# Kostis-S-Z/exploring_meta

Hardware: AMD Instinct MI355X
Metric: tasks/sec (higher is better)
Workload: dtype f32

## Files before the change

### exploring_meta_amd/_lib.py

```python

import ctypes as C
import os
import subprocess

_HERE = os.path.dirname(os.path.abspath(__file__))
CSRC = os.path.join(_HERE, 'csrc')
LIB_PATH = os.path.join(CSRC, 'libmi_maml.so')

_lib = None


class MiModelDesc(C.Structure):
    _fields_ = [('n_layers', C.c_int32), ('in_channels', C.c_int32), ('in_h', C.c_int32), ('in_w', C.c_int32),
                ('hidden', C.c_int32), ('max_pool', C.c_int32), ('ways', C.c_int32), ('head_mean_pool', C.c_int32)]


class MiPolicyDesc(C.Structure):
    _fields_ = [('state_size', C.c_int32), ('action_size', C.c_int32), ('hidden1', C.c_int32), ('hidden2', C.c_int32),
                ('activation', C.c_int32)]


class MiBnTangentArgs(C.Structure):
    _fields_ = [('z', C.c_void_p), ('zd', C.c_void_p), ('mu', C.c_void_p), ('rstd', C.c_void_p), ('m1', C.c_void_p),
                ('m2', C.c_void_p), ('gamma', C.c_void_p), ('beta', C.c_void_p), ('pstride', C.c_size_t),
                ('gammad', C.c_void_p), ('betad', C.c_void_p), ('vstride', C.c_size_t), ('dgamma', C.c_void_p),
                ('dbeta', C.c_void_p), ('gstride', C.c_size_t), ('dp', C.c_void_p), ('dpd', C.c_void_p),
                ('tasks', C.c_int32), ('n', C.c_int32), ('ho', C.c_int32), ('wo', C.c_int32), ('c', C.c_int32),
                ('pool', C.c_int32)]


class MiBlock1Args(C.Structure):
    _fields_ = [('x', C.c_void_p), ('w', C.c_void_p), ('wd', C.c_void_p), ('gamma', C.c_void_p), ('beta', C.c_void_p),
                ('pstride', C.c_size_t), ('gammad', C.c_void_p), ('betad', C.c_void_p), ('vstride', C.c_size_t),
                ('mu', C.c_void_p), ('rstd', C.c_void_p), ('m1', C.c_void_p), ('m2', C.c_void_p), ('dgamma', C.c_void_p),
                ('dbeta', C.c_void_p), ('gstride', C.c_size_t), ('rdgamma', C.c_void_p), ('rdbeta', C.c_void_p),
                ('hstride', C.c_size_t), ('dp', C.c_void_p), ('dpd', C.c_void_p), ('arg_in', C.c_void_p), ('zh_in', C.c_void_p),
                ('tasks', C.c_int32), ('n', C.c_int32), ('h', C.c_int32), ('w_', C.c_int32), ('ci', C.c_int32), ('co', C.c_int32)]


class MiTailArgs(C.Structure):
    _fields_ = [('z', C.c_void_p), ('zd', C.c_void_p), ('mu', C.c_void_p), ('rstd', C.c_void_p), ('m1', C.c_void_p), ('m2', C.c_void_p),
                ('gamma', C.c_void_p), ('beta', C.c_void_p), ('wl', C.c_void_p), ('bl', C.c_void_p), ('pstride', C.c_size_t),
                ('gammad', C.c_void_p), ('betad', C.c_void_p), ('wld', C.c_void_p), ('bld', C.c_void_p), ('vstride', C.c_size_t),
                ('y', C.c_void_p), ('f', C.c_void_p), ('dp', C.c_void_p), ('prob', C.c_void_p), ('dl', C.c_void_p),
                ('pooled', C.c_void_p), ('loss', C.c_void_p), ('acc', C.c_void_p), ('logits', C.c_void_p),
                ('dwl', C.c_void_p), ('dbl', C.c_void_p), ('sum0', C.c_void_p), ('sum1', C.c_void_p), ('gstride', C.c_size_t),
                ('df', C.c_void_p),
                ('tasks', C.c_int32), ('n', C.c_int32), ('ho', C.c_int32), ('wo', C.c_int32), ('c', C.c_int32), ('pool', C.c_int32),
                ('ways', C.c_int32), ('with_grad', C.c_int32), ('bwd_tasks', C.c_int32)]


class MiError(RuntimeError):
    pass


def build(verbose=False):
    r = subprocess.run(['make', '-C', CSRC, '-j4'], capture_output=True, text=True)
    if verbose or r.returncode != 0:
        print(r.stdout[-4000:], r.stderr[-4000:])
    if r.returncode != 0:
        raise MiError('building libmi_maml.so failed')
    return LIB_PATH


_SIGS = {
    'mi_engine_create': (C.c_int, [C.POINTER(MiModelDesc), C.c_int, C.POINTER(C.c_void_p)]),
    'mi_engine_destroy': (None, [C.c_void_p]),
    'mi_last_error': (C.c_char_p, [C.c_void_p]),
    'mi_version': (C.c_char_p, []),
    'mi_engine_set_fused_block1': (C.c_int, [C.c_void_p, C.c_int]),
    'mi_engine_set_overlap': (C.c_int, [C.c_void_p, C.c_int]),
    'mi_engine_set_graph': (C.c_int, [C.c_void_p, C.c_int]),
    'mi_engine_set_bn_export': (C.c_int, [C.c_void_p, C.c_void_p, C.c_size_t]),
    'mi_engine_set_fused_finalize': (C.c_int, [C.c_void_p, C.c_int]),
    'mi_engine_set_fused_block1_reduce': (C.c_int, [C.c_void_p, C.c_int]),
    'mi_debug_plan_offsets': (C.c_int, [C.c_void_p, C.c_int, C.c_int, C.c_int, C.c_int, C.c_int, C.POINTER(C.c_size_t)]),
    'mi_param_count': (C.c_int, [C.c_void_p, C.POINTER(C.c_size_t)]),
    'mi_workspace_bytes': (C.c_int, [C.c_void_p, C.c_int, C.c_int, C.c_int, C.c_int, C.c_int, C.POINTER(C.c_size_t)]),
    'mi_meta_batch_maml': (C.c_int, [C.c_void_p, C.c_void_p, C.c_void_p, C.c_void_p, C.c_void_p, C.c_int, C.c_int, C.c_int,
                                     C.c_int, C.c_float, C.c_int, C.c_int, C.c_void_p, C.c_void_p, C.c_void_p, C.c_void_p,
                                     C.c_void_p, C.c_size_t]),
    'mi_meta_batch_maml_tv': (C.c_int, [C.c_void_p, C.c_void_p, C.c_void_p, C.c_void_p, C.c_void_p, C.c_int, C.c_int, C.c_int, C.c_int,
                                        C.c_int, C.c_float, C.c_int, C.c_void_p, C.c_void_p, C.c_void_p, C.c_void_p, C.c_void_p, C.c_size_t]),
    'mi_workspace_bytes_lr': (C.c_int, [C.c_void_p, C.c_int, C.c_int, C.c_int, C.c_int, C.c_int, C.c_int, C.c_int, C.POINTER(C.c_size_t)]),
    'mi_meta_batch_maml_lr': (C.c_int, [C.c_void_p, C.c_void_p, C.c_void_p, C.c_void_p, C.c_void_p, C.c_int, C.c_int, C.c_int, C.c_int,
                                        C.c_int, C.c_void_p, C.c_int, C.c_int, C.c_void_p, C.c_void_p, C.c_void_p, C.c_void_p, C.c_void_p,
                                        C.c_void_p, C.c_size_t]),
    'mi_workspace_bytes_steps': (C.c_int, [C.c_void_p, C.c_int, C.c_int, C.c_int, C.c_int, C.c_int, C.c_int, C.c_int, C.c_int,
                                           C.POINTER(C.c_size_t)]),
    'mi_meta_batch_maml_steps': (C.c_int, [C.c_void_p, C.c_void_p, C.c_void_p, C.c_void_p, C.c_void_p, C.c_int, C.c_int, C.c_int, C.c_int,
                                           C.c_int, C.c_float, C.c_void_p, C.c_int, C.c_void_p, C.c_int, C.c_void_p, C.c_void_p, C.c_void_p,
                                           C.c_void_p, C.c_void_p, C.c_void_p, C.c_size_t]),
    'mi_engine_set_fused_tail': (C.c_int, [C.c_void_p, C.c_int]),
    'mi_engine_set_fused_last_block': (C.c_int, [C.c_void_p, C.c_int]),
    'mi_debug_tail_stamps': (C.c_int, [C.c_void_p, C.c_void_p]),
    'mi_anil_workspace_bytes': (C.c_int, [C.c_void_p, C.c_int, C.c_int, C.c_int, C.c_int, C.POINTER(C.c_size_t)]),
    'mi_meta_batch_anil': (C.c_int, [C.c_void_p, C.c_void_p, C.c_void_p, C.c_void_p, C.c_void_p, C.c_int, C.c_int, C.c_int,
                                     C.c_int, C.c_float, C.c_int, C.c_int, C.c_void_p, C.c_void_p, C.c_void_p, C.c_void_p,
                                     C.c_void_p, C.c_size_t]),
    'mi_anil_workspace_bytes_steps': (C.c_int, [C.c_void_p] + [C.c_int] * 9 + [C.POINTER(C.c_size_t)]),
    'mi_meta_batch_anil_lr': (C.c_int, [C.c_void_p, C.c_void_p, C.c_void_p, C.c_void_p, C.c_void_p, C.c_int, C.c_int, C.c_int, C.c_int,
                                        C.c_void_p, C.c_int, C.c_int, C.c_int, C.c_void_p, C.c_void_p, C.c_void_p, C.c_void_p, C.c_void_p,
                                        C.c_void_p, C.c_size_t]),
    'mi_meta_batch_anil_steps': (C.c_int, [C.c_void_p, C.c_void_p, C.c_void_p, C.c_void_p, C.c_void_p, C.c_int, C.c_int, C.c_int, C.c_int,
                                           C.c_float, C.c_void_p, C.c_int, C.c_void_p, C.c_int, C.c_int, C.c_void_p, C.c_void_p, C.c_void_p,
                                           C.c_void_p, C.c_void_p, C.c_void_p, C.c_size_t]),
    'mi_forward_workspace_bytes': (C.c_int, [C.c_void_p, C.c_int, C.c_int, C.POINTER(C.c_size_t)]),
    'mi_forward_logits': (C.c_int, [C.c_void_p, C.c_void_p, C.c_void_p, C.c_void_p, C.c_int, C.c_int, C.c_void_p, C.c_void_p,
                                    C.c_size_t]),
    'mi_learner_forward': (C.c_int, [C.c_void_p, C.c_void_p, C.c_void_p, C.c_int, C.c_void_p, C.c_int, C.c_int, C.c_void_p,
                                     C.c_int, C.c_void_p, C.c_void_p, C.c_size_t]),
    'mi_learner_backward': (C.c_int, [C.c_void_p, C.c_void_p, C.c_void_p, C.c_int, C.c_void_p, C.c_void_p, C.c_int, C.c_int,
                                      C.c_void_p, C.c_void_p, C.c_size_t]),
    'mi_learner_hvp_workspace_bytes': (C.c_int, [C.c_void_p, C.c_int, C.c_int, C.POINTER(C.c_size_t)]),
    'mi_learner_hvp': (C.c_int, [C.c_void_p, C.c_void_p, C.c_void_p, C.c_int, C.c_void_p, C.c_void_p, C.c_void_p, C.c_int, C.c_int,
                                 C.c_void_p, C.c_void_p, C.c_void_p, C.c_size_t]),
    'mi_cg_update': (C.c_int, [C.c_void_p, C.c_void_p, C.c_void_p, C.c_void_p, C.c_void_p, C.c_void_p, C.c_void_p, C.c_size_t, C.c_double]),
    'mi_cg_update_checked': (C.c_int, [C.c_void_p, C.c_void_p, C.c_void_p, C.c_void_p, C.c_void_p, C.c_void_p, C.c_void_p, C.c_size_t, C.c_double, C.c_double]),
    'mi_cg_init': (C.c_int, [C.c_void_p, C.c_void_p, C.c_void_p, C.c_void_p, C.c_void_p, C.c_void_p, C.c_void_p, C.c_size_t]),
    'mi_trpo_scale_step': (C.c_int, [C.c_void_p, C.c_void_p, C.c_void_p, C.c_size_t, C.c_float, C.c_void_p, C.c_void_p]),
    'mi_gae_max_rows': (C.c_int, [C.c_int]),
    'mi_upload_i32': (C.c_int, [C.c_void_p, C.c_void_p, C.c_void_p, C.c_int]),
    'mi_copy_segments': (C.c_int, [C.c_void_p, C.c_void_p, C.c_void_p, C.c_void_p, C.c_void_p, C.c_int]),
    'mi_gae_advantages': (C.c_int, [C.c_void_p, C.c_void_p, C.c_void_p, C.c_void_p, C.c_void_p, C.c_void_p, C.c_void_p, C.c_int, C.c_int,
                                    C.c_int, C.c_double, C.c_double, C.c_double, C.c_int, C.c_void_p, C.c_void_p]),
    'mi_adam_step': (C.c_int, [C.c_void_p, C.c_void_p, C.c_void_p, C.c_void_p, C.c_void_p, C.c_size_t, C.c_int, C.c_float,
                               C.c_float, C.c_float, C.c_float, C.c_float]),
    'mi_prepare_batch': (C.c_int, [C.c_void_p, C.c_void_p, C.c_void_p, C.c_int, C.c_int, C.c_int, C.c_int, C.c_int,
                                   C.c_void_p, C.c_void_p, C.c_void_p, C.c_void_p]),
    'mi_input_gram_scratch_bytes': (C.c_size_t, [C.c_int, C.c_int, C.c_int, C.c_int]),
    'mi_input_gram': (C.c_int, [C.c_void_p, C.c_void_p, C.c_int, C.c_int, C.c_int, C.c_int, C.c_int, C.c_void_p, C.c_size_t, C.c_void_p]),
    'mi_gram_bn_stats': (C.c_int, [C.c_void_p, C.c_void_p, C.c_int, C.c_int, C.c_int, C.c_void_p, C.c_size_t, C.c_void_p, C.c_size_t,
                                   C.c_int, C.c_void_p, C.c_void_p, C.c_void_p, C.c_void_p]),
    'mi_cka_scratch_bytes': (C.c_size_t, [C.c_int, C.c_int, C.c_int]),
    'mi_cka': (C.c_int, [C.c_void_p, C.c_void_p, C.c_void_p, C.c_int, C.c_int, C.c_int, C.c_double, C.c_void_p, C.c_size_t,
                         C.c_void_p]),
    'mi_cca_scratch_bytes': (C.c_size_t, [C.c_int, C.c_int, C.c_int]),
    'mi_cca': (C.c_int, [C.c_void_p, C.c_void_p, C.c_void_p, C.c_int, C.c_int, C.c_int, C.c_double, C.c_double, C.c_void_p,
                         C.c_size_t, C.c_void_p, C.c_void_p]),
    'mi_stream_copy': (C.c_int, [C.c_void_p, C.c_void_p, C.c_void_p, C.c_size_t]),
    'mi_sample_tasks': (C.c_int, [C.c_void_p, C.c_void_p, C.c_int, C.c_size_t, C.c_int, C.c_int, C.c_int, C.c_void_p, C.c_void_p,
                                  C.c_int, C.c_int, C.c_void_p]),
    'mi_draw_tasks': (C.c_int, [C.c_void_p, C.c_void_p, C.c_void_p, C.c_int, C.c_int, C.c_int, C.c_void_p, C.c_int, C.c_int, C.c_uint64,
                                C.c_uint64, C.c_uint64, C.c_int, C.c_void_p, C.c_void_p, C.c_void_p, C.c_void_p]),
    'mi_conv3x3_bn_stats': (C.c_int, [C.c_void_p, C.c_void_p, C.c_void_p, C.c_size_t, C.c_int, C.c_int, C.c_int, C.c_int,
                                      C.c_int, C.c_int, C.c_int, C.c_void_p, C.c_void_p, C.c_void_p, C.c_void_p, C.c_size_t]),
    'mi_bn_relu_pool': (C.c_int, [C.c_void_p, C.c_void_p, C.c_void_p, C.c_void_p, C.c_void_p, C.c_void_p, C.c_size_t,
                                  C.c_int, C.c_int, C.c_int, C.c_int, C.c_int, C.c_int, C.c_void_p]),
    'mi_bn_relu_pool_bwd': (C.c_int, [C.c_void_p, C.c_void_p, C.c_void_p, C.c_void_p, C.c_void_p, C.c_void_p, C.c_size_t,
                                      C.c_void_p, C.c_int, C.c_int, C.c_int, C.c_int, C.c_int, C.c_int, C.c_void_p,
                                      C.c_void_p, C.c_size_t, C.c_void_p, C.c_void_p, C.c_size_t]),
    'mi_conv3x3_bwd': (C.c_int, [C.c_void_p, C.c_void_p, C.c_void_p, C.c_void_p, C.c_size_t, C.c_int, C.c_int, C.c_int,
                                 C.c_int, C.c_int, C.c_int, C.c_int, C.c_void_p, C.c_void_p, C.c_size_t, C.c_void_p, C.c_size_t]),
    'mi_head_fwd_bwd': (C.c_int, [C.c_void_p, C.c_void_p, C.c_void_p, C.c_void_p, C.c_size_t, C.c_void_p, C.c_int, C.c_int,
                                  C.c_int, C.c_int, C.c_void_p, C.c_void_p, C.c_void_p, C.c_void_p, C.c_void_p, C.c_void_p,
                                  C.c_void_p, C.c_size_t, C.c_void_p]),
    'mi_kernel_scratch_bytes': (C.c_size_t, [C.c_int, C.c_int, C.c_int, C.c_int, C.c_int]),
    'mi_head_grads': (C.c_int, [C.c_void_p, C.c_void_p, C.c_void_p, C.c_size_t, C.c_void_p] + [C.c_int] * 4 +
                      [C.c_void_p, C.c_void_p, C.c_size_t, C.c_void_p]),
    'mi_head_tangent': (C.c_int, [C.c_void_p] * 5 + [C.c_size_t, C.c_void_p, C.c_void_p, C.c_size_t] + [C.c_void_p] * 4 + [C.c_int] * 5 +
                        [C.c_void_p, C.c_void_p, C.c_size_t, C.c_void_p]),
    'mi_spatial_mean': (C.c_int, [C.c_void_p, C.c_void_p, C.c_void_p, C.c_int, C.c_int, C.c_int]),
    'mi_spatial_mean_bwd': (C.c_int, [C.c_void_p, C.c_void_p, C.c_void_p, C.c_int, C.c_int, C.c_int]),
    'mi_tail_supported': (C.c_int, [C.c_int] * 7),
    'mi_tail_lds_bytes': (C.c_size_t, [C.c_int] * 4),
    'mi_tail_scratch_bytes': (C.c_size_t, [C.c_int] * 7),
    'mi_tail_run': (C.c_int, [C.c_void_p, C.POINTER(MiTailArgs), C.c_int, C.c_void_p, C.c_size_t]),
    'mi_conv3x3_tangent': (C.c_int, [C.c_void_p] * 5 + [C.c_size_t] + [C.c_void_p] * 3 + [C.c_int] * 7 + [C.c_void_p] * 4 + [C.c_size_t]),
    'mi_conv3x3_bwd2': (C.c_int, [C.c_void_p] * 7 + [C.c_size_t] + [C.c_int] * 7 + [C.c_void_p, C.c_void_p, C.c_size_t, C.c_void_p, C.c_size_t]),
    'mi_bn_tangent_fwd': (C.c_int, [C.c_void_p, C.POINTER(MiBnTangentArgs), C.c_void_p]),
    'mi_bn_tangent_bwd': (C.c_int, [C.c_void_p, C.POINTER(MiBnTangentArgs), C.c_void_p, C.c_void_p, C.c_size_t, C.c_void_p,
                                    C.c_void_p, C.c_size_t]),
    'mi_block1_scratch_bytes': (C.c_size_t, [C.c_int] * 6),
    'mi_block1_run': (C.c_int, [C.c_void_p, C.c_int, C.POINTER(MiBlock1Args), C.c_void_p, C.c_void_p, C.c_void_p, C.c_void_p,
                                C.c_void_p, C.c_size_t, C.c_void_p, C.c_size_t]),
    'mi_pooled_reduce': (C.c_int, [C.c_void_p] * 6 + [C.c_int] * 3 + [C.c_void_p, C.c_void_p, C.c_size_t, C.c_void_p, C.c_size_t]),
    'mi_block1_wgrad_gram': (C.c_int, [C.c_void_p, C.POINTER(MiBlock1Args), C.c_void_p, C.c_int, C.c_void_p, C.c_size_t,
                                       C.c_void_p, C.c_size_t]),
    'mi_debug_conv_tiles_per_wave': (C.c_int, [C.c_int] * 5),
    'mi_debug_wgrad_plan': (C.c_int, [C.c_int] * 8 + [C.POINTER(C.c_int)]),
    'mi_debug_conv_plan': (C.c_int, [C.c_int] * 10 + [C.POINTER(C.c_int)]),
    'mi_debug_set_trace': (C.c_int, [C.c_void_p, C.c_void_p, C.c_size_t]),
    'mi_policy_create': (C.c_int, [C.POINTER(MiPolicyDesc), C.c_int, C.POINTER(C.c_void_p)]),
    'mi_policy_destroy': (None, [C.c_void_p]),
    'mi_policy_last_error': (C.c_char_p, [C.c_void_p]),
    'mi_policy_param_count': (C.c_int, [C.c_void_p, C.POINTER(C.c_size_t)]),
    'mi_policy_forward': (C.c_int, [C.c_void_p, C.c_void_p, C.c_void_p, C.c_size_t, C.c_void_p, C.c_int, C.c_int, C.c_void_p,
                                    C.c_void_p, C.c_size_t]),
    'mi_particles_rollout_scratch_bytes': (C.c_size_t, [C.c_void_p, C.c_int, C.c_int, C.c_int]),
    'mi_particles_rollout': (C.c_int, [C.c_void_p, C.c_void_p, C.c_void_p, C.c_size_t, C.c_void_p, C.c_void_p, C.c_uint64, C.c_int, C.c_int,
                                       C.c_int] + [C.c_void_p] * 8 + [C.c_void_p, C.c_size_t]),
    'mi_policy_adapt': (C.c_int, [C.c_void_p, C.c_void_p, C.c_void_p, C.c_size_t, C.c_void_p, C.c_void_p, C.c_void_p,
                                  C.c_void_p, C.c_int, C.c_int, C.c_float, C.c_int, C.c_void_p, C.c_void_p, C.c_void_p, C.c_size_t]),
    'mi_policy_set_fused_fvp': (C.c_int, [C.c_int]),
    'mi_debug_policy_sweep_stamps': (C.c_int, [C.c_void_p]),
    'mi_policy_learner_workspace_bytes': (C.c_int, [C.c_void_p, C.c_int, C.c_int, C.POINTER(C.c_size_t)]),
    'mi_policy_vjp': (C.c_int, [C.c_void_p, C.c_void_p, C.c_void_p, C.c_size_t, C.c_void_p, C.c_void_p, C.c_void_p, C.c_int, C.c_int, C.c_int,
                                C.c_void_p, C.c_void_p, C.c_size_t]),
    'mi_policy_hvp': (C.c_int, [C.c_void_p, C.c_void_p, C.c_void_p, C.c_size_t, C.c_void_p, C.c_void_p, C.c_void_p, C.c_void_p, C.c_int, C.c_int,
                                C.c_int, C.c_void_p, C.c_void_p, C.c_void_p, C.c_size_t]),
    'mi_policy_set_fused_learner': (C.c_int, [C.c_int]),
    'mi_policy_learner_fused_supported': (C.c_int, [C.c_void_p]),
    'mi_debug_conv_stamps': (C.c_int, [C.c_void_p]),
    'mi_conv_set_split_bf16': (C.c_int, [C.c_int]),
    'mi_conv_get_split_bf16': (C.c_int, [C.POINTER(C.c_uint)]),
    'mi_conv_set_b16': (C.c_int, [C.c_int]),
    'mi_block1_set_split_bf16': (C.c_int, [C.c_int]),
    'mi_sparse_wgrad_set_split_bf16': (C.c_int, [C.c_int]),
    'mi_policy_meta_workspace_bytes': (C.c_int, [C.c_void_p, C.c_int, C.c_int, C.c_int, C.c_int, C.c_int, C.POINTER(C.c_size_t)]),
    'mi_policy_meta_batch': (C.c_int, [C.c_void_p, C.c_void_p, C.c_void_p, C.c_int, C.c_void_p, C.c_void_p, C.c_int] + [C.c_void_p] * 8 +
                             [C.c_int, C.c_int, C.c_int, C.c_float, C.c_float, C.c_int, C.c_int, C.c_int, C.c_void_p, C.c_void_p,
                              C.c_void_p, C.c_void_p, C.c_size_t]),
    'mi_policy_meta_batch_dones': (C.c_int, [C.c_void_p, C.c_void_p, C.c_void_p, C.c_int, C.c_void_p, C.c_void_p, C.c_int] + [C.c_void_p] * 10 +
                                   [C.c_int, C.c_int, C.c_int, C.c_float, C.c_float, C.c_int, C.c_int, C.c_int, C.c_void_p, C.c_void_p,
                                    C.c_void_p, C.c_void_p, C.c_size_t]),
    'mi_policy_update_workspace_bytes': (C.c_int, [C.c_void_p, C.c_int, C.c_int, C.POINTER(C.c_size_t)]),
    'mi_policy_update': (C.c_int, [C.c_void_p, C.c_void_p, C.c_void_p, C.c_size_t] + [C.c_void_p] * 5 +
                         [C.c_int, C.c_int, C.c_int, C.c_int, C.c_float, C.c_float, C.c_int, C.c_void_p, C.c_void_p, C.c_void_p, C.c_size_t]),
    'mi_policy_meta_lr_workspace_bytes': (C.c_int, [C.c_void_p, C.c_int, C.c_int, C.c_int, C.c_int, C.c_int, C.c_int, C.c_int,
                                                    C.POINTER(C.c_size_t)]),
    'mi_policy_meta_batch_lr': (C.c_int, [C.c_void_p, C.c_void_p, C.c_void_p, C.c_int, C.c_void_p, C.c_void_p, C.c_void_p, C.c_int] +
                                [C.c_void_p] * 10 + [C.c_int, C.c_int, C.c_int, C.c_float, C.c_void_p, C.c_int, C.c_int, C.c_int, C.c_int] +
                                [C.c_void_p] * 5 + [C.c_size_t]),
    'mi_policy_update_lr': (C.c_int, [C.c_void_p, C.c_void_p, C.c_void_p, C.c_size_t] + [C.c_void_p] * 5 +
                            [C.c_int, C.c_int, C.c_int, C.c_int, C.c_float, C.c_void_p, C.c_int, C.c_void_p, C.c_void_p, C.c_void_p, C.c_size_t]),
    'mi_trpo_steps_workspace_bytes': (C.c_int, [C.c_void_p, C.c_int, C.c_int, C.c_int, C.POINTER(C.c_size_t)]),
    'mi_trpo_surrogate_steps': (C.c_int, [C.c_void_p, C.c_void_p, C.c_void_p, C.c_int] + [C.c_void_p] * 10 +
                                [C.c_int, C.c_int, C.c_float, C.c_void_p, C.c_void_p, C.c_void_p, C.c_void_p, C.c_size_t]),
    'mi_trpo_fvp_steps': (C.c_int, [C.c_void_p, C.c_void_p, C.c_int] + [C.c_void_p] * 5 +
                          [C.c_int, C.c_int, C.c_float, C.c_float, C.c_void_p, C.c_void_p, C.c_void_p, C.c_size_t]),
    'mi_trpo_general_steps_workspace_bytes': (C.c_int, [C.c_void_p, C.c_int, C.c_int, C.c_int, C.POINTER(C.c_size_t)]),
    'mi_trpo_kl_prepare_steps': (C.c_int, [C.c_void_p, C.c_void_p, C.c_int] + [C.c_void_p] * 7 +
                                 [C.c_int, C.c_int, C.c_float, C.c_void_p, C.c_void_p, C.c_size_t]),
    'mi_trpo_fvp_general_steps': (C.c_int, [C.c_void_p, C.c_void_p, C.c_int] + [C.c_void_p] * 6 +
                                  [C.c_int, C.c_int, C.c_float, C.c_float, C.c_void_p, C.c_void_p, C.c_void_p, C.c_size_t]),
    'mi_policy_adapt_lr': (C.c_int, [C.c_void_p, C.c_void_p, C.c_void_p, C.c_size_t, C.c_void_p, C.c_void_p, C.c_void_p,
                                     C.c_void_p, C.c_int, C.c_int, C.c_void_p, C.c_int, C.c_void_p, C.c_void_p, C.c_void_p, C.c_size_t]),
    'mi_trpo_steps_lr_workspace_bytes': (C.c_int, [C.c_void_p, C.c_int, C.c_int, C.c_int, C.c_int, C.POINTER(C.c_size_t)]),
    'mi_trpo_surrogate_steps_lr': (C.c_int, [C.c_void_p, C.c_void_p, C.c_void_p, C.c_int] + [C.c_void_p] * 10 +
                                   [C.c_int, C.c_int, C.c_void_p, C.c_int, C.c_void_p, C.c_void_p, C.c_void_p, C.c_void_p, C.c_void_p,
                                    C.c_size_t]),
    'mi_trpo_fvp_steps_lr': (C.c_int, [C.c_void_p, C.c_void_p, C.c_int] + [C.c_void_p] * 5 +
                             [C.c_int, C.c_int, C.c_void_p, C.c_int, C.c_void_p, C.c_float, C.c_void_p, C.c_void_p, C.c_void_p, C.c_size_t]),
    'mi_trpo_general_steps_lr_workspace_bytes': (C.c_int, [C.c_void_p, C.c_int, C.c_int, C.c_int, C.c_int, C.POINTER(C.c_size_t)]),
    'mi_trpo_kl_prepare_steps_lr': (C.c_int, [C.c_void_p, C.c_void_p, C.c_int] + [C.c_void_p] * 7 +
                                    [C.c_int, C.c_int, C.c_void_p, C.c_int, C.c_void_p, C.c_void_p, C.c_void_p, C.c_size_t]),
    'mi_trpo_fvp_general_steps_lr': (C.c_int, [C.c_void_p, C.c_void_p, C.c_int] + [C.c_void_p] * 6 +
                                     [C.c_int, C.c_int, C.c_void_p, C.c_int, C.c_void_p, C.c_float, C.c_void_p, C.c_void_p, C.c_void_p,
                                      C.c_size_t]),
    'mi_profile_enable': (C.c_int, [C.c_void_p, C.c_int, C.c_int]),
    'mi_profile_kinds': (C.c_int, []),
    'mi_profile_op_name': (C.c_char_p, [C.c_int]),
    'mi_profile_collect': (C.c_int, [C.c_void_p, C.POINTER(C.c_double), C.POINTER(C.c_int64), C.c_int]),
}

EXPORTS = tuple(_SIGS)


def load():
    global _lib
    if _lib is not None:
        return _lib
    path = os.environ.get('MI_MAML_LIB', LIB_PATH)
    if not os.path.exists(path):
        raise MiError(f'{path} is missing: run `python -c "import __graft_entry__ as g; g.build()"` '
                      '(hipcc --offload-arch=gfx950). There is no CPU fallback for the MAML hot path.')
    import torch
    lib = C.CDLL(path)
    for name, (res, args) in _SIGS.items():
        fn = getattr(lib, name)
        fn.restype = res
        fn.argtypes = args
    _lib = lib
    return lib


def check(rc, handle=None):
    if rc != 0:
        msg = load().mi_last_error(handle)
        raise MiError(f'libmi_maml error {rc}: {msg.decode() if msg else "?"}')
```

### exploring_meta_amd/csrc/bn_pool.hip

```cpp
#include "mi_common.h"
#include "kernels.h"

#include "bn_window.h"

#define BN_THREAD_SETUP(POOL)                                                                   \
  const int quads = a.c >> 2;                                                                   \
  const int quad = threadIdx.x % quads, wl = threadIdx.x / quads, wpb = 256 / quads;            \
  const int task = blockIdx.y, c0 = quad * 4;                                                   \
  const WinIter<POOL> it(a);                                                                    \
  const size_t z_task = (size_t)a.n * a.ho * a.wo * a.c;                                        \
  const size_t p_task = (size_t)a.n * it.hp * it.wp * a.c;                                      \
  const ChanConst k = load_consts(a, task, c0);                                                 \
  const float* z_t = a.z + (size_t)task * z_task;                                               \
  (void)p_task; (void)z_t;

__device__ __forceinline__ void block_reduce_write(const double* acc0, const double* acc1, const BnArgs& a, int quads,
                                                   int task) {
  __shared__ double red[256 * 8];
#pragma unroll
  for (int c = 0; c < 4; ++c) {
    red[threadIdx.x * 8 + c] = acc0[c];
    red[threadIdx.x * 8 + 4 + c] = acc1[c];
  }
  __syncthreads();
  if ((int)threadIdx.x < a.c) {
    const int q = threadIdx.x >> 2, comp = threadIdx.x & 3, wpb = 256 / quads;
    double s0 = 0.0, s1 = 0.0;
    for (int w = 0; w < wpb; ++w) {
      s0 += red[(w * quads + q) * 8 + comp];
      s1 += red[(w * quads + q) * 8 + 4 + comp];
    }
    double* pb = a.partial + ((size_t)task * gridDim.x + blockIdx.x) * 2 * a.c;
    mi_partial_store(pb + threadIdx.x, s0, a.fin);
    mi_partial_store(pb + a.c + threadIdx.x, s1, a.fin);
  }
  mi_finalize_last(a.fin, a.partial + (size_t)task * gridDim.x * 2 * a.c, gridDim.x, a.c, task, gridDim.x, red);
}

template <int POOL>
__global__ __launch_bounds__(256) void bn_fwd_kernel(BnArgs a) {
  BN_THREAD_SETUP(POOL)
  float* out_t = a.out + (size_t)task * p_task;
  float* zh_t = a.zh_out ? a.zh_out + (size_t)task * p_task : nullptr;
  unsigned am = 0u;
  Window<POOL> w;
  for (int win = blockIdx.x * wpb + wl; win < it.nwin; win += gridDim.x * wpb) {
    w.locate(a, it, win, c0);
    if (!w.pooled) continue;
    floatx4 umax, zh_at, zd_at;
    scan_window<POOL, false>(w, z_t, nullptr, k, umax, zh_at, zd_at);
    floatx4 o;
#pragma unroll
    for (int c = 0; c < 4; ++c) { o[c] = fmaxf(umax[c], 0.f); mi_amax_acc(am, o[c]); }
    *reinterpret_cast<floatx4*>(out_t + w.poff) = o;
    if (zh_t) *reinterpret_cast<floatx4*>(zh_t + w.poff) = zh_at;
  }
  if (a.amax_out) mi_amax_commit(am, a.amax_out, task);
}

template <int POOL>
__global__ __launch_bounds__(256) void bn_bwd_reduce_kernel(BnArgs a) {
  BN_THREAD_SETUP(POOL)
  const float* dp_t = a.dp + (size_t)task * p_task;
  double dg[4] = {0, 0, 0, 0}, db[4] = {0, 0, 0, 0};
  Window<POOL> w;
  for (int win = blockIdx.x * wpb + wl; win < it.nwin; win += gridDim.x * wpb) {
    w.locate(a, it, win, c0);
    if (!w.pooled) continue;
    floatx4 umax, zh_at, zd_at;
    scan_window<POOL, false>(w, z_t, nullptr, k, umax, zh_at, zd_at);
    const floatx4 d = *reinterpret_cast<const floatx4*>(dp_t + w.poff);
#pragma unroll
    for (int c = 0; c < 4; ++c) {
      const float du = umax[c] > 0.f ? d[c] : 0.f;
      db[c] += (double)du;
      dg[c] += (double)du * (double)zh_at[c];
    }
  }
  block_reduce_write(dg, db, a, quads, task);
}

template <int POOL>
__global__ __launch_bounds__(256) void bn_bwd_apply_kernel(BnArgs a) {
  BN_THREAD_SETUP(POOL)
  const float* dp_t = a.dp + (size_t)task * p_task;
  float* out_t = a.out + (size_t)task * z_task;
  float dgm[4], dbm[4], gr[4];
  load4(a.dgamma + (size_t)task * a.gstride + c0, dgm);
  load4(a.dbeta + (size_t)task * a.gstride + c0, dbm);
#pragma unroll
  for (int c = 0; c < 4; ++c) { dgm[c] *= a.inv_m; dbm[c] *= a.inv_m; gr[c] = k.g[c] * k.r[c]; }
  unsigned am = 0u;
  Window<POOL> w;
  for (int win = blockIdx.x * wpb + wl; win < it.nwin; win += gridDim.x * wpb) {
    w.locate(a, it, win, c0);
    w.analyse(z_t, k);
    float d[4] = {0.f, 0.f, 0.f, 0.f};
    if (w.pooled) load4(dp_t + w.poff, d);
#pragma unroll
    for (int p = 0; p < Window<POOL>::NP; ++p) {
      if (!w.exists[p]) continue;
      float o[4];
#pragma unroll
      for (int c = 0; c < 4; ++c) {
        const float du = (w.pooled && w.arg[c] == p && w.umax[c] > 0.f) ? d[c] : 0.f;
        o[c] = gr[c] * (du - dbm[c] - w.zh[p][c] * dgm[c]);
        mi_amax_acc(am, o[c]);
      }
      store4(out_t + w.off[p], o);
    }
  }
  if (a.amax_out) mi_amax_commit(am, a.amax_out, task);
}

template <int POOL>
__global__ __launch_bounds__(256) void bn_tan_fwd_kernel(BnArgs a) {
  BN_THREAD_SETUP(POOL)
  const float* zd_t = a.zd + (size_t)task * z_task;
  float* out_t = a.out + (size_t)task * p_task;
  float m1[4], m2[4], gd[4], bd[4];
  load4(a.m1 + (size_t)task * a.c + c0, m1);
  load4(a.m2 + (size_t)task * a.c + c0, m2);
  load4(a.gammad + (size_t)task * a.vstride + c0, gd);
  load4(a.betad + (size_t)task * a.vstride + c0, bd);
  unsigned am = 0u;
  Window<POOL> w;
  for (int win = blockIdx.x * wpb + wl; win < it.nwin; win += gridDim.x * wpb) {
    w.locate(a, it, win, c0);
    if (!w.pooled) continue;
    floatx4 umax, zh_at, zd_at;
    scan_window<POOL, true>(w, z_t, zd_t, k, umax, zh_at, zd_at);
    floatx4 o, zo;
#pragma unroll
    for (int c = 0; c < 4; ++c) {
      const float zhd = k.r[c] * (zd_at[c] - m1[c] - zh_at[c] * m2[c]);
      const float ud = gd[c] * zh_at[c] + k.g[c] * zhd + bd[c];
      o[c] = (umax[c] > 0.f) ? ud : 0.f;
      zo[c] = zhd;
      mi_amax_acc(am, o[c]);
    }
    *reinterpret_cast<floatx4*>(out_t + w.poff) = o;
    if (a.zh_out) *reinterpret_cast<floatx4*>(a.zh_out + (size_t)task * p_task + w.poff) = zo;
  }
  if (a.amax_out) mi_amax_commit(am, a.amax_out, task);
}

template <int POOL>
__global__ __launch_bounds__(256) void bn_tan_bwd_reduce_kernel(BnArgs a) {
  BN_THREAD_SETUP(POOL)
  const float* zd_t = a.zd + (size_t)task * z_task;
  const float* dp_t = a.dp + (size_t)task * p_task;
  const float* dpd_t = a.dpd + (size_t)task * p_task;
  float m1[4], m2[4];
  load4(a.m1 + (size_t)task * a.c + c0, m1);
  load4(a.m2 + (size_t)task * a.c + c0, m2);
  double rg[4] = {0, 0, 0, 0}, rb[4] = {0, 0, 0, 0};
  Window<POOL> w;
  for (int win = blockIdx.x * wpb + wl; win < it.nwin; win += gridDim.x * wpb) {
    w.locate(a, it, win, c0);
    if (!w.pooled) continue;
    floatx4 umax, zh_at, zd_at;
    scan_window<POOL, true>(w, z_t, zd_t, k, umax, zh_at, zd_at);
    const floatx4 d = *reinterpret_cast<const floatx4*>(dp_t + w.poff);
    const floatx4 dd = *reinterpret_cast<const floatx4*>(dpd_t + w.poff);
#pragma unroll
    for (int c = 0; c < 4; ++c) {
      const bool on = umax[c] > 0.f;
      const float du = on ? d[c] : 0.f, dud = on ? dd[c] : 0.f;
      const float zhd = k.r[c] * (zd_at[c] - m1[c] - zh_at[c] * m2[c]);
      rb[c] += (double)dud;
      rg[c] += (double)dud * (double)zh_at[c] + (double)du * (double)zhd;
    }
  }
  block_reduce_write(rg, rb, a, quads, task);
}

template <int POOL>
__global__ __launch_bounds__(256) void bn_tan_bwd_apply_kernel(BnArgs a) {
  BN_THREAD_SETUP(POOL)
  const float* zd_t = a.zd + (size_t)task * z_task;
  const float* dp_t = a.dp + (size_t)task * p_task;
  const float* dpd_t = a.dpd + (size_t)task * p_task;
  float* out_t = a.out + (size_t)task * z_task;
  float m1[4], m2[4], gd[4], dgm[4], dbm[4], rgm[4], rbm[4], c1[4], gr[4];
  load4(a.m1 + (size_t)task * a.c + c0, m1);
  load4(a.m2 + (size_t)task * a.c + c0, m2);
  load4(a.gammad + (size_t)task * a.vstride + c0, gd);
  load4(a.dgamma + (size_t)task * a.gstride + c0, dgm);
  load4(a.dbeta + (size_t)task * a.gstride + c0, dbm);
  load4(a.rdgamma + (size_t)task * a.hstride + c0, rgm);
  load4(a.rdbeta + (size_t)task * a.hstride + c0, rbm);
#pragma unroll
  for (int c = 0; c < 4; ++c) {
    dgm[c] *= a.inv_m; dbm[c] *= a.inv_m; rgm[c] *= a.inv_m; rbm[c] *= a.inv_m;
    const float rd = -k.r[c] * k.r[c] * m2[c];
    c1[c] = gd[c] * k.r[c] + k.g[c] * rd;
    gr[c] = k.g[c] * k.r[c];
  }
  unsigned am = 0u;
  Window<POOL> w;
  for (int win = blockIdx.x * wpb + wl; win < it.nwin; win += gridDim.x * wpb) {
    w.locate(a, it, win, c0);
    w.analyse(z_t, k);
    float d[4] = {0.f, 0.f, 0.f, 0.f}, dd[4] = {0.f, 0.f, 0.f, 0.f};
    if (w.pooled) { load4(dp_t + w.poff, d); load4(dpd_t + w.poff, dd); }
#pragma unroll
    for (int p = 0; p < Window<POOL>::NP; ++p) {
      if (!w.exists[p]) continue;
      float zdv[4], o[4];
      load4(zd_t + w.off[p], zdv);
#pragma unroll
      for (int c = 0; c < 4; ++c) {
        const bool sel = w.pooled && w.arg[c] == p && w.umax[c] > 0.f;
        const float du = sel ? d[c] : 0.f, dud = sel ? dd[c] : 0.f;
        const float zh = w.zh[p][c];
        const float zhd = k.r[c] * (zdv[c] - m1[c] - zh * m2[c]);
        const float e = du - dbm[c] - zh * dgm[c];
        o[c] = c1[c] * e + gr[c] * (dud - rbm[c] - zhd * dgm[c] - zh * rgm[c]);
        mi_amax_acc(am, o[c]);
      }
      store4(out_t + w.off[p], o);
    }
  }
  if (a.amax_out) mi_amax_commit(am, a.amax_out, task);
}

__global__ __launch_bounds__(256) void bn_finalize_kernel(const double* __restrict__ partial, int nblk, int c, FinArgs f) {
  __shared__ double red[2 * 256];
  mi_fold_partials<false>(partial + (size_t)blockIdx.x * nblk * 2 * c, nblk, c, f, blockIdx.x, red);
}

template <bool TAN>
__global__ __launch_bounds__(256) void pooled_reduce_kernel(PoolRedArgs a) {
  __shared__ double red[256 * 8];
  const int task = blockIdx.y, quads = a.c >> 2, wpb = 256 / quads;
  const int q = threadIdx.x % quads, rl = threadIdx.x / quads;
  const size_t base = (size_t)task * a.rows * a.c + 4 * q;
  double s0[4] = {0, 0, 0, 0}, s1[4] = {0, 0, 0, 0};
  if (rl < wpb)
    for (int row = blockIdx.x * wpb + rl; row < a.rows; row += gridDim.x * wpb) {
      const size_t off = base + (size_t)row * a.c;
      float p[4], d[4], zh[4], dd[4], zhd[4];
      load4(a.p + off, p); load4(a.dp + off, d); load4(a.zh + off, zh);
      if (TAN) { load4(a.dpd + off, dd); load4(a.zhd + off, zhd); }
#pragma unroll
      for (int c = 0; c < 4; ++c) {
        const bool on = p[c] > 0.f;
        const float dv = on ? d[c] : 0.f;
        if (!TAN) {
          s0[c] += (double)dv * (double)zh[c];
          s1[c] += (double)dv;
        } else {
          const float ddv = on ? dd[c] : 0.f;
          s0[c] += (double)ddv * (double)zh[c] + (double)dv * (double)zhd[c];
          s1[c] += (double)ddv;
        }
      }
    }
#pragma unroll
  for (int c = 0; c < 4; ++c) {
    red[threadIdx.x * 8 + c] = s0[c];
    red[threadIdx.x * 8 + 4 + c] = s1[c];
  }
  __syncthreads();
  if ((int)threadIdx.x < a.c) {
    const int qq = threadIdx.x >> 2, comp = threadIdx.x & 3;
    double t0 = 0.0, t1 = 0.0;
    for (int w = 0; w < wpb; ++w) {
      t0 += red[(w * quads + qq) * 8 + comp];
      t1 += red[(w * quads + qq) * 8 + 4 + comp];
    }
    double* pb = a.partial + ((size_t)task * gridDim.x + blockIdx.x) * 2 * a.c;
    mi_partial_store(pb + threadIdx.x, t0, a.fin);
    mi_partial_store(pb + a.c + threadIdx.x, t1, a.fin);
  }
  mi_finalize_last(a.fin, a.partial + (size_t)task * gridDim.x * 2 * a.c, gridDim.x, a.c, task, gridDim.x, red);
}

int pooled_reduce_blocks(int rows, int c, int tasks) {
  const int wpb = 256 / (c / 4);
  int blocks = ceil_div(rows, wpb);
  const int cap = ceil_div(2048, tasks);
  if (blocks > cap) blocks = cap;
  return blocks < 1 ? 1 : blocks;
}
hipError_t launch_pooled_reduce(hipStream_t st, const PoolRedArgs& a, int tasks, int tangent, int* nblk) {
  if (a.c % 4 || a.c > 256 || 256 % (a.c / 4)) return hipErrorInvalidValue;
  const int blocks = pooled_reduce_blocks(a.rows, a.c, tasks);
  if (tangent) hipLaunchKernelGGL(pooled_reduce_kernel<true>, dim3(blocks, tasks), dim3(256), 0, st, a);
  else hipLaunchKernelGGL(pooled_reduce_kernel<false>, dim3(blocks, tasks), dim3(256), 0, st, a);
  *nblk = blocks;
  return hipGetLastError();
}

int bn_blocks_per_task(int n, int ho, int wo, int c, int pool, int tasks) {
  const int nwin = pool ? n * ((ho + 1) / 2) * ((wo + 1) / 2) : n * ho * wo;
  const int wpb = 256 / (c / 4);
  int blocks = ceil_div(nwin, wpb);
  const int cap = ceil_div(2048, tasks);
  if (blocks > cap) blocks = cap;
  if (blocks < 1) blocks = 1;
  return blocks;
}

hipError_t launch_bn_finalize(hipStream_t st, const double* partial, int nblk, int tasks, int c, double inv_m, int mode,
                              float* out0, size_t stride0, float* out1, size_t stride1) {
  if (c > 256 || 256 % c != 0) return hipErrorInvalidValue;
  const FinArgs f{nullptr, out0, out1, stride0, stride1, inv_m, mode};
  hipLaunchKernelGGL(bn_finalize_kernel, dim3(tasks), dim3(256), 0, st, partial, nblk, c, f);
  return hipGetLastError();
}

#define BN_LAUNCH(KERNEL)                                                                          \
  const int blocks = bn_blocks_per_task(a.n, a.ho, a.wo, a.c, pool, tasks);                        \
  dim3 grid(blocks, tasks);                                                                        \
  if (pool) hipLaunchKernelGGL(KERNEL<1>, grid, dim3(256), 0, st, a);                              \
  else hipLaunchKernelGGL(KERNEL<0>, grid, dim3(256), 0, st, a);

hipError_t launch_bn_fwd(hipStream_t st, const BnArgs& a, int tasks, int pool) {
  BN_LAUNCH(bn_fwd_kernel)
  return hipGetLastError();
}
hipError_t launch_bn_bwd_reduce(hipStream_t st, const BnArgs& a, int tasks, int pool, int* nblk) {
  BN_LAUNCH(bn_bwd_reduce_kernel)
  *nblk = blocks;
  return hipGetLastError();
}
hipError_t launch_bn_bwd_apply(hipStream_t st, const BnArgs& a, int tasks, int pool) {
  BN_LAUNCH(bn_bwd_apply_kernel)
  return hipGetLastError();
}
hipError_t launch_bn_tan_fwd(hipStream_t st, const BnArgs& a, int tasks, int pool) {
  BN_LAUNCH(bn_tan_fwd_kernel)
  return hipGetLastError();
}
hipError_t launch_bn_tan_bwd_reduce(hipStream_t st, const BnArgs& a, int tasks, int pool, int* nblk) {
  BN_LAUNCH(bn_tan_bwd_reduce_kernel)
  *nblk = blocks;
  return hipGetLastError();
}
hipError_t launch_bn_tan_bwd_apply(hipStream_t st, const BnArgs& a, int tasks, int pool) {
  BN_LAUNCH(bn_tan_bwd_apply_kernel)
  return hipGetLastError();
}
```

### exploring_meta_amd/csrc/bn_window.h

```cpp
#pragma once
#include "mi_common.h"
#include "kernels.h"

struct ChanConst {
  float mu[4], r[4], g[4], b[4];
};

__device__ __forceinline__ void load4(const float* p, float* o) {
  const float4 v = *reinterpret_cast<const float4*>(p);
  o[0] = v.x; o[1] = v.y; o[2] = v.z; o[3] = v.w;
}
__device__ __forceinline__ void store4(float* p, const float* o) {
  *reinterpret_cast<float4*>(p) = make_float4(o[0], o[1], o[2], o[3]);
}

__device__ __forceinline__ ChanConst load_consts(const BnArgs& a, int task, int c0) {
  ChanConst k;
  load4(a.mu + (size_t)task * a.c + c0, k.mu);
  load4(a.rstd + (size_t)task * a.c + c0, k.r);
  load4(a.gamma + (size_t)task * a.pstride + c0, k.g);
  load4(a.beta + (size_t)task * a.pstride + c0, k.b);
  return k;
}

template <int POOL>
struct WinIter {
  int hw2, ww2, nwin, hp, wp;
  __device__ WinIter(const BnArgs& a) {
    if (POOL) {
      hw2 = (a.ho + 1) >> 1; ww2 = (a.wo + 1) >> 1; hp = a.ho >> 1; wp = a.wo >> 1;
    } else {
      hw2 = a.ho; ww2 = a.wo; hp = a.ho; wp = a.wo;
    }
    nwin = a.n * hw2 * ww2;
  }
};

template <int POOL>
struct Window {
  static constexpr int NP = POOL ? 4 : 1;
  size_t off[NP];
  bool exists[NP];
  bool pooled;
  size_t poff;
  float zh[NP][4], u[NP][4];
  int arg[4];
  float umax[4];
  bool better[NP][4];

  __device__ __forceinline__ void locate(const BnArgs& a, const WinIter<POOL>& it, int win, int c0) {
    const int n = win / (it.hw2 * it.ww2);
    const int rem = win - n * it.hw2 * it.ww2;
    const int wy = rem / it.ww2, wx = rem - wy * it.ww2;
    if (POOL) {
#pragma unroll
      for (int k = 0; k < NP; ++k) {
        const int y = 2 * wy + (k >> 1), x = 2 * wx + (k & 1);
        exists[k] = (y < a.ho) && (x < a.wo);
        off[k] = ((size_t)(n * a.ho + y) * a.wo + x) * a.c + c0;
      }
      pooled = (wy < it.hp) && (wx < it.wp);
      poff = ((size_t)(n * it.hp + wy) * it.wp + wx) * a.c + c0;
    } else {
      exists[0] = true;
      off[0] = ((size_t)(n * a.ho + wy) * a.wo + wx) * a.c + c0;
      pooled = true;
      poff = off[0];
    }
  }
  __device__ __forceinline__ void analyse(const float* __restrict__ z_t, const ChanConst& k) {
#pragma unroll
    for (int p = 0; p < NP; ++p) {
      float zv[4] = {0.f, 0.f, 0.f, 0.f};
      if (exists[p]) load4(z_t + off[p], zv);
#pragma unroll
      for (int c = 0; c < 4; ++c) {
        zh[p][c] = bn_zh(zv[c], k.mu[c], k.r[c]);
        u[p][c] = bn_u(zh[p][c], k.g[c], k.b[c]);
      }
    }
#pragma unroll
    for (int c = 0; c < 4; ++c) {
      int best = 0;
      float bu = u[0][c];
#pragma unroll
      for (int p = 1; p < NP; ++p) {
        better[p][c] = u[p][c] > bu;
        if (better[p][c]) { bu = u[p][c]; best = p; }
      }
      arg[c] = best;
      umax[c] = bu;
    }
  }
  __device__ __forceinline__ float at_arg(const float (&v)[NP][4], int c) const {
    float r = v[0][c];
#pragma unroll
    for (int p = 1; p < NP; ++p) r = better[p][c] ? v[p][c] : r;
    return r;
  }
};

template <int POOL, bool WITH_ZD>
__device__ __forceinline__ void scan_values(const floatx4* zv, const floatx4* zdv, const ChanConst& k, floatx4& umax, floatx4& zh_at,
                                            floatx4& zd_at) {
#pragma unroll
  for (int p = 0; p < Window<POOL>::NP; ++p) {
    const floatx4 z = zv[p];
    floatx4 zd = {0.f, 0.f, 0.f, 0.f};
    if (WITH_ZD) zd = zdv[p];
#pragma unroll
    for (int c = 0; c < 4; ++c) {
      const float zh = bn_zh(z[c], k.mu[c], k.r[c]);
      const float u = bn_u(zh, k.g[c], k.b[c]);
      if (p == 0) {
        umax[c] = u; zh_at[c] = zh; zd_at[c] = zd[c];
      } else {
        const bool gt = u > umax[c];
        umax[c] = gt ? u : umax[c];
        zh_at[c] = gt ? zh : zh_at[c];
        zd_at[c] = gt ? zd[c] : zd_at[c];
      }
    }
  }
}
template <int POOL, bool WITH_ZD>
__device__ __forceinline__ void scan_window(const Window<POOL>& w, const float* __restrict__ z_t, const float* __restrict__ zd_t,
                                            const ChanConst& k, floatx4& umax, floatx4& zh_at, floatx4& zd_at) {
  floatx4 zv[Window<POOL>::NP], zdv[Window<POOL>::NP];
#pragma unroll
  for (int p = 0; p < Window<POOL>::NP; ++p) {
    zv[p] = *reinterpret_cast<const floatx4*>(z_t + w.off[p]);
    if (WITH_ZD) zdv[p] = *reinterpret_cast<const floatx4*>(zd_t + w.off[p]);
  }
  scan_values<POOL, WITH_ZD>(zv, zdv, k, umax, zh_at, zd_at);
}
```

### exploring_meta_amd/csrc/engine.hip

```cpp
#include <array>
#include <string>
#include <vector>
#include <cstdio>
#include <cmath>
#include <cstring>
#include "mi_common.h"
#include "kernels.h"
#include "../../include/mi_maml.h"

#define EPI_NONE 0
#define EPI_STATS 1
#define EPI_TSTATS 2
#define EPI_BRED 3

static thread_local std::string g_err;

struct Layer {
  int ci, co, h, w, ho, wo, stride, pool, hp, wp;
  size_t off_gamma, off_beta, off_w, off_b;
};

typedef std::array<unsigned long long, 31> GraphKey;
struct mi_engine {
  mi_model_desc d;
  int device;
  std::vector<Layer> L;
  int head_c, head_hw, feat;
  size_t off_wl, off_bl, P;
  size_t PS;
  int32_t* perm_dev;
  bool fuse1 = false;
  bool gram1 = true;
  bool gramq = true;
  bool overlap = true;
  bool fuse_fin = true;
  bool fuse_b1red = true;
  bool fuse_tail = true;
  bool fuse_last = !(getenv("MI_FUSE_LAST") && atoi(getenv("MI_FUSE_LAST")) == 0);
  unsigned long long* tail_stamps = nullptr;
  unsigned zoff[10] = {}, zlen[10] = {};
  int nzero = 0;
  unsigned* counters = nullptr;
  static constexpr int kMaxCounterTasks = 65536;
  struct SideCtx { hipStream_t side = nullptr; hipEvent_t fork = nullptr, join = nullptr; } sc[1];
  std::string err;
  bool graph_on = false;
  struct GraphEntry { GraphKey key; hipGraphExec_t exec = nullptr; hipGraph_t graph = nullptr; int seen = 0; };
  std::vector<GraphEntry> graphs;
  float* bn_export = nullptr;
  size_t bn_export_floats = 0;
  int export_pass = 0;
  float* trace = nullptr;
  size_t trace_floats = 0;
  int prof_on = 0, prof_filter = -1;
  std::vector<hipEvent_t> ev0, ev1;
  std::vector<int> ev_kind;
  size_t ev_used = 0;
};

enum ProfOp { OP_CONV_FWD = 0, OP_BN_FINALIZE, OP_BN_FWD, OP_HEAD, OP_BN_BWD_REDUCE, OP_BN_BWD_APPLY, OP_WGRAD, OP_WGRAD_REDUCE,
              OP_DGRAD, OP_TAN_CONV, OP_BN_TAN_FWD, OP_HEAD_TAN, OP_BN_TAN_BWD_REDUCE, OP_BN_TAN_BWD_APPLY, OP_TAN_WGRAD,
              OP_TAN_DGRAD, OP_MISC, OP_GRAM, OP_GRAM_STATS, OP_COUNT };
static const char* kOpNames[OP_COUNT] = {"conv_fwd_stats", "bn_finalize", "bn_relu_pool_fwd", "head_fwd_bwd", "bn_bwd_reduce",
                                         "bn_bwd_apply", "wgrad", "wgrad_reduce", "dgrad", "tangent_conv_fwd", "bn_tangent_fwd",
                                         "head_tangent", "bn_tangent_bwd_reduce", "bn_tangent_bwd_apply", "tangent_wgrad",
                                         "tangent_dgrad", "misc", "input_gram", "gram_stats"};

static bool prof_begin(mi_engine* e, hipStream_t st, int kind) {
  if (!e || !e->prof_on || (e->prof_filter >= 0 && e->prof_filter != kind)) return false;
  if (e->ev_used == e->ev0.size()) {
    hipEvent_t a, b;
    if (hipEventCreate(&a) != hipSuccess || hipEventCreate(&b) != hipSuccess) return false;
    e->ev0.push_back(a); e->ev1.push_back(b); e->ev_kind.push_back(0);
  }
  e->ev_kind[e->ev_used] = kind;
  (void)hipEventRecord(e->ev0[e->ev_used], st);
  return true;
}
static void prof_end(mi_engine* e, hipStream_t st, bool active) {
  if (!active) return;
  (void)hipEventRecord(e->ev1[e->ev_used], st);
  e->ev_used++;
}

static int fail(mi_engine* e, int code, const std::string& msg) {
  if (e) e->err = msg;
  g_err = msg;
  return code;
}
#define LAUNCH(e, st, op, layer, call)                                                             \
  do {                                                                                             \
    const bool _pa = prof_begin(e, st, (op) * 8 + (layer));                                        \
    hipError_t _s = (call);                                                                        \
    prof_end(e, st, _pa);                                                                          \
    if (_s != hipSuccess)                                                                          \
      return fail(e, MI_ERR_HIP, std::string(#call) + ": " + hipGetErrorString(_s) + " @" + std::to_string(__LINE__)); \
  } while (0)
#define HIPCHK(e, call)                                                                            \
  do {                                                                                             \
    hipError_t _s = (call);                                                                        \
    if (_s != hipSuccess)                                                                          \
      return fail(e, MI_ERR_HIP, std::string(#call) + ": " + hipGetErrorString(_s) + " @" + std::to_string(__LINE__)); \
  } while (0)

static int head_lds_check(mi_engine* e, const char* who, int n, int ways, int tangent) {
  if (head_lds_fits(n, ways, tangent)) return MI_OK;
  return fail(e, MI_ERR_ARG, std::string(who) + ": the classifier head's " + (tangent ? "tangent" : "gradient") + " launch with n = " + std::to_string(n) +
                                 " rows per task and ways = " + std::to_string(ways) + " needs " + std::to_string(head_grads_lds_bytes(n, ways, tangent)) +
                                 " bytes of LDS, the device has " + std::to_string(head_lds_limit_bytes()) + " (n * ways <= " + (tangent ? "19712" : "39424") + ")");
}
#define HEAD_LDS(e, who, n, ways, tangent)                                         \
  do {                                                                             \
    const int _hrc = head_lds_check(e, who, n, ways, tangent);                     \
    if (_hrc) return _hrc;                                                         \
  } while (0)

static FinArgs fin_of(const mi_engine* e, int T, double inv_m, int mode, float* o0, size_t s0, float* o1, size_t s1) {
  const bool on = e->fuse_fin && e->counters && T <= mi_engine::kMaxCounterTasks;
  return FinArgs{on ? e->counters : nullptr, o0, o1, s0, s1, inv_m, mode};
}

static ConvGeom geom(const Layer& l, int n) { return ConvGeom{n, l.h, l.w, l.ho, l.wo, l.ci, l.co, l.stride}; }
static ConvGeom geom_dgrad(const Layer& l, int n) {
  return ConvGeom{n, l.ho, l.wo, l.h, l.w, l.co, l.ci, l.stride};
}

static bool dgrad_carries_reduce(const mi_engine* e, int l) {
  if (!e->fuse_b1red || l < 1 || l >= (int)e->L.size()) return false;
  const Layer& L = e->L[l];
  return L.stride == 1 && L.ci == L.co && L.co == e->L[l - 1].co && L.h == L.ho && L.w == L.wo && (L.ci == 32 || L.ci == 64);
}

extern "C" const char* mi_version(void) { return "mi_maml 0.1 (gfx950)"; }
extern "C" const char* mi_last_error(const mi_engine* e) { return e ? e->err.c_str() : g_err.c_str(); }

extern "C" int mi_engine_create(const mi_model_desc* d, int device, mi_engine** out) {
  if (!d || !out) return fail(nullptr, MI_ERR_ARG, "null argument");
  if (d->n_layers < 1 || d->n_layers > 8) return fail(nullptr, MI_ERR_ARG, "n_layers must be 1..8");
  if (d->hidden != 32 && d->hidden != 64) return fail(nullptr, MI_ERR_ARG, "hidden must be 32 or 64");
  if (d->in_channels != 1 && d->in_channels != 3 && d->in_channels != 32 && d->in_channels != 64)
    return fail(nullptr, MI_ERR_ARG, "in_channels must be 1, 3, 32 or 64");
  if (d->ways < 1 || d->ways > 64) return fail(nullptr, MI_ERR_ARG, "ways must be 1..64");
  mi_engine* e = new mi_engine();
  e->d = *d;
  e->device = device;
  e->perm_dev = nullptr;
  int ci = d->in_channels, h = d->in_h, w = d->in_w;
  size_t off = 0;
  std::vector<int32_t> perm;
  for (int i = 0; i < d->n_layers; ++i) {
    Layer l;
    l.ci = ci; l.co = d->hidden; l.h = h; l.w = w;
    l.stride = d->max_pool ? 1 : 2;
    l.pool = d->max_pool ? 1 : 0;
    l.ho = (h + 2 - 3) / l.stride + 1;
    l.wo = (w + 2 - 3) / l.stride + 1;
    l.hp = l.pool ? l.ho / 2 : l.ho;
    l.wp = l.pool ? l.wo / 2 : l.wo;
    if (l.hp < 1 || l.wp < 1) { delete e; return fail(nullptr, MI_ERR_ARG, "input too small for this many blocks"); }
    l.off_gamma = off; off += l.co;
    l.off_beta = off; off += l.co;
    l.off_w = off; off += (size_t)9 * l.ci * l.co;
    l.off_b = off; off += l.co;
    for (size_t k = perm.size(); k < l.off_w; ++k) perm.push_back((int32_t)k);
    for (int tap = 0; tap < 9; ++tap)
      for (int c1 = 0; c1 < l.ci; ++c1)
        for (int c2 = 0; c2 < l.co; ++c2) perm.push_back((int32_t)(l.off_w + ((size_t)c2 * l.ci + c1) * 9 + tap));
    for (size_t k = perm.size(); k < off; ++k) perm.push_back((int32_t)k);
    e->L.push_back(l);
    ci = l.co; h = l.hp; w = l.wp;
  }
  e->fuse1 = block1_supported(e->L[0].ci, e->L[0].stride, e->L[0].pool, e->L[0].ho, e->L[0].wo, e->L[0].co);
  e->head_c = ci;
  e->head_hw = h * w;
  e->feat = d->head_mean_pool ? ci : ci * h * w;
  e->off_wl = off; off += (size_t)d->ways * e->feat;
  e->off_bl = off; off += d->ways;
  e->P = off;
  e->PS = align_up(off, 64);
  for (const Layer& l : e->L) { e->zoff[e->nzero] = (unsigned)l.off_b; e->zlen[e->nzero] = (unsigned)l.co; e->nzero++; }
  if (e->PS > e->P) { e->zoff[e->nzero] = (unsigned)e->P; e->zlen[e->nzero] = (unsigned)(e->PS - e->P); e->nzero++; }
  for (int wy = 0; wy < d->ways; ++wy)
    for (int i = 0; i < e->feat; ++i) {
      size_t ref;
      if (d->head_mean_pool) ref = (size_t)wy * e->feat + i;
      else { const int s = i / e->head_c, c = i % e->head_c; ref = (size_t)wy * e->feat + (size_t)c * e->head_hw + s; }
      perm.push_back((int32_t)(e->off_wl + ref));
    }
  for (size_t k = perm.size(); k < off; ++k) perm.push_back((int32_t)k);
  int prev = -1;
  (void)hipGetDevice(&prev);
  if (hipSetDevice(device) != hipSuccess) { delete e; return fail(nullptr, MI_ERR_HIP, "hipSetDevice failed"); }
  const bool ok = hipMalloc(&e->perm_dev, perm.size() * sizeof(int32_t)) == hipSuccess &&
                  hipMemcpy(e->perm_dev, perm.data(), perm.size() * sizeof(int32_t), hipMemcpyHostToDevice) == hipSuccess &&
                  hipMalloc(&e->counters, mi_engine::kMaxCounterTasks * sizeof(unsigned)) == hipSuccess &&
                  hipMemset(e->counters, 0, mi_engine::kMaxCounterTasks * sizeof(unsigned)) == hipSuccess;
  if (prev >= 0 && prev != device) (void)hipSetDevice(prev);
  if (!ok) {
    if (e->perm_dev) (void)hipFree(e->perm_dev);
    if (e->counters) (void)hipFree(e->counters);
    delete e;
    return fail(nullptr, MI_ERR_HIP, "allocating the parameter permutation table / arrival counters failed");
  }
  *out = e;
  return MI_OK;
}

extern "C" void mi_engine_destroy(mi_engine* e) {
  if (!e) return;
  if (e->perm_dev) (void)hipFree(e->perm_dev);
  if (e->counters) (void)hipFree(e->counters);
  for (auto& g : e->graphs) {
    if (g.exec) (void)hipGraphExecDestroy(g.exec);
    if (g.graph) (void)hipGraphDestroy(g.graph);
  }
  for (auto& c : e->sc) {
    if (c.fork) (void)hipEventDestroy(c.fork);
    if (c.join) (void)hipEventDestroy(c.join);
  }
  for (auto ev : e->ev0) (void)hipEventDestroy(ev);
  for (auto ev : e->ev1) (void)hipEventDestroy(ev);
  delete e;
}

extern "C" int mi_engine_set_fused_block1(mi_engine* e, int on) {
  if (!e) return MI_ERR_ARG;
  e->fuse1 = on && block1_supported(e->L[0].ci, e->L[0].stride, e->L[0].pool, e->L[0].ho, e->L[0].wo, e->L[0].co);
  e->gram1 = on != 2;
  e->gramq = on != 3;
  return MI_OK;
}

extern "C" int mi_engine_set_fused_finalize(mi_engine* e, int on) {
  if (!e) return MI_ERR_ARG;
  e->fuse_fin = on != 0;
  return MI_OK;
}
extern "C" int mi_engine_set_fused_block1_reduce(mi_engine* e, int on) {
  if (!e) return MI_ERR_ARG;
  e->fuse_b1red = on != 0;
  return MI_OK;
}

extern "C" int mi_engine_set_graph(mi_engine* e, int on) {
  if (!e) return MI_ERR_ARG;
  e->graph_on = on != 0;
  return MI_OK;
}

extern "C" int mi_engine_set_fused_tail(mi_engine* e, int on) {
  if (!e) return MI_ERR_ARG;
  e->fuse_tail = on != 0;
  return MI_OK;
}

extern "C" int mi_engine_set_fused_last_block(mi_engine* e, int on) {
  if (!e) return MI_ERR_ARG;
  e->fuse_last = on != 0;
  return MI_OK;
}

extern "C" int mi_engine_set_overlap(mi_engine* e, int on) {
  if (!e) return MI_ERR_ARG;
  e->overlap = on != 0;
  return MI_OK;
}

static hipStream_t pool_stream(const mi_engine* e, int which) {
  static hipStream_t g_pool[64][1] = {};
  const int d = (e->device >= 0 && e->device < 64) ? e->device : 0;
  if (!g_pool[d][which]) {
    int prev = -1;
    (void)hipGetDevice(&prev);
    if (prev != e->device) (void)hipSetDevice(e->device);
    if (hipStreamCreateWithFlags(&g_pool[d][which], hipStreamNonBlocking) != hipSuccess) g_pool[d][which] = nullptr;
    if (prev >= 0 && prev != e->device) (void)hipSetDevice(prev);
  }
  return g_pool[d][which];
}
static bool make_event(hipEvent_t* ev) { return *ev || hipEventCreateWithFlags(ev, hipEventDisableTiming) == hipSuccess; }

static hipStream_t side_fork(mi_engine* e, hipStream_t st, int half) {
  if (!e->overlap) return st;
  mi_engine::SideCtx& c = e->sc[half];
  if (!c.side) {
    c.side = pool_stream(e, 0);
    if (!c.side || !make_event(&c.fork) || !make_event(&c.join)) { e->overlap = false; return st; }
  }
  if (hipEventRecord(c.fork, st) != hipSuccess || hipStreamWaitEvent(c.side, c.fork, 0) != hipSuccess) return st;
  return c.side;
}
static int side_join(mi_engine* e, hipStream_t st, int half, bool used) {
  if (!used) return MI_OK;
  mi_engine::SideCtx& c = e->sc[half];
  if (hipEventRecord(c.join, c.side) != hipSuccess || hipStreamWaitEvent(st, c.join, 0) != hipSuccess)
    return fail(e, MI_ERR_HIP, "side-stream join failed");
  return MI_OK;
}

extern "C" int mi_engine_set_bn_export(mi_engine* e, float* buf, size_t floats) {
  if (!e) return MI_ERR_ARG;
  e->bn_export = buf;
  e->bn_export_floats = buf ? floats : 0;
  return MI_OK;
}

extern "C" int mi_debug_set_trace(mi_engine* e, float* buf, size_t floats) {
  if (!e) return MI_ERR_ARG;
  e->trace = buf;
  e->trace_floats = buf ? floats : 0;
  return MI_OK;
}

int mi_internal_fail(int code, const char* msg) { return fail(nullptr, code, msg); }

extern "C" int mi_param_count(const mi_engine* e, size_t* n) {
  if (!e || !n) return MI_ERR_ARG;
  *n = e->P;
  return MI_OK;
}

struct Bump {
  char* base;
  size_t off;
  template <class T> T* take(size_t count) {
    off = align_up(off, 256);
    T* p = base ? reinterpret_cast<T*>(base + off) : nullptr;
    off += count * sizeof(T);
    return p;
  }
};

struct ActSet {
  float *z[8], *p[8], *dz[8], *dp[8], *mu[8], *rstd[8];
  float* zhl[8];
  float* zhm;
  uint8_t* arg0;
  float *f, *df, *prob, *dl;
};
struct TanSet {
  float *zd[8], *pd[8], *m1[8], *m2[8];
  float* zhdl[8];
  float* zhdm;
  float* rdz[8];
  float *dpd[2], *fd, *rdf;
};
struct Plan {
  float *theta, *g, *lam, *hv;
  float* lam2;
  float *lrv = nullptr, *dir = nullptr, *dir2 = nullptr, *prod = nullptr;
  float* qg = nullptr;
  float *xs, *xq;
  int32_t *ys, *yq;
  std::vector<ActSet> sup;
  ActSet qry;
  TanSet tan;
  double* bnpart;
  float* wgpart;
  float* wgpart_side;
  float* wgpart_l[8];
  double *gram_part, *gram_s;
  double *gram_q, *gram_part_q;
  int half = 0;
  float *tmp_loss, *tmp_acc;
  float* hscr;
  float* tail_wpart = nullptr; double* tail_bpart = nullptr; float* tail_scr = nullptr;
  unsigned* cells;
  int cell_cap, cell_used = 0, cell_T = 0;
  bool f16 = false;
  std::vector<std::pair<const void*, unsigned*>> cellmap;
  size_t bytes;
};

static void plan_actset(const mi_engine* e, Bump& b, ActSet& A, int T, int n, bool with_bwd) {
  const int nl = (int)e->L.size();
  A.zhm = nullptr;
  A.arg0 = nullptr;
  for (int l = 0; l < 8; ++l) A.zhl[l] = nullptr;
  for (int l = 0; l < nl; ++l) {
    const Layer& L = e->L[l];
    const size_t zs = (size_t)T * n * L.ho * L.wo * L.co, ps = (size_t)T * n * L.hp * L.wp * L.co;
    const bool fused = (l == 0 && e->fuse1);
    A.z[l] = fused ? nullptr : b.take<float>(zs);
    A.p[l] = b.take<float>(ps);
    A.dz[l] = (with_bwd && !fused) ? b.take<float>(zs) : nullptr;
    A.dp[l] = with_bwd ? b.take<float>(ps) : nullptr;
    if (fused && with_bwd && e->gram1) { A.zhm = b.take<float>(ps); A.arg0 = b.take<uint8_t>(ps); }
    A.zhl[l] = (!fused && with_bwd && l >= 1 && L.pool && dgrad_carries_reduce(e, l + 1)) ? b.take<float>(ps) : nullptr;
    A.mu[l] = b.take<float>((size_t)T * L.co);
    A.rstd[l] = b.take<float>((size_t)T * L.co);
  }
  if (e->d.head_mean_pool) {
    A.f = b.take<float>((size_t)T * n * e->feat);
    A.df = with_bwd ? b.take<float>((size_t)T * n * e->feat) : nullptr;
  } else {
    A.f = A.p[nl - 1];
    A.df = A.dp[nl - 1];
  }
  A.prob = b.take<float>((size_t)T * n * e->d.ways);
  A.dl = b.take<float>((size_t)T * n * e->d.ways);
}

static unsigned long long kernel_selection_key() {
  unsigned mask = 0;
  const unsigned form = (unsigned)mi_conv_get_split_bf16(&mask);
  return (unsigned long long)form + 4ull * (unsigned)conv_b16() + 16ull * (unsigned)block1_split_form() + 64ull * (unsigned)sparse_wgrad_split_form() + 128ull * (unsigned long long)mask;
}

struct PlanShape { int T, ns, nq, K, second_order, lr_steps, want_lr_grad, steps; };
static PlanShape maml_shape(int tasks, int ways, int shots, int K, int second_order, int lr_steps, int want_lr_grad, int steps = 0) {
  return PlanShape{tasks, ways * shots, ways * shots, K, second_order, lr_steps, want_lr_grad, steps};
}
static PlanShape forward_shape(int tasks, int n) { return PlanShape{tasks, n, n, 0, 0, 0, 0, 0}; }
static PlanShape hvp_shape(int tasks, int n) { return PlanShape{tasks, n, n, 1, 1, 0, 0, 0}; }

template <class Between>
static void plan_partials(const mi_engine* e, Bump& b, Plan& pl, int T, int n, bool per_block, bool gram, int ng, bool gram_q, bool cells_first,
                          Between between) {
  const int nl = (int)e->L.size();
  size_t bnp = 0, wgp = 0, pmax = 0;
  for (int l = 0; l < nl; ++l) {
    const Layer& L = e->L[l];
    const ConvGeom gg = geom(L, n);
    int blk = conv_max_blocks_per_task(gg);
    const int bb = bn_blocks_per_task(n, L.ho, L.wo, L.co, L.pool, 1);
    if (bb > blk) blk = bb;
    const size_t need = (size_t)T * blk * 2 * L.co;
    if (need > bnp) bnp = need;
    size_t w = wgrad_partial_floats(gg, T);
    if (l == 0 && e->fuse1) {
      int bpt = block1_blocks_per_task(n, L.ho, L.wo, L.co, T);
      const int sb = sparse_wgrad_blocks_per_task(n, L.ho, L.wo, L.co, T);
      if (sb > bpt) bpt = sb;
      w = (size_t)T * bpt * 9 * L.ci * L.co;
    }
    if (w > wgp) wgp = w;
    const size_t ps = (size_t)T * n * L.hp * L.wp * L.co;
    if (ps > pmax) pmax = ps;
  }
  pl.bnpart = b.take<double>(bnp);
  pl.wgpart = b.take<float>(wgp);
  pl.wgpart_side = b.take<float>(wgp);
  for (int l = 0; l < 8; ++l) pl.wgpart_l[l] = nullptr;
  for (int l = 0; per_block && l < nl; ++l) {
    if (l == 0 && e->fuse1) { pl.wgpart_l[0] = pl.wgpart; continue; }
    pl.wgpart_l[l] = b.take<float>(wgrad_partial_floats(geom(e->L[l], n), T));
  }
  auto cells = [&] {
    pl.cells = conv_operand_form() == 2 ? b.take<unsigned>((size_t)pl.cell_cap * T * MI_CELL_WORDS) : nullptr;
    pl.cell_T = T;
  };
  if (cells_first) cells();
  pl.gram_part = pl.gram_s = pl.gram_q = pl.gram_part_q = nullptr;
  if (gram && e->fuse1 && e->gram1 && gram_supported(e->L[0].w, e->L[0].ci)) {
    pl.gram_part = b.take<double>(gram_partial_doubles(T, ng, e->L[0].h, e->L[0].ci));
    pl.gram_s = b.take<double>(gram_doubles(T, e->L[0].ci));
    if (gram_q) {
      pl.gram_q = b.take<double>(gram_doubles(T, e->L[0].ci));
      pl.gram_part_q = b.take<double>(gram_partial_doubles(T, ng, e->L[0].h, e->L[0].ci));
    }
  }
  if (!cells_first) { between(pmax); cells(); }
}

static void make_plan(const mi_engine* e, void* ws, const PlanShape& s, Plan& pl) {
  const int T = s.T, ns = s.ns, nq = s.nq, K = s.K, second_order = s.second_order;
  Bump b{reinterpret_cast<char*>(ws), 0};
  const int nl = (int)e->L.size();
  const size_t TP = (size_t)T * e->PS;
  pl.theta = b.take<float>(TP * (K + 1));
  pl.g = b.take<float>(TP * (K > 0 ? K : 1));
  pl.lam = b.take<float>(TP);
  pl.hv = b.take<float>(TP);
  pl.lam2 = (second_order && K > 0) ? b.take<float>(TP) : nullptr;
  const size_t img = (size_t)e->d.in_h * e->d.in_w * e->d.in_channels;
  pl.xs = b.take<float>((size_t)T * ns * img);
  pl.xq = b.take<float>((size_t)T * nq * img);
  pl.ys = b.take<int32_t>((size_t)T * ns);
  pl.yq = b.take<int32_t>((size_t)T * nq);
  pl.tmp_loss = b.take<float>(T);
  pl.tmp_acc = b.take<float>(T);
  const int nmax = ns > nq ? ns : nq;
  pl.hscr = b.take<float>((size_t)T * nmax * (e->d.ways + 2));
  pl.tail_wpart = b.take<float>(tail_wpart_floats(T, e->feat, e->d.ways));
  pl.tail_bpart = b.take<double>(tail_bpart_doubles(T, e->L.back().co));
  pl.tail_scr = b.take<float>(tail_scr_floats(T, nmax, e->d.ways));
  const int nsets = (second_order && K > 0) ? K : 1;
  pl.sup.resize(nsets);
  for (int k = 0; k < nsets; ++k) plan_actset(e, b, pl.sup[k], T, ns, true);
  plan_actset(e, b, pl.qry, T, nq, true);
  pl.cell_cap = 8 + (K + 1) * 2 * nl + K * 4 * nl + 4 * nl;
  if (s.steps) pl.cell_cap += K * 2 * nl;
  const bool swept_twice = K >= 2 || (K >= 1 && second_order);
  plan_partials(e, b, pl, T, nmax, true, swept_twice, ns, e->gramq && nq == ns, false, [&](size_t pmax) {
    if (!(second_order && K > 0)) return;
    TanSet& X = pl.tan;
    for (int l = 0; l < nl; ++l) {
      const Layer& L = e->L[l];
      X.zd[l] = (l == 0 && e->fuse1) ? nullptr : b.take<float>((size_t)T * ns * L.ho * L.wo * L.co);
      X.pd[l] = b.take<float>((size_t)T * ns * L.hp * L.wp * L.co);
      if (l == 0) X.zhdm = e->fuse1 ? b.take<float>((size_t)T * ns * L.hp * L.wp * L.co) : nullptr;
      X.zhdl[l] = (!(l == 0 && e->fuse1) && l >= 1 && L.pool && dgrad_carries_reduce(e, l + 1)) ? b.take<float>((size_t)T * ns * L.hp * L.wp * L.co) : nullptr;
      X.m1[l] = b.take<float>((size_t)T * L.co);
      X.m2[l] = b.take<float>((size_t)T * L.co);
    }
    for (int l = 0; l < nl; ++l) {
      const Layer& L = e->L[l];
      X.rdz[l] = (l == 0 && e->fuse1) ? nullptr : b.take<float>((size_t)T * ns * L.ho * L.wo * L.co);
    }
    X.dpd[0] = b.take<float>(pmax);
    X.dpd[1] = b.take<float>(pmax);
    if (e->d.head_mean_pool) {
      X.fd = b.take<float>((size_t)T * ns * e->feat);
      X.rdf = b.take<float>((size_t)T * ns * e->feat);
    } else {
      X.fd = nullptr;
      X.rdf = nullptr;
    }
  });
  if (s.lr_steps > 0) {
    pl.lrv = b.take<float>((size_t)s.lr_steps * e->PS);
    if (second_order && K > 0) {
      pl.dir = b.take<float>(TP);
      pl.dir2 = b.take<float>(TP);
      if (s.want_lr_grad) pl.prod = b.take<float>(TP * K);
    } else if (s.steps == 2 && s.want_lr_grad) {
      pl.prod = b.take<float>(TP * K);
    }
  }
  if (s.steps == 2) pl.qg = b.take<float>(TP * K);
  pl.bytes = align_up(b.off, 256);
}

static int plan_in(mi_engine* e, void* workspace, size_t workspace_bytes, const PlanShape& s, Plan& pl) {
  make_plan(e, workspace, s, pl);
  if (pl.bytes > workspace_bytes)
    return fail(e, MI_ERR_WORKSPACE, "workspace too small: need " + std::to_string(pl.bytes) + " bytes");
  return MI_OK;
}

static int plan_bytes(const mi_engine* e, const PlanShape& s, size_t* bytes) {
  Plan pl;
  make_plan(e, nullptr, s, pl);
  *bytes = pl.bytes;
  return MI_OK;
}

static int plan_begin(mi_engine* e, hipStream_t st, Plan& pl) {
  pl.f16 = conv_operand_form() == 2;
  pl.cell_used = 0;
  pl.cellmap.clear();
  if (pl.f16) HIPCHK(e, hipMemsetAsync(pl.cells, 0, (size_t)pl.cell_cap * pl.cell_T * MI_CELL_WORDS * sizeof(unsigned), st));
  return MI_OK;
}
static unsigned* cell_bind(mi_engine* e, Plan& pl, const void* tensor) {
  static const bool no_hooks = getenv("MI_F16_NO_PRODUCER_AMAX") && atoi(getenv("MI_F16_NO_PRODUCER_AMAX")) != 0;
  if (!pl.f16 || !tensor) return nullptr;
  for (auto it = pl.cellmap.begin(); it != pl.cellmap.end(); ++it)
    if (it->first == tensor) { pl.cellmap.erase(it); break; }
  if (no_hooks || pl.cell_used >= pl.cell_cap) return nullptr;
  unsigned* c = pl.cells + (size_t)(pl.cell_used++) * pl.cell_T * MI_CELL_WORDS;
  pl.cellmap.emplace_back(tensor, c);
  return c;
}
static int cell_of(mi_engine* e, hipStream_t st, Plan& pl, const float* tensor, size_t per_task, int T, const unsigned** out) {
  *out = nullptr;
  if (!pl.f16 || !tensor) return MI_OK;
  for (const auto& kv : pl.cellmap)
    if (kv.first == tensor) { *out = kv.second; return MI_OK; }
  if (pl.cell_used >= pl.cell_cap) return fail(e, MI_ERR_WORKSPACE, "fp16 operand form: no largest-magnitude cell left for this call");
  unsigned* c = pl.cells + (size_t)(pl.cell_used++) * pl.cell_T * MI_CELL_WORDS;
  pl.cellmap.emplace_back(tensor, c);
  LAUNCH(e, st, OP_MISC, 5, launch_amax(st, tensor, per_task, T, c));
  *out = c;
  return MI_OK;
}

extern "C" int mi_debug_plan_offsets(const mi_engine* e, int tasks, int ways, int shots, int adapt_steps, int second_order,
                                     size_t* out) {
  if (!e || !out) return MI_ERR_ARG;
  Plan pl;
  char* base = reinterpret_cast<char*>(4096);
  make_plan(e, base, maml_shape(tasks, ways, shots, adapt_steps, second_order, 0, 0), pl);
  auto off = [&](const void* p) { return (size_t)(reinterpret_cast<const char*>(p) - base); };
  out[0] = off(pl.theta); out[1] = off(pl.g); out[2] = off(pl.xs); out[3] = off(pl.sup[0].p[0]); out[4] = off(pl.sup[0].dp[0]);
  out[5] = off(pl.sup[0].mu[0]); out[6] = off(pl.sup[0].rstd[0]); out[7] = off(pl.sup[0].p[1]); out[8] = off(pl.qry.p[0]);
  out[9] = pl.bytes;
  return MI_OK;
}

static bool lr_steps_ok(int lr_steps, int adapt_steps) { return lr_steps == 1 || (adapt_steps > 0 && lr_steps == adapt_steps); }

extern "C" int mi_workspace_bytes(const mi_engine* e, int tasks, int ways, int shots, int adapt_steps, int second_order,
                                  size_t* bytes) {
  if (!e || !bytes || tasks < 1 || ways < 1 || shots < 1 || adapt_steps < 0) return MI_ERR_ARG;
  return plan_bytes(e, maml_shape(tasks, ways, shots, adapt_steps, second_order, 0, 0), bytes);
}

extern "C" int mi_workspace_bytes_lr(const mi_engine* e, int tasks, int ways, int shots, int adapt_steps, int second_order, int lr_steps,
                                     int want_lr_grad, size_t* bytes) {
  if (!e || !bytes || tasks < 1 || ways < 1 || shots < 1 || adapt_steps < 0) return MI_ERR_ARG;
  if (!lr_steps_ok(lr_steps, adapt_steps)) return MI_ERR_ARG;
  return plan_bytes(e, maml_shape(tasks, ways, shots, adapt_steps, second_order, lr_steps, want_lr_grad), bytes);
}

static PlanShape steps_shape(int tasks, int grad_tasks, int ways, int shots, int K, int second_order, int lr_steps, int want_lr_grad) {
  return maml_shape(tasks, ways, shots, K, (second_order && grad_tasks > 0) ? 1 : 0, lr_steps, want_lr_grad, grad_tasks > 0 ? 2 : 1);
}
extern "C" int mi_workspace_bytes_steps(const mi_engine* e, int tasks, int grad_tasks, int ways, int shots, int adapt_steps, int second_order,
                                        int lr_steps, int want_lr_grad, size_t* bytes) {
  if (!e || !bytes || tasks < 1 || grad_tasks < 0 || grad_tasks > tasks || ways < 1 || shots < 1 || adapt_steps < 1) return MI_ERR_ARG;
  if (lr_steps != 0 && !lr_steps_ok(lr_steps, adapt_steps)) return MI_ERR_ARG;
  return plan_bytes(e, steps_shape(tasks, grad_tasks, ways, shots, adapt_steps, second_order, lr_steps, want_lr_grad), bytes);
}

struct Tangent {
  const float* v;
  const float* g;
  float* hv;
  TanSet& X;
  int cur = 0;
};

#define CELL(ptr, per_task, out)                                                   \
  do {                                                                             \
    const int _crc = cell_of(e, st, pl, ptr, per_task, T, &(out));                 \
    if (_crc) return _crc;                                                         \
  } while (0)

static B1Args b1_args(const mi_engine* e, Plan& pl, const ActSet& A, const Tangent* tan, const float* x0, int n, const float* theta) {
  const Layer& L = e->L[0];
  const size_t P = e->PS;
  B1Args a{};
  a.x = x0;
  a.w = theta + L.off_w; a.wstride = P;
  a.mu = A.mu[0]; a.rstd = A.rstd[0];
  a.gamma = theta + L.off_gamma; a.beta = theta + L.off_beta; a.pstride = P;
  a.partial = pl.bnpart; a.wpartial = pl.wgpart;
  a.n = n; a.hh = L.ho; a.ww = L.wo; a.co = L.co;
  a.inv_m = 1.f / (float)(n * L.ho * L.wo);
  if (tan) {
    a.wd = tan->v + L.off_w; a.vstride = P;
    a.m1 = tan->X.m1[0]; a.m2 = tan->X.m2[0];
    a.gammad = tan->v + L.off_gamma; a.betad = tan->v + L.off_beta;
    a.dgamma = tan->g + L.off_gamma; a.dbeta = tan->g + L.off_beta; a.gstride = P;
  }
  return a;
}

static BnArgs bn_args(const mi_engine* e, const ActSet& A, const Tangent* tan, int l, int n, const float* theta) {
  const Layer& L = e->L[l];
  const size_t P = e->PS;
  BnArgs ba{};
  ba.z = A.z[l]; ba.mu = A.mu[l]; ba.rstd = A.rstd[l];
  ba.gamma = theta + L.off_gamma; ba.beta = theta + L.off_beta; ba.pstride = P;
  ba.dp = A.dp[l];
  ba.n = n; ba.ho = L.ho; ba.wo = L.wo; ba.c = L.co;
  ba.inv_m = 1.f / (float)(n * L.ho * L.wo);
  if (tan) {
    ba.zd = tan->X.zd[l]; ba.m1 = tan->X.m1[l]; ba.m2 = tan->X.m2[l];
    ba.gammad = tan->v + L.off_gamma; ba.betad = tan->v + L.off_beta; ba.vstride = P;
    ba.dgamma = tan->g + L.off_gamma; ba.dbeta = tan->g + L.off_beta; ba.gstride = P;
    ba.dpd = tan->X.dpd[tan->cur];
  }
  return ba;
}

static HeadArgs head_args(const mi_engine* e, float* hscr, const float* f, const float* theta, const float* v, float* g, float* df, int n, int T) {
  HeadArgs ha{};
  ha.f = f;
  ha.wl = theta + e->off_wl; ha.bl = theta + e->off_bl; ha.pstride = e->PS;
  if (v) { ha.wld = v + e->off_wl; ha.bld = v + e->off_bl; ha.vstride = e->PS; }
  ha.dwl = g ? g + e->off_wl : nullptr; ha.dbl = g ? g + e->off_bl : nullptr; ha.gstride = e->PS;
  ha.df = df;
  ha.n = n; ha.feat = e->feat; ha.ways = e->d.ways;
  if (hscr) {
    ha.rdl = hscr;
    ha.rowloss = hscr + (size_t)T * n * e->d.ways;
    ha.rowhit = ha.rowloss + (size_t)T * n;
  }
  return ha;
}
static HeadArgs head_args_primal(const mi_engine* e, float* hscr, const float* f, const int32_t* y, int n, int T, const float* theta, float* g,
                                 float* loss, float* acc, float* logits, float* prob, float* dl, float* df, bool with_grad) {
  HeadArgs ha = head_args(e, hscr, f, theta, nullptr, with_grad ? g : nullptr, with_grad ? df : nullptr, n, T);
  ha.y = y; ha.loss = loss; ha.acc = acc; ha.logits = logits; ha.prob = prob; ha.dl = dl;
  return ha;
}

static bool fused_last_ok(const mi_engine* e, const Plan& pl, int n, int T) {
  const int nl = (int)e->L.size();
  if (!e->fuse_last || e->d.head_mean_pool || pl.f16 || (nl == 1 && e->fuse1) || !e->counters || T > mi_engine::kMaxCounterTasks || T > 65535 ||
      !pl.tail_wpart)
    return false;
  const Layer& L = e->L[nl - 1];
  return tail_supported(n, L.ho, L.wo, L.co, L.pool, e->feat, e->d.ways);
}
static TailArgs tail_args(const mi_engine* e, const Plan& pl, const ActSet& A, const Tangent* tan, const HeadArgs& ha, int n, const float* theta,
                          float* g, bool with_grad, int Tb) {
  const int l = (int)e->L.size() - 1;
  const Layer& L = e->L[l];
  TailArgs ta{};
  ta.bn = bn_args(e, A, tan, l, n, theta);
  ta.bn.out = tan ? tan->X.rdz[l] : A.dz[l];
  ta.hd = ha;
  ta.pooled = tan ? tan->X.pd[l] : A.p[l];
  ta.sum0 = with_grad ? g + L.off_gamma : nullptr; ta.sum1 = with_grad ? g + L.off_beta : nullptr; ta.sum_stride = e->PS;
  ta.with_grad = with_grad ? 1 : 0; ta.bwd_tasks = Tb;
  ta.wpart = pl.tail_wpart; ta.bpart = pl.tail_bpart; ta.scr = pl.tail_scr; ta.counter = e->counters; ta.stamps = e->tail_stamps;
  return ta;
}
extern "C" int mi_debug_tail_stamps(mi_engine* e, unsigned long long* buf) {
  if (!e) return MI_ERR_ARG;
  e->tail_stamps = buf;
  return MI_OK;
}

static bool block1_reads_stored_argmax(const mi_engine* e, const ActSet& A, const double* gram) {
  const Layer& L = e->L[0];
  return gram && A.arg0 && sparse_wgrad_supported(L.wo, L.ci, L.co);
}

static int trunk_forward(mi_engine* e, hipStream_t st, Plan& pl, ActSet& A, const float* x0, int n, int T, const float* theta,
                         const double* gram = nullptr, bool stats_ready = false, bool skip_last_bn = false, const Tangent* tan = nullptr) {
  const int nl = (int)e->L.size();
  const size_t P = e->PS;
  const int fin_mode = tan ? FIN_TSTATS : FIN_STATS, op_conv = tan ? OP_TAN_CONV : OP_CONV_FWD, op_bn = tan ? OP_BN_TAN_FWD : OP_BN_FWD;
  for (int l = 0; l < nl; ++l) {
    const Layer& L = e->L[l];
    const int mpix = n * L.ho * L.wo;
    const double inv_m = 1.0 / ((double)n * L.ho * L.wo);
    float* s0 = tan ? tan->X.m1[l] : A.mu[l];
    float* s1 = tan ? tan->X.m2[l] : A.rstd[l];
    if (l == 0 && e->fuse1) {
      B1Args ba = b1_args(e, pl, A, tan, x0, n, theta);
      int blk = 0;
      if (gram && stats_ready) {
      } else if (gram) {
        LAUNCH(e, st, OP_GRAM_STATS, 0, launch_gram_stats(st, gram, T, L.ci, L.co, theta + L.off_w, P, ba.wd, ba.vstride, inv_m, tan ? 1 : 0, s0, s1,
                                                          tan ? A.mu[0] : nullptr, tan ? A.rstd[0] : nullptr));
      } else {
        ba.fin = fin_of(e, T, inv_m, fin_mode, s0, L.co, s1, L.co);
        LAUNCH(e, st, op_conv, 0, launch_block1(st, ba, T, L.ci, tan ? B1_TSTATS : B1_STATS, &blk));
        if (!ba.fin.counter)
          LAUNCH(e, st, OP_BN_FINALIZE, 0, launch_bn_finalize(st, pl.bnpart, blk, T, L.co, inv_m, fin_mode, s0, L.co, s1, L.co));
        ba.fin = FinArgs{};
      }
      int mode = B1_FWD;
      if (tan) {
        ba.out = tan->X.pd[0];
        ba.zh_out = A.zhm ? tan->X.zhdm : nullptr;
        mode = B1_TFWD;
        if (A.zhm && A.arg0) {
          ba.arg_in = A.arg0; ba.zh_in = A.zhm;
          mode = B1_TFWD_ARG;
        }
      } else {
        ba.out = A.p[0];
        ba.zh_out = A.zhm;
        ba.arg_out = A.arg0;
        ba.fwd_fp32 = (gram && A.arg0) ? 0 : 1;
      }
      ba.amax_out = cell_bind(e, pl, ba.out);
      LAUNCH(e, st, op_bn, 0, launch_block1(st, ba, T, L.ci, mode, nullptr));
      continue;
    }
    ConvArgs ca{};
    int nterms = 1;
    ca.in[0] = l == 0 ? x0 : A.p[l - 1];
    ca.wt[0] = (tan ? tan->v : theta) + L.off_w;
    if (tan) {
      if (l > 0) { ca.in[1] = tan->X.pd[l - 1]; ca.wt[1] = theta + L.off_w; nterms = 2; }
      ca.z = A.z[l]; ca.mu = A.mu[l]; ca.rstd = A.rstd[l];
    }
    ca.wstride = P;
    ca.out = tan ? tan->X.zd[l] : A.z[l];
    ca.partial = pl.bnpart;
    ca.g = geom(L, n);
    ca.mpix = mpix;
    int blk = 0;
    ca.fin = fin_of(e, T, 1.0 / (double)mpix, fin_mode, s0, L.co, s1, L.co);
    if (l >= 1) {
      CELL(ca.in[0], (size_t)n * L.h * L.w * L.ci, ca.amax[0]);
      if (tan) CELL(ca.in[1], (size_t)n * L.h * L.w * L.ci, ca.amax[1]);
    }
    LAUNCH(e, st, op_conv, l, launch_conv3x3(st, ca, T, nterms, tan ? EPI_TSTATS : EPI_STATS, 0, &blk));
    if (!ca.fin.counter)
      LAUNCH(e, st, OP_BN_FINALIZE, l, launch_bn_finalize(st, pl.bnpart, blk, T, L.co, 1.0 / (double)mpix, fin_mode, s0, L.co, s1, L.co));
    if (skip_last_bn && l == nl - 1) break;
    BnArgs ba = bn_args(e, A, tan, l, n, theta);
    ba.out = tan ? tan->X.pd[l] : A.p[l];
    ba.zh_out = tan ? (A.zhl[l] ? tan->X.zhdl[l] : nullptr) : A.zhl[l];
    ba.amax_out = cell_bind(e, pl, ba.out);
    LAUNCH(e, st, op_bn, l, tan ? launch_bn_tan_fwd(st, ba, T, L.pool) : launch_bn_fwd(st, ba, T, L.pool));
  }
  return MI_OK;
}

static const float* zh_at_argmax(const mi_engine* e, const ActSet& A, int lower) {
  return (lower == 0 && e->fuse1) ? A.zhm : A.zhl[lower];
}

static void adv_add_seg(AdvanceArgs* adv, size_t off, int nelem, const float* partial, int nchunks) {
  AdvanceSeg& sg = adv->seg[adv->nseg++];
  sg.off = (unsigned)off; sg.nelem = (unsigned)nelem; sg.partial = partial; sg.nchunks = nchunks;
}
static int trunk_backward(mi_engine* e, hipStream_t st, Plan& pl, ActSet& A, const float* x0, int n, int T, const float* theta,
                          float* g, const double* gram = nullptr, AdvanceArgs* adv = nullptr, bool last_bn_done = false, Tangent* tan = nullptr) {
  const int nl = (int)e->L.size();
  const size_t P = e->PS;
  const int op_red = tan ? OP_BN_TAN_BWD_REDUCE : OP_BN_BWD_REDUCE, op_apply = tan ? OP_BN_TAN_BWD_APPLY : OP_BN_BWD_APPLY,
            op_wgrad = tan ? OP_TAN_WGRAD : OP_WGRAD, op_dgrad = tan ? OP_TAN_DGRAD : OP_DGRAD;
  bool forked = false, red_done[9] = {false, false, false, false, false, false, false, false, false};
  auto issue_wgrad = [&](hipStream_t ws, WgradArgs& w, int wl) -> int {
    const Layer& Lw = e->L[wl];
    w.partial = adv ? pl.wgpart_l[wl] : (ws != st ? pl.wgpart_side : pl.wgpart);
    int nch = 0;
    LAUNCH(e, ws, op_wgrad, wl, launch_wgrad3x3(ws, w, T, (tan && wl > 0) ? 2 : 1, &nch));
    if (adv) adv_add_seg(adv, Lw.off_w, 9 * Lw.ci * Lw.co, w.partial, nch);
    else LAUNCH(e, ws, OP_WGRAD_REDUCE, wl, launch_wgrad_reduce(ws, w.partial, nch, 9 * Lw.ci * Lw.co, T, g + Lw.off_w, P));
    return MI_OK;
  };
  for (int l = nl - 1; l >= 0; --l) {
    const Layer& L = e->L[l];
    const int mpix = n * L.ho * L.wo;
    const float* dpd = tan ? tan->X.dpd[tan->cur] : nullptr;
    if (l == 0 && e->fuse1) {
      B1Args b1 = b1_args(e, pl, A, tan, x0, n, theta);
      b1.dp = A.dp[0]; b1.dpd = dpd;
      int blk = 0;
      const FinArgs fin = fin_of(e, T, 1.0, FIN_SUMS, g + L.off_gamma, P, g + L.off_beta, P);
      if (red_done[0]) {
      } else if (A.zhm) {
        PoolRedArgs pr{A.p[0], A.zhm, tan ? tan->X.zhdm : nullptr, A.dp[0], dpd, pl.bnpart, n * L.hp * L.wp, L.co, fin};
        LAUNCH(e, st, op_red, 0, launch_pooled_reduce(st, pr, T, tan ? 1 : 0, &blk));
      } else {
        b1.fin = fin;
        LAUNCH(e, st, op_red, 0, launch_block1(st, b1, T, L.ci, tan ? B1_TBWD_REDUCE : B1_BWD_REDUCE, &blk));
        b1.fin = FinArgs{};
      }
      if (!fin.counter && !red_done[0])
        LAUNCH(e, st, OP_BN_FINALIZE, 0, launch_bn_finalize(st, pl.bnpart, blk, T, L.co, 1.0, FIN_SUMS, g + L.off_gamma, P, g + L.off_beta, P));
      if (tan) { b1.rdgamma = g + L.off_gamma; b1.rdbeta = g + L.off_beta; b1.hstride = P; }
      else { b1.dgamma = g + L.off_gamma; b1.dbeta = g + L.off_beta; b1.gstride = P; }
      if (block1_reads_stored_argmax(e, A, gram)) {
        SparseWgArgs sw{};
        sw.x = x0; sw.arg = A.arg0; sw.dp = A.dp[0]; sw.wpartial = pl.wgpart; sw.n = n; sw.hh = L.ho; sw.ww = L.wo; sw.co = L.co;
        if (tan) {
          sw.dpd = dpd; sw.rstd = A.rstd[0]; sw.m2 = b1.m2;
          sw.gamma = b1.gamma; sw.pstride = P; sw.gammad = b1.gammad; sw.vstride = P;
        }
        LAUNCH(e, st, op_wgrad, 0, launch_sparse_wgrad(st, sw, T, L.ci, tan ? 1 : 0, &blk));
        GramWgArgs gw{};
        gw.g = gram; gw.spartial = pl.wgpart; gw.nblk = blk; gw.w = b1.w; gw.wstride = P; gw.wd = b1.wd; gw.vstride = b1.vstride;
        gw.mu = A.mu[0]; gw.rstd = A.rstd[0]; gw.m1 = b1.m1; gw.m2 = b1.m2;
        gw.gamma = b1.gamma; gw.pstride = P; gw.gammad = b1.gammad;
        gw.dgamma = b1.dgamma; gw.dbeta = b1.dbeta; gw.gstride = P;
        gw.rdgamma = b1.rdgamma; gw.rdbeta = b1.rdbeta; gw.hstride = b1.hstride;
        gw.out = g + L.off_w; gw.ostride = P; gw.ci = L.ci; gw.co = L.co; gw.inv_m = 1.0 / (double)mpix;
        if (adv) { adv->b1_wgrad = 1; adv->gw_tangent = tan ? 1 : 0; adv->gw = gw; }
        else LAUNCH(e, st, OP_WGRAD_REDUCE, 0, launch_gram_wgrad(st, gw, T, tan ? 1 : 0));
        continue;
      }
      LAUNCH(e, st, op_wgrad, 0, launch_block1(st, b1, T, L.ci, tan ? B1_TBWD_WGRAD : B1_BWD_WGRAD, &blk));
      if (adv) adv_add_seg(adv, L.off_w, 9 * L.ci * L.co, pl.wgpart, blk);
      else LAUNCH(e, st, OP_WGRAD_REDUCE, 0, launch_wgrad_reduce(st, pl.wgpart, blk, 9 * L.ci * L.co, T, g + L.off_w, P));
      continue;
    }
    BnArgs ba = bn_args(e, A, tan, l, n, theta);
    ba.partial = pl.bnpart;
    int blk = 0;
    const bool bn_done = last_bn_done && l == nl - 1;
    if (!red_done[l] && !bn_done) {
      ba.fin = fin_of(e, T, 1.0, FIN_SUMS, g + L.off_gamma, P, g + L.off_beta, P);
      LAUNCH(e, st, op_red, l, tan ? launch_bn_tan_bwd_reduce(st, ba, T, L.pool, &blk) : launch_bn_bwd_reduce(st, ba, T, L.pool, &blk));
      if (!ba.fin.counter)
        LAUNCH(e, st, OP_BN_FINALIZE, l, launch_bn_finalize(st, pl.bnpart, blk, T, L.co, 1.0, FIN_SUMS, g + L.off_gamma, P, g + L.off_beta, P));
    }
    if (tan) { ba.rdgamma = g + L.off_gamma; ba.rdbeta = g + L.off_beta; ba.hstride = P; }
    else { ba.dgamma = g + L.off_gamma; ba.dbeta = g + L.off_beta; ba.gstride = P; }
    float* dz = tan ? tan->X.rdz[l] : A.dz[l];
    ba.out = dz;
    ba.amax_out = cell_bind(e, pl, ba.out);
    LAUNCH(e, st, op_apply, l, tan ? launch_bn_tan_bwd_apply(st, ba, T, L.pool) : launch_bn_bwd_apply(st, ba, T, L.pool));
    WgradArgs wa{};
    wa.x[0] = l == 0 ? x0 : A.p[l - 1];
    wa.dz[0] = dz;
    if (tan && l > 0) { wa.x[1] = tan->X.pd[l - 1]; wa.dz[1] = A.dz[l]; }
    if (l >= 1) {
      CELL(wa.x[0], (size_t)n * L.h * L.w * L.ci, wa.amax_x[0]);
      CELL(wa.dz[0], (size_t)n * L.ho * L.wo * L.co, wa.amax_dz[0]);
      if (tan) {
        CELL(wa.x[1], (size_t)n * L.h * L.w * L.ci, wa.amax_x[1]);
        CELL(wa.dz[1], (size_t)n * L.ho * L.wo * L.co, wa.amax_dz[1]);
      }
    }
    wa.g = geom(L, n);
    wa.mpix = mpix;
    hipStream_t ws = l > 0 ? side_fork(e, st, pl.half) : st;
    if (ws != st) forked = true;
    const int rc = issue_wgrad(ws, wa, l);
    if (rc) return rc;
    if (l > 0) {
      ConvArgs ca{};
      ca.in[0] = dz; ca.wt[0] = theta + L.off_w; ca.amax[0] = wa.amax_dz[0];
      if (tan) { ca.in[1] = A.dz[l]; ca.wt[1] = tan->v + L.off_w; ca.amax[1] = wa.amax_dz[1]; }
      ca.wstride = P;
      ca.out = tan ? tan->X.dpd[tan->cur ^ 1] : A.dp[l - 1];
      ca.g = geom_dgrad(L, n);
      ca.mpix = n * L.h * L.w;
      const int nterms = tan ? 2 : 1;
      const float* zh_lo = dgrad_carries_reduce(e, l) ? zh_at_argmax(e, A, l - 1) : nullptr;
      const float* zhd_lo = !tan ? nullptr : (l - 1 == 0 && e->fuse1) ? tan->X.zhdm : tan->X.zhdl[l - 1];
      if (zh_lo && (!tan || zhd_lo)) {
        const Layer& L0 = e->L[l - 1];
        ca.bp = A.p[l - 1]; ca.bzh = zh_lo; ca.partial = pl.bnpart;
        if (tan) { ca.bzhd = zhd_lo; ca.bdp = A.dp[l - 1]; }
        ca.barg = (l - 1 == 0 && e->fuse1) ? A.arg0 : nullptr;
        ca.fin = fin_of(e, T, 1.0, FIN_SUMS, g + L0.off_gamma, P, g + L0.off_beta, P);
        int blk0 = 0;
        LAUNCH(e, st, op_dgrad, l, launch_conv3x3(st, ca, T, nterms, EPI_BRED, 1, &blk0));
        if (!ca.fin.counter)
          LAUNCH(e, st, OP_BN_FINALIZE, l - 1, launch_bn_finalize(st, pl.bnpart, blk0, T, L0.co, 1.0, FIN_SUMS, g + L0.off_gamma, P, g + L0.off_beta, P));
        red_done[l - 1] = true;
      } else {
        LAUNCH(e, st, op_dgrad, l, launch_conv3x3(st, ca, T, nterms, EPI_NONE, 1, nullptr));
      }
      if (tan) tan->cur ^= 1;
    }
  }
  return side_join(e, st, pl.half, forked);
}

static int head_pass(mi_engine* e, hipStream_t st, float* hscr, const float* f, const int32_t* y, int n, int T, const float* theta,
                     float* g, float* loss, float* acc, float* logits, float* prob, float* dl, float* df, bool with_grad) {
  const HeadArgs ha = head_args_primal(e, hscr, f, y, n, T, theta, g, loss, acc, logits, prob, dl, df, with_grad);
  if (with_grad) HEAD_LDS(e, "head", n, ha.ways, 0);
  LAUNCH(e, st, OP_HEAD, 0, launch_head_fwd_bwd(st, ha, T, with_grad ? 1 : 0));
  return MI_OK;
}

static int export_bn_stats(mi_engine* e, hipStream_t st, const ActSet& A, int T) {
  if (!e->bn_export) return MI_OK;
  const int nl = (int)e->L.size();
  int ctot = 0;
  for (const Layer& L : e->L) ctot += L.co;
  const size_t need = (size_t)(e->export_pass + 1) * T * 2 * ctot;
  if (need > e->bn_export_floats) return fail(e, MI_ERR_WORKSPACE, "BatchNorm export buffer too small: need " + std::to_string(need) + " floats");
  BnExportArgs ea{};
  ea.nl = nl; ea.ctot = ctot;
  int off = 0;
  for (int l = 0; l < nl; ++l) { ea.mu[l] = A.mu[l]; ea.rstd[l] = A.rstd[l]; ea.c[l] = e->L[l].co; ea.off[l] = off; off += e->L[l].co; }
  ea.out = e->bn_export + (size_t)e->export_pass * T * 2 * ctot;
  HIPCHK(e, launch_bn_export(st, ea, T));
  e->export_pass += 1;
  return MI_OK;
}

struct ExportPause {
  mi_engine* e; float* buf;
  explicit ExportPause(mi_engine* e_) : e(e_), buf(e_ ? e_->bn_export : nullptr) { if (e) e->bn_export = nullptr; }
  ~ExportPause() { if (e) e->bn_export = buf; }
};

static int pass_fwd_bwd(mi_engine* e, hipStream_t st, Plan& pl, ActSet& A, const float* x0, const int32_t* y, int n, int T,
                        const float* theta, float* g, float* loss, float* acc, float* logits, bool with_grad,
                        const double* gram = nullptr, AdvanceArgs* adv = nullptr, bool stats_ready = false, int Tb = -1) {
  const int nl = (int)e->L.size();
  if (Tb < 0) Tb = T;
  const bool fused_last = fused_last_ok(e, pl, n, T);
  int rc = trunk_forward(e, st, pl, A, x0, n, T, theta, gram, stats_ready, fused_last);
  if (rc) return rc;
  rc = export_bn_stats(e, st, A, T);
  if (rc) return rc;
  if (e->d.head_mean_pool) HIPCHK(e, launch_spatial_mean(st, A.p[nl - 1], A.f, T * n, e->head_hw, e->head_c));
  if (with_grad && !adv) HIPCHK(e, hipMemsetAsync(g, 0, (size_t)T * e->PS * sizeof(float), st));
  if (fused_last) {
    const HeadArgs ha = head_args_primal(e, pl.hscr, A.f, y, n, T, theta, g, loss, acc, logits, A.prob, A.dl, A.df, with_grad);
    const TailArgs ta = tail_args(e, pl, A, nullptr, ha, n, theta, g, with_grad, Tb);
    LAUNCH(e, st, OP_HEAD, 0, launch_tail(st, ta, T, e->L[nl - 1].pool, 0));
    if (!with_grad || Tb == 0) return MI_OK;
    return trunk_backward(e, st, pl, A, x0, n, Tb, theta, g, gram, adv, true);
  }
  rc = head_pass(e, st, pl.hscr, A.f, y, n, T, theta, g, loss, acc, logits, A.prob, A.dl, A.df, with_grad);
  if (rc || !with_grad || Tb == 0) return rc;
  if (e->d.head_mean_pool) HIPCHK(e, launch_spatial_mean_bwd(st, A.df, A.dp[nl - 1], Tb * n, e->head_hw, e->head_c));
  return trunk_backward(e, st, pl, A, x0, n, Tb, theta, g, gram, adv);
}

static int pass_hvp(mi_engine* e, hipStream_t st, Plan& pl, ActSet& A, const float* x0, int n, int T, const float* theta,
                    const float* g, const float* v, float* hv, const double* gram = nullptr, const float* dl_fixed = nullptr,
                    float* ld_out = nullptr, AdvanceArgs* adv = nullptr, bool stats_ready = false) {
  const int nl = (int)e->L.size();
  TanSet& X = pl.tan;
  Tangent tan{v, g, hv, X};
  const bool fused_last = !dl_fixed && !ld_out && fused_last_ok(e, pl, n, T);
  if (!adv) HIPCHK(e, hipMemsetAsync(hv, 0, (size_t)T * e->PS * sizeof(float), st));
  const int rc = trunk_forward(e, st, pl, A, x0, n, T, theta, gram, stats_ready, fused_last, &tan);
  if (rc) return rc;
  const float* fd = X.pd[nl - 1];
  if (e->d.head_mean_pool) {
    HIPCHK(e, launch_spatial_mean(st, X.pd[nl - 1], X.fd, T * n, e->head_hw, e->head_c));
    fd = X.fd;
  }
  HeadArgs ha = head_args(e, pl.hscr, A.f, theta, v, hv, e->d.head_mean_pool ? X.rdf : X.dpd[tan.cur], n, T);
  ha.fd = fd;
  ha.prob = A.prob; ha.dl = A.dl;
  if (dl_fixed) { ha.dl = const_cast<float*>(dl_fixed); ha.fixed_dl = 1; ha.ld_out = ld_out; }
  if (fused_last) {
    const TailArgs ta = tail_args(e, pl, A, &tan, ha, n, theta, hv, true, T);
    LAUNCH(e, st, OP_HEAD_TAN, 0, launch_tail(st, ta, T, e->L[nl - 1].pool, 1));
  } else {
    HEAD_LDS(e, "head tangent", n, ha.ways, 1);
    LAUNCH(e, st, OP_HEAD_TAN, 0, launch_head_tangent(st, ha, T));
  }
  if (e->d.head_mean_pool) HIPCHK(e, launch_spatial_mean_bwd(st, X.rdf, X.dpd[tan.cur], T * n, e->head_hw, e->head_c));
  return trunk_backward(e, st, pl, A, x0, n, T, theta, hv, gram, adv, fused_last, &tan);
}

static AdvanceArgs advance_base(const mi_engine* e, float* g) {
  AdvanceArgs a{};
  a.g = g; a.gstride = e->PS; a.ostride = e->PS; a.n = (unsigned)e->PS;
  a.nzero = e->nzero;
  for (int z = 0; z < e->nzero; ++z) { a.zoff[z] = e->zoff[z]; a.zlen[z] = e->zlen[z]; }
  a.off_w1 = (unsigned)e->L[0].off_w;
  a.ci = (e->L[0].ci == 1 || e->L[0].ci == 3) ? e->L[0].ci : 0;
  a.co = e->L[0].co;
  a.counter = e->counters;
  return a;
}

enum MetaAlgo { ALGO_MAML = 0, ALGO_ANIL = 1, ALGO_MAML_LR = 2, ALGO_MAML_STEPS = 3, ALGO_ANIL_LR = 4, ALGO_ANIL_STEPS = 5 };
static bool is_anil(MetaAlgo a) { return a == ALGO_ANIL || a == ALGO_ANIL_LR || a == ALGO_ANIL_STEPS; }
struct MetaCall {
  MetaAlgo algo;
  const float* theta; const float* data; const int64_t* labels;
  int tasks, grad_tasks, ways, shots, adapt_steps, second_order;
  float inner_lr;
  const float* lr_vec; int lr_steps; float* lr_grad_out;
  float *loss_out, *acc_out, *meta_grad_out, *logits_out;
  void* workspace; size_t workspace_bytes;
  const float* step_w = nullptr;
};

static int check_call(mi_engine* e, const MetaCall& c) {
  if (!e) return fail(nullptr, MI_ERR_ARG, "null engine");
  if (c.grad_tasks < 0 || c.grad_tasks > c.tasks) return fail(e, MI_ERR_ARG, "grad_tasks must be in 0..tasks");
  if (c.algo == ALGO_MAML_STEPS) {
    if (c.adapt_steps < 1) return fail(e, MI_ERR_ARG, "mi_meta_batch_maml_steps needs adapt_steps >= 1: its weights are those of theta_1 .. theta_K");
    if (!c.step_w) return fail(e, MI_ERR_ARG, "step_w is NULL: mi_meta_batch_maml_steps takes adapt_steps weights on the device");
    if (e->trace) return fail(e, MI_ERR_ARG, "the debug trace does not cover mi_meta_batch_maml_steps");
    if (!c.lr_vec && c.lr_grad_out) return fail(e, MI_ERR_ARG, "lr_grad_out given without lr_vec");
  }
  if (c.algo == ALGO_MAML_LR || (c.algo == ALGO_MAML_STEPS && c.lr_vec)) {
    if (!lr_steps_ok(c.lr_steps, c.adapt_steps))
      return fail(e, MI_ERR_ARG, "lr_steps = " + std::to_string(c.lr_steps) + " must be 1 or adapt_steps = " + std::to_string(c.adapt_steps) +
                                     (c.adapt_steps == 0 ? " (without inner steps: 1)" : ""));
    if (!c.lr_vec) return fail(e, MI_ERR_ARG, "lr_vec is NULL: mi_meta_batch_maml_lr takes lr_steps * P step sizes on the device");
    if (c.lr_grad_out && c.grad_tasks == 0)
      return fail(e, MI_ERR_ARG, "lr_grad_out given but grad_tasks = 0: the step-size gradient is summed over the train tasks");
  }
  if (c.algo == ALGO_ANIL_STEPS) {
    if (c.adapt_steps < 1)
      return fail(e, MI_ERR_ARG, "mi_meta_batch_anil_steps needs adapt_steps >= 1, got " + std::to_string(c.adapt_steps) + ": its weights are those of theta_1 .. theta_K");
    if (!c.step_w) return fail(e, MI_ERR_ARG, "step_w is NULL: mi_meta_batch_anil_steps takes adapt_steps weights on the device");
    if (!c.lr_vec && c.lr_grad_out) return fail(e, MI_ERR_ARG, "mi_meta_batch_anil_steps: lr_grad_out given without lr_vec");
  }
  if (c.algo == ALGO_ANIL_LR || c.algo == ALGO_ANIL_STEPS) {
    const char* who = c.algo == ALGO_ANIL_LR ? "mi_meta_batch_anil_lr" : "mi_meta_batch_anil_steps";
    if (e->trace) return fail(e, MI_ERR_ARG, std::string("the debug trace does not cover ") + who);
    if (c.algo == ALGO_ANIL_LR && !c.lr_vec)
// ... 232 lines not shown
static size_t anil_head_stride(const mi_engine* e) { return align_up(e->P - e->off_wl, 64); }
static void make_anil_ext(const mi_engine* e, void* ws, size_t plain_bytes, int T, int n, int K, bool with_grad, bool so, int lr_steps,
                          bool want_lr_grad, bool steps, AnilExt& ax) {
  Bump b{reinterpret_cast<char*>(ws), plain_bytes};
  ax = AnilExt{};
  ax.hs = anil_head_stride(e);
  const size_t th = (size_t)T * ax.hs;
  if (lr_steps > 0) ax.lrh = b.take<float>((size_t)lr_steps * ax.hs);
  if (lr_steps > 0 && with_grad && so && K > 0) ax.dir = b.take<float>(th);
  if (steps && with_grad) {
    if (K > 1) ax.qg = b.take<float>(th * (K - 1));
    ax.dqt = b.take<float>((size_t)T * n * e->feat);
  }
  if (lr_steps > 0 && with_grad && want_lr_grad && K > 0 && (so || steps)) ax.prod = b.take<float>(th * K);
  ax.bytes = align_up(b.off, 256);
}

extern "C" int mi_anil_workspace_bytes_steps(const mi_engine* e, int tasks, int ways, int shots, int adapt_steps, int with_grad, int second_order,
                                             int lr_steps, int want_lr_grad, int step_outputs, size_t* bytes) {
  if (!e || !bytes || tasks < 1 || ways < 1 || shots < 1 || adapt_steps < 0 || lr_steps < 0) return MI_ERR_ARG;
  if (lr_steps != 0 && !lr_steps_ok(lr_steps, adapt_steps)) return MI_ERR_ARG;
  if (lr_steps == 0 && !step_outputs) return MI_ERR_ARG;
  AnilPlan ap;
  make_anil_plan(e, nullptr, tasks, ways * shots, adapt_steps, ap);
  AnilExt ax;
  make_anil_ext(e, nullptr, ap.bytes, tasks, ways * shots, adapt_steps, with_grad != 0, with_grad && second_order, lr_steps, want_lr_grad != 0,
                step_outputs != 0, ax);
  *bytes = ax.bytes;
  return MI_OK;
}

static int meta_batch_anil_impl(mi_engine* e, void* stream, const MetaCall& c) {
  hipStream_t st = reinterpret_cast<hipStream_t>(stream);
  const int T = c.tasks, K = c.adapt_steps, n = c.ways * c.shots, nl = (int)e->L.size(), with_grad = c.grad_tasks > 0;
  const float inner_lr = c.inner_lr;
  const bool ext = c.lr_vec || c.step_w, msl = c.step_w != nullptr, so = c.second_order && with_grad;
  AnilPlan ap;
  make_anil_plan(e, c.workspace, T, n, K, ap);
  AnilExt ax{};
  if (ext) make_anil_ext(e, c.workspace, ap.bytes, T, n, K, with_grad != 0, so, c.lr_vec ? c.lr_steps : 0, c.lr_grad_out != nullptr, msl, ax);
  if ((ext ? ax.bytes : ap.bytes) > c.workspace_bytes)
    return fail(e, MI_ERR_WORKSPACE, "workspace too small: need " + std::to_string(ext ? ax.bytes : ap.bytes) + " bytes");
  const size_t TP = (size_t)T * e->PS, fsz = (size_t)T * n * e->feat, pw = (size_t)T * n * e->d.ways;
  const int Ph = (int)(e->P - e->off_wl), hbase = (int)e->off_wl;
  const size_t hb = (size_t)e->d.ways * e->feat;
  const int32_t* hperm = e->perm_dev + e->off_wl;
  auto lr_of = [&](int k) { return ax.lrh + (c.lr_steps == 1 ? 0 : (size_t)k * ax.hs); };
  LAUNCH(e, st, OP_MISC, 0, launch_nchw_to_nhwc(st, c.data, (size_t)T * 2 * n, e->d.in_channels, e->d.in_h, e->d.in_w, ap.x));
  LAUNCH(e, st, OP_MISC, 0, launch_split_labels(st, c.labels, T, 2 * n, ap.ys, ap.yq));
  LAUNCH(e, st, OP_MISC, 1, launch_gather_params(st, c.theta, 0, e->perm_dev, (int)e->P, (int)e->PS, T, ap.theta));
  const double* gram = with_grad ? ap.scratch.gram_s : nullptr;
  if (gram)
    LAUNCH(e, st, OP_GRAM, 0, launch_input_gram(st, ap.x, T, 2 * n, e->L[0].h, e->L[0].w, e->L[0].ci, ap.scratch.gram_part, ap.scratch.gram_s));
  int rc = plan_begin(e, st, ap.scratch);
  if (rc) return rc;
  rc = trunk_forward(e, st, ap.scratch, ap.act, ap.x, 2 * n, T, ap.theta, gram);
  if (rc) return rc;
  e->export_pass = 0;
  rc = export_bn_stats(e, st, ap.act, T);
  if (rc) return rc;
  LAUNCH(e, st, OP_MISC, 4, launch_split_rows(st, ap.act.p[nl - 1], T, 2 * n, e->feat, ap.fs, ap.fq));
  if (c.lr_vec) LAUNCH(e, st, OP_MISC, 1, launch_anil_gather_lr(st, c.lr_vec, hperm, hbase, Ph, (int)ax.hs, c.lr_steps, ax.lrh));
  if (msl && with_grad) HIPCHK(e, hipMemsetAsync(ap.dfq, 0, fsz * sizeof(float), st));
  auto query_at = [&](int j) -> int {
    const bool bwd = with_grad && j >= 1;
    HeadArgs ha = head_args_primal(e, ap.hscr, ap.fq, ap.yq, n, T, ap.theta + (size_t)j * TP, ap.lam, c.loss_out + (size_t)j * T,
                                   c.acc_out + (size_t)j * T, c.logits_out ? c.logits_out + (size_t)j * pw : nullptr, ap.prob + K * pw,
                                   ap.dl + K * pw, ax.dqt, bwd);
    if (bwd && j < K) { ha.dwl = ax.qg + (size_t)(j - 1) * T * ax.hs; ha.dbl = ha.dwl + hb; ha.gstride = ax.hs; }
    if (bwd) HEAD_LDS(e, "head", n, ha.ways, 0);
    LAUNCH(e, st, OP_HEAD, 0, launch_head_fwd_bwd(st, ha, T, bwd ? 1 : 0));
    if (bwd) LAUNCH(e, st, OP_MISC, 2, launch_fma_dev(st, ap.dfq, ax.dqt, c.step_w + (j - 1), fsz));
    return MI_OK;
  };
  for (int k = 0; k < K; ++k) {
    if (msl) { rc = query_at(k); if (rc) return rc; }
    float* th = ap.theta + (size_t)k * TP;
    float* gk = ap.g + (size_t)k * TP;
    if (!ext) HIPCHK(e, hipMemsetAsync(gk, 0, TP * sizeof(float), st));
    rc = head_pass(e, st, ap.hscr, ap.fs, ap.ys, n, T, th, gk, ap.tmp_loss, ap.tmp_acc, nullptr, ap.prob + k * pw, ap.dl + k * pw,
                   nullptr, true);
    if (rc) return rc;
    if (ext)
      LAUNCH(e, st, OP_MISC, 2, launch_anil_advance(st, th + hbase, gk + hbase, e->PS, c.lr_vec ? lr_of(k) : nullptr, inner_lr, Ph, T, th + TP + hbase));
    else
      LAUNCH(e, st, OP_MISC, 2, launch_axpy(st, th, gk, inner_lr, TP, th + TP));
  }
  float* thK = ap.theta + (size_t)K * TP;
  if (with_grad) HIPCHK(e, hipMemsetAsync(ap.lam, 0, TP * sizeof(float), st));
  if (msl) rc = query_at(K);
  else rc = head_pass(e, st, ap.hscr, ap.fq, ap.yq, n, T, thK, ap.lam, c.loss_out, c.acc_out, c.logits_out, ap.prob + K * pw, ap.dl + K * pw, ap.dfq,
                      with_grad != 0);
  if (rc || !with_grad) return rc;
  HIPCHK(e, hipMemsetAsync(ap.dfs, 0, fsz * sizeof(float), st));
  if (ext) {
    auto adjoint = [&](int k, bool hessian) -> int {
      AnilAdjArgs a{};
      a.lam = ap.lam + hbase; a.lstride = e->PS; a.cstride = ax.hs; a.ph = Ph; a.tasks = T;
      a.alpha = c.lr_vec ? 1.f : inner_lr;
      if (hessian) { a.hv = ap.hv + hbase; a.dfs = ap.dfs; a.rdf = ap.rdf; a.fcount = fsz; }
      if (msl && k == K) a.w = c.step_w + (K - 1);
      else if (msl && k >= 1) { a.w = c.step_w + (k - 1); a.inj = ax.qg + (size_t)(k - 1) * T * ax.hs; }
      if (k >= 1 && ax.dir) { a.lr = lr_of(k - 1); a.dir = ax.dir; }
      if (k >= 1 && ax.prod) { a.g = ap.g + (size_t)(k - 1) * TP + hbase; a.prod = ax.prod + (size_t)(k - 1) * T * ax.hs; }
      if (!a.hv && !a.w && !a.lr && !a.prod) return MI_OK;
      LAUNCH(e, st, OP_MISC, 2, launch_anil_adjoint(st, a));
      return MI_OK;
    };
    rc = adjoint(K, false);
    if (rc) return rc;
    for (int k = K - 1; k >= 0; --k) {
      if (so) {
        HeadArgs ha = head_args(e, ap.hscr, ap.fs, ap.theta + (size_t)k * TP, c.lr_vec ? nullptr : ap.lam, ap.hv, ap.rdf, n, T);
        if (c.lr_vec) { ha.wld = ax.dir; ha.bld = ax.dir + hb; ha.vstride = ax.hs; }
        ha.prob = ap.prob + k * pw; ha.dl = ap.dl + k * pw;
        HEAD_LDS(e, "head tangent", n, ha.ways, 1);
        LAUNCH(e, st, OP_HEAD_TAN, 0, launch_head_tangent(st, ha, T));
        rc = adjoint(k, true);
      } else if (msl && k >= 1) {
        rc = adjoint(k, false);
      }
      if (rc) return rc;
    }
  } else if (c.second_order) {
    for (int k = K - 1; k >= 0; --k) {
      HIPCHK(e, hipMemsetAsync(ap.hv, 0, TP * sizeof(float), st));
      HeadArgs ha = head_args(e, ap.hscr, ap.fs, ap.theta + (size_t)k * TP, ap.lam, ap.hv, ap.rdf, n, T);
      ha.prob = ap.prob + k * pw; ha.dl = ap.dl + k * pw;
      HEAD_LDS(e, "head tangent", n, ha.ways, 1);
      LAUNCH(e, st, OP_HEAD_TAN, 0, launch_head_tangent(st, ha, T));
      LAUNCH(e, st, OP_MISC, 2, launch_axpy(st, ap.dfs, ap.rdf, inner_lr, fsz, ap.dfs));
      LAUNCH(e, st, OP_MISC, 2, launch_axpy(st, ap.lam, ap.hv, inner_lr, TP, ap.lam));
    }
  }
  LAUNCH(e, st, OP_MISC, 4, launch_interleave_rows(st, ap.dfs, ap.dfq, T, n, e->feat, ap.act.dp[nl - 1]));
  rc = trunk_backward(e, st, ap.scratch, ap.act, ap.x, 2 * n, T, ap.theta, ap.lam, gram);
  if (rc) return rc;
  LAUNCH(e, st, OP_MISC, 3, launch_scatter_sum(st, ap.lam, e->perm_dev, (int)e->P, (int)e->PS, T, c.meta_grad_out));
  if (c.lr_vec && c.lr_grad_out)
    LAUNCH(e, st, OP_MISC, 3, launch_anil_lr_fold(st, ax.prod, ax.hs, ap.g + hbase, ap.lam + hbase, e->PS, hperm, hbase, Ph, T, K, c.lr_steps,
                                                  c.lr_grad_out));
  return MI_OK;
}

static GraphKey graph_key(const mi_engine* e, void* stream, const MetaCall& c) {
  typedef unsigned long long u;
  unsigned lr_bits;
  memcpy(&lr_bits, &c.inner_lr, sizeof lr_bits);
  return GraphKey{(u)c.algo, (u)(uintptr_t)stream, (u)(uintptr_t)c.theta, (u)(uintptr_t)c.data, (u)(uintptr_t)c.labels, (u)c.tasks,
                  (u)c.grad_tasks, (u)c.ways, (u)c.shots, (u)c.adapt_steps, (u)c.second_order, (u)lr_bits, (u)(uintptr_t)c.lr_vec,
                  (u)c.lr_steps, (u)(uintptr_t)c.lr_grad_out, (u)(uintptr_t)c.loss_out, (u)(uintptr_t)c.acc_out,
                  (u)(uintptr_t)c.meta_grad_out, (u)(uintptr_t)c.logits_out, (u)(uintptr_t)c.workspace, (u)c.workspace_bytes,
                  (u)e->fuse1, (u)e->gram1, (u)e->gramq, (u)e->overlap, (u)e->fuse_fin, (u)e->fuse_b1red, (u)e->fuse_tail, (u)e->fuse_last,
                  kernel_selection_key(), (u)(uintptr_t)c.step_w};
}

static int meta_batch_entry(mi_engine* e, void* stream, const MetaCall& c) {
  const int crc = check_call(e, c);
  if (crc) return crc;
  const auto fn = is_anil(c.algo) ? meta_batch_anil_impl : meta_batch_maml_impl;
  if (!e->graph_on || e->prof_on || e->trace || e->bn_export || !stream)
    return fn(e, stream, c);
  const GraphKey key = graph_key(e, stream, c);
  mi_engine::GraphEntry* ent = nullptr;
  for (auto& g : e->graphs)
    if (g.key == key) { ent = &g; break; }
  hipStream_t st = reinterpret_cast<hipStream_t>(stream);
  if (ent && ent->exec) {
    HIPCHK(e, hipGraphLaunch(ent->exec, st));
    return MI_OK;
  }
  if (!ent) {
    if (e->graphs.size() >= 8) {
      if (e->graphs.front().exec) (void)hipGraphExecDestroy(e->graphs.front().exec);
      if (e->graphs.front().graph) (void)hipGraphDestroy(e->graphs.front().graph);
      e->graphs.erase(e->graphs.begin());
    }
    e->graphs.push_back(mi_engine::GraphEntry{});
    e->graphs.back().key = key;
    e->graphs.back().seen = 1;
    return fn(e, stream, c);
  }
  HIPCHK(e, hipStreamBeginCapture(st, hipStreamCaptureModeThreadLocal));
  const int rc = fn(e, stream, c);
  hipGraph_t graph = nullptr;
  const hipError_t ce = hipStreamEndCapture(st, &graph);
  if (rc != MI_OK || ce != hipSuccess || !graph) {
    if (graph) (void)hipGraphDestroy(graph);
    e->graph_on = false;
    return rc != MI_OK ? rc : fail(e, MI_ERR_HIP, std::string("graph capture failed: ") + hipGetErrorString(ce));
  }
  hipGraphExec_t exec = nullptr;
  if (hipGraphInstantiate(&exec, graph, nullptr, nullptr, 0) != hipSuccess) {
    (void)hipGraphDestroy(graph);
    e->graph_on = false;
    return fail(e, MI_ERR_HIP, "hipGraphInstantiate failed");
  }
  ent->graph = graph;
  ent->exec = exec;
  HIPCHK(e, hipGraphLaunch(exec, st));
  return MI_OK;
}

extern "C" int mi_meta_batch_maml(mi_engine* e, void* stream, const float* theta, const float* data, const int64_t* labels,
                                  int tasks, int ways, int shots, int adapt_steps, float inner_lr, int second_order,
                                  int with_grad, float* loss_out, float* acc_out, float* meta_grad_out, float* logits_out,
                                  void* workspace, size_t workspace_bytes) {
  return meta_batch_entry(e, stream, MetaCall{ALGO_MAML, theta, data, labels, tasks, with_grad ? tasks : 0, ways, shots, adapt_steps,
                                              second_order, inner_lr, nullptr, 0, nullptr, loss_out, acc_out, meta_grad_out, logits_out,
                                              workspace, workspace_bytes});
}
extern "C" int mi_meta_batch_maml_tv(mi_engine* e, void* stream, const float* theta, const float* data, const int64_t* labels,
                                     int tasks, int grad_tasks, int ways, int shots, int adapt_steps, float inner_lr, int second_order,
                                     float* loss_out, float* acc_out, float* meta_grad_out, float* logits_out,
                                     void* workspace, size_t workspace_bytes) {
  return meta_batch_entry(e, stream, MetaCall{ALGO_MAML, theta, data, labels, tasks, grad_tasks, ways, shots, adapt_steps, second_order,
                                              inner_lr, nullptr, 0, nullptr, loss_out, acc_out, meta_grad_out, logits_out, workspace,
                                              workspace_bytes});
}
extern "C" int mi_meta_batch_maml_lr(mi_engine* e, void* stream, const float* theta, const float* data, const int64_t* labels, int tasks,
                                     int grad_tasks, int ways, int shots, int adapt_steps, const float* lr_vec, int lr_steps,
                                     int second_order, float* loss_out, float* acc_out, float* meta_grad_out, float* lr_grad_out,
                                     float* logits_out, void* workspace, size_t workspace_bytes) {
  return meta_batch_entry(e, stream, MetaCall{ALGO_MAML_LR, theta, data, labels, tasks, grad_tasks, ways, shots, adapt_steps, second_order,
                                              0.f, lr_vec, lr_steps, lr_grad_out, loss_out, acc_out, meta_grad_out, logits_out, workspace,
                                              workspace_bytes});
}
extern "C" int mi_meta_batch_maml_steps(mi_engine* e, void* stream, const float* theta, const float* data, const int64_t* labels, int tasks,
                                        int grad_tasks, int ways, int shots, int adapt_steps, float inner_lr, const float* lr_vec, int lr_steps,
                                        const float* step_w, int second_order, float* loss_steps_out, float* acc_steps_out, float* meta_grad_out,
                                        float* lr_grad_out, float* logits_steps_out, void* workspace, size_t workspace_bytes) {
  MetaCall c{ALGO_MAML_STEPS, theta, data, labels, tasks, grad_tasks, ways, shots, adapt_steps, second_order, lr_vec ? 0.f : inner_lr, lr_vec,
             lr_vec ? lr_steps : 0, lr_grad_out, loss_steps_out, acc_steps_out, meta_grad_out, logits_steps_out, workspace, workspace_bytes};
  c.step_w = step_w;
  return meta_batch_entry(e, stream, c);
}
extern "C" int mi_meta_batch_anil(mi_engine* e, void* stream, const float* theta, const float* data, const int64_t* labels,
                                  int tasks, int ways, int shots, int adapt_steps, float inner_lr, int second_order,
                                  int with_grad, float* loss_out, float* acc_out, float* meta_grad_out, float* logits_out,
                                  void* workspace, size_t workspace_bytes) {
  return meta_batch_entry(e, stream, MetaCall{ALGO_ANIL, theta, data, labels, tasks, with_grad ? tasks : 0, ways, shots, adapt_steps,
                                              second_order, inner_lr, nullptr, 0, nullptr, loss_out, acc_out, meta_grad_out, logits_out,
                                              workspace, workspace_bytes});
}

extern "C" int mi_meta_batch_anil_lr(mi_engine* e, void* stream, const float* theta, const float* data, const int64_t* labels, int tasks,
                                     int ways, int shots, int adapt_steps, const float* lr_vec, int lr_steps, int second_order, int with_grad,
                                     float* loss_out, float* acc_out, float* meta_grad_out, float* lr_grad_out, float* logits_out,
                                     void* workspace, size_t workspace_bytes) {
  return meta_batch_entry(e, stream, MetaCall{ALGO_ANIL_LR, theta, data, labels, tasks, with_grad ? tasks : 0, ways, shots, adapt_steps,
                                              second_order, 0.f, lr_vec, lr_steps, lr_grad_out, loss_out, acc_out, meta_grad_out, logits_out,
                                              workspace, workspace_bytes});
}
extern "C" int mi_meta_batch_anil_steps(mi_engine* e, void* stream, const float* theta, const float* data, const int64_t* labels, int tasks,
                                        int ways, int shots, int adapt_steps, float inner_lr, const float* lr_vec, int lr_steps,
                                        const float* step_w, int second_order, int with_grad, float* loss_steps_out, float* acc_steps_out,
                                        float* meta_grad_out, float* lr_grad_out, float* logits_steps_out, void* workspace,
                                        size_t workspace_bytes) {
  MetaCall c{ALGO_ANIL_STEPS, theta, data, labels, tasks, with_grad ? tasks : 0, ways, shots, adapt_steps, second_order, lr_vec ? 0.f : inner_lr,
             lr_vec, lr_vec ? lr_steps : 0, lr_grad_out, loss_steps_out, acc_steps_out, meta_grad_out, logits_steps_out, workspace,
             workspace_bytes};
  c.step_w = step_w;
  return meta_batch_entry(e, stream, c);
}

extern "C" int mi_forward_logits(mi_engine* e, void* stream, const float* theta, const float* x, int tasks, int n,
                                 float* logits_out, void* workspace, size_t workspace_bytes) {
  return mi_learner_forward(e, stream, theta, 1, x, tasks, n, logits_out, 0, nullptr, workspace, workspace_bytes);
}

extern "C" int mi_forward_workspace_bytes(const mi_engine* e, int tasks, int n, size_t* bytes) {
  if (!e || !bytes || tasks < 1 || n < 1) return MI_ERR_ARG;
  return plan_bytes(e, forward_shape(tasks, n), bytes);
}

static int learner_begin(mi_engine* e, hipStream_t st, const float* theta, int theta_tasks, const float* x, int tasks, int n, const char* bad,
                         void* workspace, size_t workspace_bytes, const PlanShape& s, Plan& pl, float* Plan::*ximg) {
  if (!e) return fail(nullptr, MI_ERR_ARG, "null engine");
  if (!theta || !x || !workspace || tasks < 1 || n < 1) return fail(e, MI_ERR_ARG, "bad learner arguments");
  if (theta_tasks != 1 && theta_tasks != tasks) return fail(e, MI_ERR_ARG, "theta_tasks must be 1 (shared) or == tasks");
  if (bad) return fail(e, MI_ERR_ARG, bad);
  int rc = plan_in(e, workspace, workspace_bytes, s, pl);
  if (rc) return rc;
  rc = plan_begin(e, st, pl);
  if (rc) return rc;
  LAUNCH(e, st, OP_MISC, 0, launch_nchw_to_nhwc(st, x, (size_t)tasks * n, e->d.in_channels, e->d.in_h, e->d.in_w, pl.*ximg));
  LAUNCH(e, st, OP_MISC, 1, launch_gather_params(st, theta, theta_tasks == 1 ? 0 : e->P, e->perm_dev, (int)e->P, (int)e->PS, tasks, pl.theta));
  return MI_OK;
}
static int learner_scatter(mi_engine* e, hipStream_t st, const float* g, int theta_tasks, int tasks, float* out) {
  if (theta_tasks == 1) {
    LAUNCH(e, st, OP_MISC, 3, launch_scatter_sum(st, g, e->perm_dev, (int)e->P, (int)e->PS, tasks, out));
  } else {
    LAUNCH(e, st, OP_MISC, 3, launch_scatter_tasks(st, g, e->perm_dev, (int)e->P, (int)e->PS, tasks, out));
  }
  return MI_OK;
}

static int learner_fwd_bwd(mi_engine* e, hipStream_t st, Plan& pl, ActSet& A, const float* x, const float* dlogits, int n, int tasks, float* g) {
  const int nl = (int)e->L.size();
  int rc = trunk_forward(e, st, pl, A, x, n, tasks, pl.theta);
  if (rc) return rc;
  if (e->d.head_mean_pool) HIPCHK(e, launch_spatial_mean(st, A.p[nl - 1], A.f, tasks * n, e->head_hw, e->head_c));
  HIPCHK(e, hipMemsetAsync(g, 0, (size_t)tasks * e->PS * sizeof(float), st));
  HeadArgs ha = head_args(e, nullptr, A.f, pl.theta, nullptr, g, A.df, n, tasks);
  ha.dl = const_cast<float*>(dlogits);
  HEAD_LDS(e, "head backward", n, ha.ways, 0);
// ... 412 lines not shown
```

### exploring_meta_amd/csrc/kernels.h

```cpp
#pragma once
#include "mi_common.h"
#include "finalize.h"

struct ConvArgs {
  const float* in[2];
  const float* wt[2];
  size_t wstride;
  float* out;
  const float* z;
  const float* mu;
  const float* rstd;
  double* partial;
  FinArgs fin;
  const float *bp, *bzh, *bzhd, *bdp;
  const uint8_t* barg;
  ConvGeom g;
  int mpix;
  int ntiles, tiles_per_wave;
  int split_bf16;
  int stagger;
  const unsigned* amax[2];
};

struct WgradArgs {
  const float* x[2];
  const float* dz[2];
  float* partial;
  ConvGeom g;
  int mpix, chunk_pix, nchunks, nterms;
  const unsigned* amax_x[2]; const unsigned* amax_dz[2];
  int form;
};

struct BnArgs {
  const float* z;
  const float* zd;
  const float* mu;
  const float* rstd;
  const float* m1;
  const float* m2;
  const float* gamma; const float* beta; size_t pstride;
  const float* gammad; const float* betad; size_t vstride;
  const float* dgamma; const float* dbeta; size_t gstride;
  const float* rdgamma; const float* rdbeta; size_t hstride;
  const float* dp;
  const float* dpd;
  float* out;
  unsigned* amax_out;
  float* zh_out;
  double* partial;
  FinArgs fin;
  int n, ho, wo, c;
  float inv_m;
};


struct PoolRedArgs {
  const float* p;
  const float* zh;
  const float* zhd;
  const float* dp;
  const float* dpd;
  double* partial;
  int rows, c;
  FinArgs fin;
};
int pooled_reduce_blocks(int rows, int c, int tasks);
hipError_t launch_pooled_reduce(hipStream_t st, const PoolRedArgs& a, int tasks, int tangent, int* nblk);

int conv_operand_form();
int conv_b16();
int block1_split_form();
int sparse_wgrad_split_form();
hipError_t launch_conv3x3(hipStream_t st, ConvArgs a, int tasks, int nterms, int epi, int mode, int* blocks_per_task);
hipError_t launch_wgrad3x3(hipStream_t st, WgradArgs a, int tasks, int nterms, int* nchunks_out);
hipError_t launch_wgrad_reduce(hipStream_t st, const float* partial, int nchunks, int nelem, int tasks, float* out, size_t ostride);
size_t wgrad_partial_floats(const ConvGeom& g, int tasks);
int conv_max_blocks_per_task(const ConvGeom& g);
int conv_tiles_per_wave(int mpix, int tasks, int cot);
enum { WG_FAM_FIRST = 0, WG_FAM_CHUNKED = 1, WG_FAM_ROWS_F32 = 2, WG_FAM_ROWS_BF16 = 3, WG_FAM_STRIPS_BF16 = 4 };
struct WgradPlan {
  int family;
  int size;
  int exact;
  int per_block;
  int blocks;
  int per_term;
  int form;
  int nchunks;
  int strip_cand;
};
WgradPlan wgrad_plan(const ConvGeom& g, int tasks, int nterms, bool have_scales);
enum { CONV_K_FIRST = 0, CONV_K_GENERIC = 1, CONV_K_S1_F32 = 2, CONV_K_S1_BF16_32X32 = 3, CONV_K_S1_BF16_16X16 = 4, CONV_K_S1_F16 = 5 };
struct ConvPlan { int kernel, tiles_per_wave, ntiles, blocks, tile_pix, waves, form, stats64; };
ConvPlan conv_plan(const ConvGeom& g, int tasks, int nterms, int epi, int mode, bool have_scales);

int bn_blocks_per_task(int n, int ho, int wo, int c, int pool, int tasks);
hipError_t launch_bn_finalize(hipStream_t st, const double* partial, int nblk, int tasks, int c, double inv_m, int mode,
                              float* out0, size_t stride0, float* out1, size_t stride1);
hipError_t launch_bn_fwd(hipStream_t st, const BnArgs& a, int tasks, int pool);
hipError_t launch_bn_bwd_reduce(hipStream_t st, const BnArgs& a, int tasks, int pool, int* nblk);
hipError_t launch_bn_bwd_apply(hipStream_t st, const BnArgs& a, int tasks, int pool);
hipError_t launch_bn_tan_fwd(hipStream_t st, const BnArgs& a, int tasks, int pool);
hipError_t launch_bn_tan_bwd_reduce(hipStream_t st, const BnArgs& a, int tasks, int pool, int* nblk);
hipError_t launch_bn_tan_bwd_apply(hipStream_t st, const BnArgs& a, int tasks, int pool);

struct B1Args {
  const float* x;
  const float* w; const float* wd;
  size_t wstride, vstride;
  const float *mu, *rstd, *m1, *m2;
  const float *gamma, *beta; size_t pstride;
  const float *gammad, *betad;
  const float *dgamma, *dbeta; size_t gstride;
  const float *rdgamma, *rdbeta; size_t hstride;
  const float* dp; const float* dpd;
  float* out;
  unsigned* amax_out;
  float* zh_out;
  uint8_t* arg_out;
  const uint8_t* arg_in; const float* zh_in;
  double* partial;
  FinArgs fin;
  float* wpartial;
  int n, hh, ww, co;
  float inv_m;
  int ntiles, tiles_per_wave;
  int fwd_fp32;
};
enum { B1_STATS = 0, B1_FWD = 1, B1_BWD_REDUCE = 2, B1_BWD_WGRAD = 3, B1_TSTATS = 4, B1_TFWD = 5, B1_TBWD_REDUCE = 6, B1_TBWD_WGRAD = 7,
       B1_TFWD_ARG = 8, B1_FORCE_GENERAL = 0x100 };
bool block1_supported(int ci, int stride, int pool, int h, int w, int co);
int block1_blocks_per_task(int n, int h, int w, int co, int tasks);
hipError_t launch_block1(hipStream_t st, B1Args a, int tasks, int ci, int mode, int* blocks_per_task);

struct SparseWgArgs {
  const float* x;
  const uint8_t* arg;
  const float* dp; const float* dpd;
  const float *mu_unused, *rstd, *m2;
  const float* gamma; size_t pstride;
  const float* gammad; size_t vstride;
  float* wpartial;
  int n, hh, ww, co;
  int ntiles, tiles_per_wave, row_pitch;
};
bool sparse_wgrad_supported(int w, int ci, int co);
int sparse_wgrad_blocks_per_task(int n, int h, int w, int co, int tasks);
hipError_t launch_sparse_wgrad(hipStream_t st, SparseWgArgs a, int tasks, int ci, int tangent, int* blocks_per_task);
struct GramWgArgs {
  const double* g;
  const float* spartial; int nblk;
  const float* w; size_t wstride; const float* wd; size_t vstride;
  const float *mu, *rstd, *m1, *m2;
  const float* gamma; size_t pstride; const float* gammad;
  const float *dgamma, *dbeta; size_t gstride;
  const float *rdgamma, *rdbeta; size_t hstride;
  float* out; size_t ostride;
  int ci, co; double inv_m;
};
hipError_t launch_gram_wgrad(hipStream_t st, const GramWgArgs& a, int tasks, int tangent);

struct AdvanceSeg { unsigned off, nelem; const float* partial; int nchunks; };
struct AdvanceArgs {
  float* g; size_t gstride;
  AdvanceSeg seg[8]; int nseg;
  unsigned zoff[10], zlen[10]; int nzero;
  const float* a; float* out; size_t ostride; float alpha;
  unsigned n;
  int b1_wgrad, gw_tangent; GramWgArgs gw;
  unsigned off_w1;
  int stats;
  const double* gram; int ci, co;
  const float* sw; size_t swstride;
  const float *mu_in, *rstd_in;
  float *out0, *out1; double inv_m;
  unsigned* counter;
  const float* lr;
  const float* dlr; float* dir;
  const float* dg; float* prod;
  const float* inj_w;
  const float* inj;
};
hipError_t launch_advance(hipStream_t st, const AdvanceArgs& a, int tasks);

int gram_blocks_per_task(int n, int h);
size_t gram_partial_doubles(int tasks, int n, int h, int ci);
size_t gram_doubles(int tasks, int ci);
bool gram_supported(int w, int ci);
hipError_t launch_input_gram(hipStream_t st, const float* x, int tasks, int n, int h, int w, int ci, double* partial, double* g);
hipError_t launch_gram_stats(hipStream_t st, const double* g, int tasks, int ci, int co, const float* w, size_t wstride,
                             const float* wd, size_t vstride, double inv_m, int tangent, float* out0, float* out1,
                             const float* mu, const float* rstd);

struct HeadArgs {
  const float* f;
  const float* fd;
  const float* wl; const float* bl; size_t pstride;
  const float* wld; const float* bld; size_t vstride;
  const int32_t* y;
  float* loss; float* acc;
  float* logits;
// ... 100 lines not shown
```

### exploring_meta_amd/engine.py

```python

import ctypes as C
from dataclasses import dataclass

import torch

from . import _lib


@dataclass(frozen=True)
class ModelSpec:
    n_layers: int
    in_channels: int
    in_h: int
    in_w: int
    hidden: int
    max_pool: bool
    ways: int
    head_mean_pool: bool

    @staticmethod
    def mini_imagenet(ways, hidden=32, layers=4):
        return ModelSpec(layers, 3, 84, 84, hidden, True, ways, False)

    @staticmethod
    def omniglot(ways, hidden=64, layers=4):
        return ModelSpec(layers, 1, 28, 28, hidden, False, ways, True)

    @staticmethod
    def anil(ways, hidden=64, channels=3, max_pool=True, layers=4, in_hw=84):
        return ModelSpec(layers, channels, in_hw, in_hw, hidden, bool(max_pool), ways, False)

    def block_output_shape(self, layer):
        if not 1 <= layer <= self.n_layers:
            raise ValueError(f'layer must be in 1..{self.n_layers}')
        h, w = self.in_h, self.in_w
        for _ in range(layer):
            if self.max_pool:
                h, w = h // 2, w // 2
            else:
                h, w = (h - 1) // 2 + 1, (w - 1) // 2 + 1
        return self.hidden, h, w

    def param_shapes(self):
        out, ci = [], self.in_channels
        for i in range(self.n_layers):
            out += [(f'base.{i}.normalize.weight', (self.hidden,)), (f'base.{i}.normalize.bias', (self.hidden,)),
                    (f'base.{i}.conv.weight', (self.hidden, ci, 3, 3)), (f'base.{i}.conv.bias', (self.hidden,))]
            ci = self.hidden
        h, w = self.in_h, self.in_w
        for _ in range(self.n_layers):
            if self.max_pool:
                h, w = h // 2, w // 2
            else:
                h, w = (h - 1) // 2 + 1, (w - 1) // 2 + 1
        feat = self.hidden if self.head_mean_pool else self.hidden * h * w
        out += [('linear.weight', (self.ways, feat)), ('linear.bias', (self.ways,))]
        return out


def _ptr(t):
    return C.c_void_p(t.data_ptr()) if t is not None else C.c_void_p(0)


def _stream(device=None):
    return C.c_void_p(torch.cuda.current_stream(device).cuda_stream)


def _on_device(fn):
    import functools

    @functools.wraps(fn)
    def wrapped(self, *args, **kwargs):
        with torch.cuda.device(self.device):
            return fn(self, *args, **kwargs)
    return wrapped


def _resolve_device(device):
    if device is None:
        return torch.device('cuda', torch.cuda.current_device())
    device = torch.device(device)
    if device.type != 'cuda':
        raise _lib.MiError(f'the engine runs on a GPU, got device {device}')
    return torch.device('cuda', device.index if device.index is not None else torch.cuda.current_device())


class MetaEngine:

    def __init__(self, spec, device=None):
        self.lib = _lib.load()
        if not torch.cuda.is_available():
            raise _lib.MiError('MetaEngine needs a GPU: the MAML hot path has no CPU implementation in this package '
                               '(the CPU restatement under oracle/ is test infrastructure only).')
        self.spec = spec
        self.device = _resolve_device(device)
        desc = _lib.MiModelDesc(spec.n_layers, spec.in_channels, spec.in_h, spec.in_w, spec.hidden, int(spec.max_pool),
                                spec.ways, int(spec.head_mean_pool))
        self._h = C.c_void_p()
        _lib.check(self.lib.mi_engine_create(C.byref(desc), self.device.index, C.byref(self._h)))
        n = C.c_size_t()
        _lib.check(self.lib.mi_param_count(self._h, C.byref(n)), self._h)
        self.param_count = n.value
        self._ws = None

    def __del__(self):
        h = getattr(self, '_h', None)
        if h is not None and h.value:
            self.lib.mi_engine_destroy(h)
            self._h = C.c_void_p()

    def set_fused_block1(self, on):
        _lib.check(self.lib.mi_engine_set_fused_block1(self._h, int(on)), self._h)

    def set_overlap(self, on):
        _lib.check(self.lib.mi_engine_set_overlap(self._h, int(on)), self._h)

    def set_fused_finalize(self, on):
        _lib.check(self.lib.mi_engine_set_fused_finalize(self._h, int(on)), self._h)

    def set_fused_block1_reduce(self, on):
        _lib.check(self.lib.mi_engine_set_fused_block1_reduce(self._h, int(on)), self._h)

    def set_fused_tail(self, on):
        _lib.check(self.lib.mi_engine_set_fused_tail(self._h, int(on)), self._h)

    def set_fused_last_block(self, on):
        _lib.check(self.lib.mi_engine_set_fused_last_block(self._h, int(on)), self._h)

    def set_graph(self, on):
        _lib.check(self.lib.mi_engine_set_graph(self._h, int(on)), self._h)
        self._graph = bool(on)
        self._persist = {}
        self._gstream = torch.cuda.Stream(device=self.device) if on else None

    def _fused_call(self, fn, *args):
        gs = getattr(self, '_gstream', None)
        if gs is None:
            return fn(self._h, _stream(self.device), *args)
        cur = torch.cuda.current_stream(self.device)
        gs.wait_stream(cur)
        rc = fn(self._h, C.c_void_p(gs.cuda_stream), *args)
        cur.wait_stream(gs)
        return rc

    def _persistent(self, key, make):
        if not getattr(self, '_graph', False):
            return make()
        if key not in self._persist:
            self._persist[key] = make()
        return self._persist[key]

    def _outputs(self, kind, T, nlog, with_grad, return_logits):
        def fresh():
            P = self.param_count if with_grad else 0
            buf = torch.empty(P + 2 * T, dtype=torch.float32, device=self.device)
            return (buf[P:P + T], buf[P + T:], buf[:P] if with_grad else None,
                    torch.empty(T, nlog, self.spec.ways, dtype=torch.float32, device=self.device) if return_logits else None)
        return self._persistent((kind, T, nlog, bool(with_grad), bool(return_logits)), fresh)

    def set_bn_export(self, tasks=0, passes=0):
        if not tasks:
            _lib.check(self.lib.mi_engine_set_bn_export(self._h, C.c_void_p(0), 0), self._h)
            self._bn_export = None
            return None
        ctot = self.spec.hidden * self.spec.n_layers
        self._bn_export = torch.zeros(passes, tasks, 2, ctot, dtype=torch.float32, device=self.device)
        _lib.check(self.lib.mi_engine_set_bn_export(self._h, _ptr(self._bn_export), self._bn_export.numel()), self._h)
        return self._bn_export

    def set_trace(self, tasks=0, adapt_steps=0):
        if not tasks:
            _lib.check(self.lib.mi_debug_set_trace(self._h, None, 0), self._h)
            self._trace = None
            return None
        K, T, P = adapt_steps, tasks, self.param_count
        buf = torch.zeros((4 * K + 1) * T * P, dtype=torch.float32, device=self.device)
        _lib.check(self.lib.mi_debug_set_trace(self._h, _ptr(buf), buf.numel()), self._h)
        self._trace = buf
        v = buf.view(4 * K + 1, T, P)
        return dict(theta=v[:K + 1], g=v[K + 1:2 * K + 1], lam_in=v[2 * K + 1:3 * K + 1], hv=v[3 * K + 1:])

    def workspace_bytes(self, tasks, shots, adapt_steps, second_order):
        b = C.c_size_t()
        _lib.check(self.lib.mi_workspace_bytes(self._h, tasks, self.spec.ways, shots, adapt_steps, int(second_order),
                                               C.byref(b)), self._h)
        return b.value

    def _workspace(self, nbytes):
        if self._ws is None or self._ws.numel() < nbytes:
            self._ws = None
            self._ws = torch.empty(nbytes, dtype=torch.uint8, device=self.device)
        return self._ws

    def _check_batch(self, theta, data, labels, shots, lr_vec=None, flat_data=True):
        s = self.spec
        T = data.shape[0]
        n2 = 2 * shots * s.ways
        if tuple(data.shape) != (T, n2, s.in_channels, s.in_h, s.in_w) and \
                not (flat_data and s.in_channels == 1 and data.numel() == T * n2 * s.in_h * s.in_w):
            raise ValueError(f'data shape {tuple(data.shape)} does not match [T, {n2}, {s.in_channels}, {s.in_h}, {s.in_w}]')
        if tuple(labels.shape) != (T, n2):
            raise ValueError(f'labels shape {tuple(labels.shape)} != {(T, n2)}')
        if theta.numel() != self.param_count:
            raise ValueError(f'theta has {theta.numel()} elements, the model has {self.param_count}')
        for t, dt in ((theta, torch.float32), (data, torch.float32), (labels, torch.int64)) + (((lr_vec, torch.float32),) if lr_vec is not None else ()):
            if t.dtype != dt or not t.is_cuda or not t.is_contiguous():
                raise ValueError('theta/data/lr_vec must be contiguous fp32 CUDA tensors and labels contiguous int64 CUDA')
        return T

    def _maml_call(self, theta, data, labels, shots, adapt_steps, inner_lr, lr_vec, first_order, grad_tasks, want_lr_grad, return_logits,
                   step_w=None):
        s = self.spec
        T = self._check_batch(theta, data, labels, shots, lr_vec)
        if step_w is not None:
            if adapt_steps < 1:
                raise _lib.MiError('libmi_maml error -1: meta_batch_steps needs adapt_steps >= 1')
            if not torch.is_tensor(step_w) or step_w.dtype != torch.float32 or not step_w.is_cuda or step_w.device != theta.device or \
                    not step_w.is_contiguous() or tuple(step_w.shape) != (adapt_steps,):
                raise _lib.MiError(f'libmi_maml error -1: step_w must be a contiguous fp32 tensor of shape ({adapt_steps},) on {theta.device}')
        if lr_vec is not None:
            if lr_vec.numel() % self.param_count != 0 or lr_vec.numel() == 0 or lr_vec.dim() > 2 or \
                    (lr_vec.dim() == 2 and lr_vec.shape[1] != self.param_count):
                raise _lib.MiError(f'libmi_maml error -1: lr_vec has shape {tuple(lr_vec.shape)}, expected [P], [1, P] or [adapt_steps, P] '
                                   f'with P = {self.param_count}')
            lr_steps = lr_vec.numel() // self.param_count
        if not 0 <= grad_tasks <= T:
            raise ValueError(f'grad_tasks must be in 0..{T}, got {grad_tasks}')
        with_grad = grad_tasks > 0
        so = (not first_order) and with_grad
        b = C.c_size_t(0 if lr_vec is not None or step_w is not None else self.workspace_bytes(T, shots, adapt_steps, so))
        if step_w is not None:
            if self.lib.mi_workspace_bytes_steps(self._h, T, int(grad_tasks), s.ways, shots, adapt_steps, int(so),
                                                 lr_steps if lr_vec is not None else 0, int(bool(want_lr_grad)), C.byref(b)):
                raise _lib.MiError(f'libmi_maml error -1: lr_steps must be 1 or adapt_steps = {adapt_steps}')
        elif lr_vec is not None and self.lib.mi_workspace_bytes_lr(self._h, T, s.ways, shots, adapt_steps, int(so), lr_steps,
                                                                 int(bool(want_lr_grad)), C.byref(b)):
            raise _lib.MiError(f'libmi_maml error -1: lr_steps = {lr_steps} must be 1 or adapt_steps = {adapt_steps}')
        ws = self._workspace(b.value)
        if step_w is not None:
            return self._steps_call(theta, data, labels, shots, adapt_steps, inner_lr, lr_vec, first_order, grad_tasks, want_lr_grad,
                                    return_logits, step_w, T, ws)
        loss, acc, grad, logits = self._outputs('maml' if lr_vec is None else 'maml_lr', T, shots * s.ways, with_grad, return_logits)
        head = (_ptr(theta), _ptr(data), _ptr(labels), T, int(grad_tasks), s.ways, shots, adapt_steps)
        tail = (_ptr(logits), _ptr(ws), ws.numel())
        lr_grad = None
        if lr_vec is None:
            rc = self._fused_call(self.lib.mi_meta_batch_maml_tv, *head, float(inner_lr), int(not first_order), _ptr(loss), _ptr(acc), _ptr(grad),
                                  *tail)
        else:
            if want_lr_grad:
                lr_grad = self._persistent(('lr_grad', T, lr_steps),
                                           lambda: torch.empty(lr_steps, self.param_count, dtype=torch.float32, device=self.device))
            rc = self._fused_call(self.lib.mi_meta_batch_maml_lr, *head, _ptr(lr_vec), lr_steps, int(not first_order), _ptr(loss), _ptr(acc),
                                  _ptr(grad), _ptr(lr_grad), *tail)
        _lib.check(rc, self._h)
        return loss, acc, grad, lr_grad, logits

    def _steps_call(self, theta, data, labels, shots, adapt_steps, inner_lr, lr_vec, first_order, grad_tasks, want_lr_grad, return_logits,
                    step_w, T, ws):
        s, K1 = self.spec, adapt_steps + 1
        with_grad = grad_tasks > 0
        lr_steps = 0 if lr_vec is None else lr_vec.numel() // self.param_count

        def fresh():
            return (torch.empty(K1, T, dtype=torch.float32, device=self.device), torch.empty(K1, T, dtype=torch.float32, device=self.device),
                    torch.empty(self.param_count, dtype=torch.float32, device=self.device) if with_grad else None,
                    torch.empty(K1, T, shots * s.ways, s.ways, dtype=torch.float32, device=self.device) if return_logits else None)
        loss, acc, grad, logits = self._persistent(('steps', lr_vec is None, K1, T, shots * s.ways, with_grad, bool(return_logits)), fresh)
        lr_grad = None
        if lr_vec is not None and want_lr_grad:
            lr_grad = self._persistent(('lr_grad_steps', T, lr_steps),
                                       lambda: torch.empty(lr_steps, self.param_count, dtype=torch.float32, device=self.device))
        rc = self._fused_call(self.lib.mi_meta_batch_maml_steps, _ptr(theta), _ptr(data), _ptr(labels), T, int(grad_tasks), s.ways, shots,
                              adapt_steps, float(inner_lr) if lr_vec is None else 0.0, _ptr(lr_vec), lr_steps, _ptr(step_w),
                              int(not first_order), _ptr(loss), _ptr(acc), _ptr(grad), _ptr(lr_grad), _ptr(logits), _ptr(ws), ws.numel())
        _lib.check(rc, self._h)
        return loss, acc, grad, lr_grad, logits

    @_on_device
    def meta_batch_steps(self, theta, data, labels, shots, adapt_steps, step_w, inner_lr=None, lr_vec=None, first_order=False, grad_tasks=None,
# ... 585 lines not shown
```

### exploring_meta_amd/utils/roofline.py

```python

PEAK_TFLOPS = 157.3
PEAK_GBPS = 8000.0
BF16_PEAK_TFLOPS = 2500.0
SPLIT_BF16_PEAK_TFLOPS = BF16_PEAK_TFLOPS / 6.0
SPLIT_F16_PEAK_TFLOPS = BF16_PEAK_TFLOPS / 3.0
SPLIT_BF16_OPS = ('conv_fwd_stats', 'dgrad', 'tangent_conv_fwd', 'tangent_dgrad')
SPLIT_BF16_WGRAD_OPS = ('wgrad', 'tangent_wgrad')


def mfma_peak(spec, op, layer, form=1):
    h, w, ci, co, ho, wo, _, _ = layer_geometry(spec)[layer]
    same = ci == co and (h, w) == (ho, wo)
    form = int(form)
    split = (SPLIT_F16_PEAK_TFLOPS, 'fp16 x3 (two scaled planes)') if form == 2 else (SPLIT_BF16_PEAK_TFLOPS, 'bf16 x6 (split operands)')
    if form and same and ci == 32 and (op in SPLIT_BF16_OPS or (op in SPLIT_BF16_WGRAD_OPS and w >= 16)):
        return split
    if form and same and ci == 64 and (op in ('conv_fwd_stats', 'dgrad') or (op in SPLIT_BF16_WGRAD_OPS and w >= 16)):
        return split
    if form and layer == 0 and ci == 3 and op in ('bn_relu_pool_fwd', 'bn_tangent_fwd'):
        return BF16_PEAK_TFLOPS / 8.0, 'bf16 x8 (split operands)'
    if form and layer == 0 and op in SPLIT_BF16_WGRAD_OPS and ci == 3 and w == 84:
        return SPLIT_BF16_PEAK_TFLOPS, 'bf16 x6 (split operands)'
    return PEAK_TFLOPS, 'fp32'


def layer_geometry(spec):
    out, h, w, ci = [], spec.in_h, spec.in_w, spec.in_channels
    for _ in range(spec.n_layers):
        s = 1 if spec.max_pool else 2
        ho, wo = (h - 1) // s + 1, (w - 1) // s + 1
        hp, wp = (ho // 2, wo // 2) if spec.max_pool else (ho, wo)
        out.append((h, w, ci, spec.hidden, ho, wo, hp, wp))
        h, w, ci = hp, wp, spec.hidden
    return out


def fused_block1(spec):
    return spec.max_pool and spec.in_channels in (1, 3) and spec.in_h % 2 == 0 and spec.in_w % 2 == 0 and spec.in_w // 2 >= 8


def op_costs(spec, op, layer, images):
    h, w, ci, co, ho, wo, hp, wp = layer_geometry(spec)[layer]
    x, z, p = h * w * ci * 4, ho * wo * co * 4, hp * wp * co * 4
    f = 2 * 9 * ci * co * ho * wo
    if layer == 0 and fused_block1(spec):
        a = p // 4
        t = {'conv_fwd_stats': (f, x), 'bn_relu_pool_fwd': (f, x + 2 * p + a), 'bn_bwd_reduce': (0, 3 * p), 'wgrad': (f, x + p + a),
             'tangent_conv_fwd': (2 * f, x), 'bn_tangent_fwd': (f, x + 3 * p + a), 'bn_tangent_bwd_reduce': (0, 5 * p),
             'tangent_wgrad': (f, x + 2 * p + a)}
    else:
        rides = spec.max_pool and layer >= 1
        ridden = spec.max_pool and layer + 1 < spec.n_layers
        pb = x // 4 if (layer == 1 and fused_block1(spec)) else x
        t = {'conv_fwd_stats': (f, x + z), 'dgrad': (f, z + x + (x + pb if rides else 0)), 'wgrad': (f, x + z),
             'tangent_conv_fwd': (2 * f, 2 * x + 2 * z), 'tangent_dgrad': (2 * f, 2 * z + x + (3 * x + pb if rides else 0)),
             'tangent_wgrad': (2 * f, 2 * x + 2 * z),
             'bn_relu_pool_fwd': (0, z + p + (p if ridden else 0)), 'bn_bwd_reduce': (0, z + p), 'bn_bwd_apply': (0, 2 * z + p),
             'bn_tangent_fwd': (0, 2 * z + p + (p if ridden else 0)), 'bn_tangent_bwd_reduce': (0, 2 * z + 2 * p),
             'bn_tangent_bwd_apply': (0, 3 * z + 2 * p)}
        if layer == 0:
            t['tangent_conv_fwd'] = (f, x + 2 * z)
            t['tangent_wgrad'] = (f, x + z)
    if op not in t:
        return None
    fl, by = t[op]
    return fl * images, by * images


def bound_of(flops, nbytes, peak_tflops=PEAK_TFLOPS):
    if not flops:
        return 'hbm'
    return 'mfma' if flops / nbytes > peak_tflops * 1e12 / (PEAK_GBPS * 1e9) else 'hbm'


KERNEL_NAMES = {
    'conv_fwd_stats': 'conv3x3_s1_mfma_kernel<{ci},1,EPI_STATS,fwd>', 'dgrad': 'conv3x3_s1_mfma_kernel<{ci},1,EPI_BRED,dgrad>',
    'wgrad': 'wgrad3x3_rows_mfma_kernel (1 term)', 'tangent_conv_fwd': 'conv3x3_s1_mfma_kernel<{ci},2,EPI_TSTATS,fwd>',
    'tangent_dgrad': 'conv3x3_s1_mfma_kernel<{ci},2,EPI_BRED,dgrad>', 'tangent_wgrad': 'wgrad3x3_rows_mfma_kernel (2 terms)',
    'bn_relu_pool_fwd': 'bn_fwd_kernel', 'bn_bwd_reduce': 'bn_bwd_reduce_kernel', 'bn_bwd_apply': 'bn_bwd_apply_kernel',
    'bn_tangent_fwd': 'bn_tan_fwd_kernel', 'bn_tangent_bwd_reduce': 'bn_tan_bwd_reduce_kernel',
    'bn_tangent_bwd_apply': 'bn_tan_bwd_apply_kernel',
}
BLOCK1_KERNEL_NAMES = {
    'bn_relu_pool_fwd': 'block1_fwd_kernel<{ci},FWD>', 'bn_tangent_fwd': 'block1_fwd_kernel<{ci},TFWD_ARG>', 'wgrad': 'sparse_wgrad_rows_kernel<{ci},false>',
    'tangent_wgrad': 'sparse_wgrad_rows_kernel<{ci},true>', 'bn_bwd_reduce': 'pooled_reduce_kernel<false>',
    'bn_tangent_bwd_reduce': 'pooled_reduce_kernel<true>', 'conv_fwd_stats': 'block1_kernel<{ci},STATS>',
}


def conv_kernel_is_b16(mpix, tasks, co, mode, min_tpw=6):
    if mode == 2:
        return True
    if mode != 1:
        return False
    tiles = -(-mpix // 30) * tasks * max(1, co // 32)
    return -(-tiles // 2048) >= min_tpw


def kernel_name(spec, op, layer, b16=False):
    ci = layer_geometry(spec)[layer][2]
    names = BLOCK1_KERNEL_NAMES if (layer == 0 and fused_block1(spec)) else KERNEL_NAMES
    name = names.get(op, op).format(ci=ci)
    if b16 and name.startswith('conv3x3_s1_mfma_kernel'):
        name = name.replace('conv3x3_s1_mfma_kernel', 'conv3x3_s1_b16_kernel')
    return name
```

### include/mi_maml.h

```cpp
#ifndef MI_MAML_H
#define MI_MAML_H

#include <stddef.h>
#include <stdint.h>

#ifdef __cplusplus
extern "C" {
#endif

#define MI_OK 0
#define MI_ERR_ARG (-1)
#define MI_ERR_HIP (-2)
#define MI_ERR_WORKSPACE (-3)

typedef struct mi_engine mi_engine;

typedef struct {
  int32_t n_layers;
  int32_t in_channels, in_h, in_w;
  int32_t hidden;
  int32_t max_pool;
  int32_t ways;
  int32_t head_mean_pool;
} mi_model_desc;

int mi_engine_create(const mi_model_desc* desc, int device, mi_engine** out);
void mi_engine_destroy(mi_engine* e);
const char* mi_last_error(const mi_engine* e);
const char* mi_version(void);

int mi_engine_set_fused_block1(mi_engine* e, int on);

int mi_engine_set_overlap(mi_engine* e, int on);

int mi_engine_set_graph(mi_engine* e, int on);

int mi_engine_set_bn_export(mi_engine* e, float* buf, size_t floats);

int mi_engine_set_fused_finalize(mi_engine* e, int on);

int mi_engine_set_fused_block1_reduce(mi_engine* e, int on);

int mi_debug_plan_offsets(const mi_engine* e, int tasks, int ways, int shots, int adapt_steps, int second_order, size_t* out);

int mi_param_count(const mi_engine* e, size_t* n);

int mi_workspace_bytes(const mi_engine* e, int tasks, int ways, int shots, int adapt_steps, int second_order, size_t* bytes);

int mi_meta_batch_maml(mi_engine* e, void* stream, const float* theta, const float* data, const int64_t* labels,
                       int tasks, int ways, int shots, int adapt_steps, float inner_lr, int second_order, int with_grad,
                       float* loss_out, float* acc_out, float* meta_grad_out, float* logits_out,
                       void* workspace, size_t workspace_bytes);

int mi_meta_batch_maml_tv(mi_engine* e, void* stream, const float* theta, const float* data, const int64_t* labels,
                          int tasks, int grad_tasks, int ways, int shots, int adapt_steps, float inner_lr, int second_order,
                          float* loss_out, float* acc_out, float* meta_grad_out, float* logits_out,
                          void* workspace, size_t workspace_bytes);

int mi_workspace_bytes_lr(const mi_engine* e, int tasks, int ways, int shots, int adapt_steps, int second_order, int lr_steps,
                          int want_lr_grad, size_t* bytes);
int mi_meta_batch_maml_lr(mi_engine* e, void* stream, const float* theta, const float* data, const int64_t* labels,
                          int tasks, int grad_tasks, int ways, int shots, int adapt_steps, const float* lr_vec, int lr_steps,
                          int second_order, float* loss_out, float* acc_out, float* meta_grad_out, float* lr_grad_out,
                          float* logits_out, void* workspace, size_t workspace_bytes);

int mi_workspace_bytes_steps(const mi_engine* e, int tasks, int grad_tasks, int ways, int shots, int adapt_steps, int second_order,
                             int lr_steps, int want_lr_grad, size_t* bytes);
int mi_meta_batch_maml_steps(mi_engine* e, void* stream, const float* theta, const float* data, const int64_t* labels, int tasks,
                             int grad_tasks, int ways, int shots, int adapt_steps, float inner_lr, const float* lr_vec, int lr_steps,
                             const float* step_w, int second_order, float* loss_steps_out, float* acc_steps_out, float* meta_grad_out,
                             float* lr_grad_out, float* logits_steps_out, void* workspace, size_t workspace_bytes);

int mi_engine_set_fused_tail(mi_engine* e, int on);

int mi_engine_set_fused_last_block(mi_engine* e, int on);
int mi_debug_tail_stamps(mi_engine* e, unsigned long long* buf);

int mi_anil_workspace_bytes(const mi_engine* e, int tasks, int ways, int shots, int adapt_steps, size_t* bytes);
int mi_meta_batch_anil(mi_engine* e, void* stream, const float* theta, const float* data, const int64_t* labels,
                       int tasks, int ways, int shots, int adapt_steps, float inner_lr, int second_order, int with_grad,
                       float* loss_out, float* acc_out, float* meta_grad_out, float* logits_out,
                       void* workspace, size_t workspace_bytes);

int mi_anil_workspace_bytes_steps(const mi_engine* e, int tasks, int ways, int shots, int adapt_steps, int with_grad, int second_order,
                                  int lr_steps, int want_lr_grad, int step_outputs, size_t* bytes);
int mi_meta_batch_anil_lr(mi_engine* e, void* stream, const float* theta, const float* data, const int64_t* labels, int tasks,
                          int ways, int shots, int adapt_steps, const float* lr_vec, int lr_steps, int second_order, int with_grad,
                          float* loss_out, float* acc_out, float* meta_grad_out, float* lr_grad_out, float* logits_out,
                          void* workspace, size_t workspace_bytes);
int mi_meta_batch_anil_steps(mi_engine* e, void* stream, const float* theta, const float* data, const int64_t* labels, int tasks,
                             int ways, int shots, int adapt_steps, float inner_lr, const float* lr_vec, int lr_steps, const float* step_w,
                             int second_order, int with_grad, float* loss_steps_out, float* acc_steps_out, float* meta_grad_out,
                             float* lr_grad_out, float* logits_steps_out, void* workspace, size_t workspace_bytes);

int mi_forward_workspace_bytes(const mi_engine* e, int tasks, int n, size_t* bytes);
int mi_forward_logits(mi_engine* e, void* stream, const float* theta, const float* x, int tasks, int n, float* logits_out,
                      void* workspace, size_t workspace_bytes);

int mi_learner_forward(mi_engine* e, void* stream, const float* theta, int theta_tasks, const float* x, int tasks, int n,
                       float* logits_out, int rep_layer, float* rep_out, void* workspace, size_t workspace_bytes);
int mi_learner_backward(mi_engine* e, void* stream, const float* theta, int theta_tasks, const float* x, const float* dlogits,
                        int tasks, int n, float* grad_out, void* workspace, size_t workspace_bytes);

int mi_learner_hvp_workspace_bytes(const mi_engine* e, int tasks, int n, size_t* bytes);
int mi_learner_hvp(mi_engine* e, void* stream, const float* theta, int theta_tasks, const float* x, const float* dlogits,
                   const float* v, int tasks, int n, float* grad_theta_out, float* logits_dot_out, void* workspace,
                   size_t workspace_bytes);

int mi_cg_update(void* stream, double* x, double* r, double* p, const float* ap, double* rr, float* p32, size_t n, double eps);
int mi_cg_update_checked(void* stream, double* x, double* r, double* p, const float* ap, double* rr, float* p32, size_t n, double eps,
                         double tol);

int mi_cg_init(void* stream, const float* b, double* x, double* r, double* p, float* p32, double* rr, size_t n);

int mi_trpo_scale_step(void* stream, const float* step, const float* fstep, size_t n, float max_kl, float* out, float* lagrange_out);

int mi_gae_max_rows(int state_dim);
int mi_gae_advantages(void* stream, const float* states, const float* next_states, const float* rewards, const float* dones,
                      const int32_t* count, const double* weight_in, int replays, int rows, int state_dim, double gamma, double tau,
                      double reg, int normalize, float* adv_out, double* weight_out);

int mi_copy_segments(void* stream, const void* const* src, void* const* dst, const uint32_t* nfloat, const uint32_t* npad, int nseg);
int mi_upload_i32(void* stream, int32_t* dst, const int32_t* host_values, int n);

int mi_adam_step(void* stream, float* theta, const float* grad, float* exp_avg, float* exp_avg_sq, size_t n, int step,
                 float lr, float beta1, float beta2, float eps, float grad_scale);


int mi_prepare_batch(void* stream, const float* data, const int64_t* labels, int tasks, int n2, int c, int h, int w,
                     float* xs, float* xq, int32_t* ys, int32_t* yq);

size_t mi_input_gram_scratch_bytes(int tasks, int n, int h, int ci);
int mi_input_gram(void* stream, const float* x, int tasks, int n, int h, int w, int ci, void* scratch, size_t scratch_bytes,
                  double* g_out);
int mi_gram_bn_stats(void* stream, const double* g, int tasks, int ci, int co, const float* w9, size_t pstride, const float* w9d,
                     size_t vstride, int pixels, float* out0, float* out1, const float* mu, const float* rstd);

size_t mi_cka_scratch_bytes(int pairs, int n, int p);
int mi_cka(void* stream, const float* x, const float* y, int pairs, int n, int p, double sigma,
           void* scratch, size_t scratch_bytes, double* out);

size_t mi_cca_scratch_bytes(int pairs, int n, int p);
int mi_cca(void* stream, const float* x, const float* y, int pairs, int n, int p, double epsilon, double threshold,
           void* scratch, size_t scratch_bytes, double* coefs, double* stats);

int mi_stream_copy(void* stream, const void* src, void* dst, size_t bytes);

int mi_sample_tasks(void* stream, const void* dataset, int dataset_is_u8, size_t num_images, int c, int h, int w,
                    const int64_t* index, const uint8_t* rot, int tasks, int n2, float* data_out);

int mi_draw_tasks(void* stream, const int32_t* class_offsets, const int32_t* class_index, int n_classes, int ways, int k,
                  const uint8_t* rot_table, int n_rot, int remap_shuffle, uint64_t seed, uint64_t first_slot, uint64_t num_tasks,
                  int tasks, int64_t* index_out, int64_t* labels_out, uint8_t* rot_out, uint64_t* task_id_out);

int mi_conv3x3_bn_stats(void* stream, const float* x, const float* w9, size_t pstride, int tasks, int n, int h, int wd,
                        int ci, int co, int stride, float* z, float* mu, float* rstd, void* scratch, size_t scratch_bytes);
int mi_bn_relu_pool(void* stream, const float* z, const float* mu, const float* rstd, const float* gamma, const float* beta,
                    size_t pstride, int tasks, int n, int ho, int wo, int c, int pool, float* p);
int mi_bn_relu_pool_bwd(void* stream, const float* z, const float* mu, const float* rstd, const float* gamma, const float* beta,
                        size_t pstride, const float* dp, int tasks, int n, int ho, int wo, int c, int pool,
                        float* dgamma, float* dbeta, size_t gstride, float* dz, void* scratch, size_t scratch_bytes);
int mi_conv3x3_bwd(void* stream, const float* x, const float* dz, const float* w9, size_t pstride, int tasks, int n, int h,
                   int wd, int ci, int co, int stride, float* dx, float* dw9, size_t gstride, void* scratch, size_t scratch_bytes);
int mi_head_fwd_bwd(void* stream, const float* f, const float* wl, const float* bl, size_t pstride, const int32_t* y,
                    int tasks, int n, int feat, int ways, float* loss, float* acc, float* logits, float* prob, float* dl,
                    float* dwl, float* dbl, size_t gstride, float* df);
size_t mi_kernel_scratch_bytes(int tasks, int n, int h, int w, int c);
int mi_head_grads(void* stream, const float* f, const float* wl, size_t pstride, const float* dl, int tasks, int n, int feat,
                  int ways, float* dwl, float* dbl, size_t gstride, float* df);
int mi_head_tangent(void* stream, const float* f, const float* fd, const float* wl, const float* bl, size_t pstride,
                    const float* wld, const float* bld, size_t vstride, const float* prob, const float* dl, float* rdl,
                    float* ld_out, int fixed_dl, int tasks, int n, int feat, int ways, float* dwl, float* dbl, size_t gstride,
                    float* df);
int mi_spatial_mean(void* stream, const float* p, float* f, int rows, int hw, int c);
int mi_spatial_mean_bwd(void* stream, const float* df, float* dp, int rows, int hw, int c);

typedef struct {
  const float *z, *zd;
  const float *mu, *rstd, *m1, *m2;
  const float *gamma, *beta, *wl, *bl; size_t pstride;
  const float *gammad, *betad, *wld, *bld; size_t vstride;
  const int32_t* y;
  const float *f, *dp;
  float *prob, *dl;
  float *pooled;
  float *loss, *acc, *logits;
  float *dwl, *dbl, *sum0, *sum1; size_t gstride;
  float *df;
  int32_t tasks, n, ho, wo, c, pool, ways;
  int32_t with_grad, bwd_tasks;
} mi_tail_args;
int mi_tail_supported(int n, int ho, int wo, int c, int pool, int feat, int ways);
size_t mi_tail_lds_bytes(int n, int feat, int ways, int tangent);
size_t mi_tail_scratch_bytes(int tasks, int n, int ho, int wo, int c, int pool, int ways);
int mi_tail_run(void* stream, const mi_tail_args* a, int tangent, void* scratch, size_t scratch_bytes);


int mi_conv3x3_tangent(void* stream, const float* x0, const float* w0, const float* x1, const float* w1, size_t pstride,
                       const float* z, const float* mu, const float* rstd, int tasks, int n, int h, int wd, int ci, int co,
                       int stride, float* zd, float* m1, float* m2, void* scratch, size_t scratch_bytes);
int mi_conv3x3_bwd2(void* stream, const float* x0, const float* dz0, const float* x1, const float* dz1, const float* w0,
                    const float* w1, size_t pstride, int tasks, int n, int h, int wd, int ci, int co, int stride, float* dx,
                    float* dw9, size_t gstride, void* scratch, size_t scratch_bytes);

typedef struct {
  const float *z, *zd;
  const float *mu, *rstd, *m1, *m2;
  const float *gamma, *beta; size_t pstride;
  const float *gammad, *betad; size_t vstride;
  const float *dgamma, *dbeta; size_t gstride;
  const float *dp, *dpd;
  int32_t tasks, n, ho, wo, c, pool;
} mi_bn_tangent_args;
int mi_bn_tangent_fwd(void* stream, const mi_bn_tangent_args* a, float* pd);
int mi_bn_tangent_bwd(void* stream, const mi_bn_tangent_args* a, float* rdgamma, float* rdbeta, size_t hstride, float* rdz,
                      void* scratch, size_t scratch_bytes);

#define MI_B1_STATS 0
#define MI_B1_FWD 1
#define MI_B1_BWD_REDUCE 2
#define MI_B1_BWD_WGRAD 3
#define MI_B1_TSTATS 4
#define MI_B1_TFWD 5
#define MI_B1_TBWD_REDUCE 6
#define MI_B1_TBWD_WGRAD 7
#define MI_B1_TFWD_ARG 8
typedef struct {
  const float* x;
  const float *w, *wd;
  const float *gamma, *beta; size_t pstride;
  const float *gammad, *betad; size_t vstride;
  const float *mu, *rstd, *m1, *m2;
  const float *dgamma, *dbeta; size_t gstride;
  const float *rdgamma, *rdbeta; size_t hstride;
  const float *dp, *dpd;
  const uint8_t* arg_in; const float* zh_in;
  int32_t tasks, n, h, w_, ci, co;
} mi_block1_args;
size_t mi_block1_scratch_bytes(int tasks, int n, int h, int w, int ci, int co);
int mi_block1_run(void* stream, int mode, const mi_block1_args* a, float* p_out, float* zh_out, uint8_t* arg_out, float* out0,
                  float* out1, size_t ostride, void* scratch, size_t scratch_bytes);
int mi_pooled_reduce(void* stream, const float* p, const float* zh, const float* zhd, const float* dp, const float* dpd,
                     int tasks, int rows, int c, float* out0, float* out1, size_t ostride, void* scratch, size_t scratch_bytes);
int mi_block1_wgrad_gram(void* stream, const mi_block1_args* a, const double* g, int tangent, float* dw, size_t ostride,
                         void* scratch, size_t scratch_bytes);

int mi_debug_conv_tiles_per_wave(int tasks, int n, int ho, int wo, int co);
int mi_debug_wgrad_plan(int tasks, int n, int h, int w, int ci, int co, int stride, int nterms, int* out);
int mi_debug_conv_plan(int tasks, int n, int h, int w, int ci, int co, int stride, int nterms, int epi, int mode, int* out);
int mi_debug_set_trace(mi_engine* e, float* buf, size_t floats);

int mi_profile_enable(mi_engine* e, int on, int kind_filter);
int mi_profile_kinds(void);
const char* mi_profile_op_name(int op);
int mi_profile_collect(mi_engine* e, double* total_ms, int64_t* count, int n_kinds);

typedef struct mi_policy mi_policy;
typedef struct {
  int32_t state_size, action_size, hidden1, hidden2;
  int32_t activation;
} mi_policy_desc;

int mi_policy_create(const mi_policy_desc* desc, int device, mi_policy** out);
void mi_policy_destroy(mi_policy* p);
const char* mi_policy_last_error(const mi_policy* p);
int mi_policy_param_count(const mi_policy* p, size_t* n);

int mi_policy_forward(mi_policy* p, void* stream, const float* theta, size_t tstride, const float* states, int tasks, int batch,
                      float* loc_out, void* workspace, size_t workspace_bytes);

size_t mi_particles_rollout_scratch_bytes(const mi_policy* p, int tasks, int episodes, int max_path_length);
int mi_particles_rollout(mi_policy* p, void* stream, const float* theta, size_t tstride, const float* goals,
                         const uint64_t* rollout_ids, uint64_t seed, int tasks, int episodes, int max_path_length,
                         float* states, float* actions, float* next_states, float* rewards, float* dones,
                         int32_t* count, int32_t* ep_len, float* noise_out, void* scratch, size_t scratch_bytes);
int mi_policy_adapt(mi_policy* p, void* stream, const float* theta, size_t tstride, const float* states, const float* actions,
                    const float* adv, const int32_t* count, int tasks, int batch, float lr, int head_only, float* theta_out,
                    float* loss_out, void* workspace, size_t workspace_bytes);
int mi_policy_set_fused_fvp(int on);
int mi_policy_learner_workspace_bytes(const mi_policy* p, int tasks, int batch, size_t* bytes);
int mi_policy_vjp(mi_policy* p, void* stream, const float* theta, size_t tstride, const float* states, const float* dloc,
                  const int32_t* count, int tasks, int batch, int head_only, float* grad_out, void* workspace, size_t workspace_bytes);
int mi_policy_hvp(mi_policy* p, void* stream, const float* theta, size_t tstride, const float* states, const float* dloc, const float* v,
                  const int32_t* count, int tasks, int batch, int head_only, float* grad_theta_out, float* loc_dot_out, void* workspace,
                  size_t workspace_bytes);
int mi_policy_set_fused_learner(int on);
int mi_policy_learner_fused_supported(const mi_policy* p);
int mi_debug_policy_sweep_stamps(void* buf);
int mi_debug_conv_stamps(void* buf);
int mi_conv_set_split_bf16(int on);
int mi_conv_get_split_bf16(unsigned* mask_out);
int mi_conv_set_b16(int on);
int mi_block1_set_split_bf16(int on);
int mi_sparse_wgrad_set_split_bf16(int on);


#define MI_PLOSS_A2C 0
#define MI_PLOSS_PPO 1
#define MI_PLOSS_DICE 2
int mi_policy_meta_workspace_bytes(const mi_policy* p, int tasks, int batch, int steps, int n_batches, int second_order,
                                   size_t* bytes);
int mi_policy_meta_batch(mi_policy* p, void* stream, const float* theta, int steps, const int32_t* step_batch,
                         const int32_t* step_new_old, int n_batches, const float* s_states, const float* s_actions,
                         const float* s_adv, const int32_t* s_count, const float* q_states, const float* q_actions,
                         const float* q_adv, const int32_t* q_count, int tasks, int batch, int loss_kind, float clip,
                         float inner_lr, int head_only, int second_order, int with_grad, float* loss_out, float* theta_out,
                         float* grad_out, void* workspace, size_t workspace_bytes);
int mi_policy_meta_batch_dones(mi_policy* p, void* stream, const float* theta, int steps, const int32_t* step_batch,
                               const int32_t* step_new_old, int n_batches, const float* s_states, const float* s_actions,
                               const float* s_adv, const int32_t* s_count, const float* s_done, const float* q_states,
                               const float* q_actions, const float* q_adv, const int32_t* q_count, const float* q_done, int tasks,
                               int batch, int loss_kind, float clip, float inner_lr, int head_only, int second_order,
                               int with_grad, float* loss_out, float* theta_out, float* grad_out, void* workspace,
                               size_t workspace_bytes);

int mi_policy_update_workspace_bytes(const mi_policy* p, int tasks, int batch, size_t* bytes);
int mi_policy_update(mi_policy* p, void* stream, const float* theta, size_t tstride, const float* states, const float* actions,
                     const float* adv, const int32_t* count, const float* done, int tasks, int batch, int loss_kind, int epochs,
                     float clip, float lr, int head_only, float* theta_out, float* loss_out, void* workspace, size_t workspace_bytes);

int mi_policy_meta_lr_workspace_bytes(const mi_policy* p, int tasks, int batch, int steps, int n_batches, int second_order, int lr_rows,
                                      int want_lr_grad, size_t* bytes);
int mi_policy_meta_batch_lr(mi_policy* p, void* stream, const float* theta, int steps, const int32_t* step_batch,
                            const int32_t* step_new_old, const int32_t* step_lr_row, int n_batches, const float* s_states,
                            const float* s_actions, const float* s_adv, const int32_t* s_count, const float* s_done,
                            const float* q_states, const float* q_actions, const float* q_adv, const int32_t* q_count,
                            const float* q_done, int tasks, int batch, int loss_kind, float clip, const float* lr_vec, int lr_rows,
                            int head_only, int second_order, int with_grad, float* loss_out, float* theta_out, float* grad_out,
                            float* lr_grad_out, void* workspace, size_t workspace_bytes);
int mi_policy_update_lr(mi_policy* p, void* stream, const float* theta, size_t tstride, const float* states, const float* actions,
                        const float* adv, const int32_t* count, const float* done, int tasks, int batch, int loss_kind, int epochs,
                        float clip, const float* lr_vec, int head_only, float* theta_out, float* loss_out, void* workspace,
                        size_t workspace_bytes);

int mi_trpo_steps_workspace_bytes(const mi_policy* p, int tasks, int batch, int steps, size_t* bytes);
int mi_trpo_surrogate_steps(mi_policy* p, void* stream, const float* theta, int steps, const float* s_states,
                            const float* s_actions, const float* s_adv, const int32_t* s_count, const float* q_states,
                            const float* q_actions, const float* q_adv, const int32_t* q_count, const float* old_loc,
                            const float* old_scale, int tasks, int batch, float inner_lr, float* loss_out, float* kl_out,
                            float* grad_out, void* workspace, size_t workspace_bytes);
int mi_trpo_fvp_steps(mi_policy* p, void* stream, int steps, const float* s_states, const float* s_actions, const int32_t* s_count,
                      const float* q_states, const int32_t* q_count, int tasks, int batch, float inner_lr, float damping,
                      const float* v, float* out, void* workspace, size_t workspace_bytes);

int mi_trpo_general_steps_workspace_bytes(const mi_policy* p, int tasks, int batch, int steps, size_t* bytes);
int mi_trpo_kl_prepare_steps(mi_policy* p, void* stream, int steps, const float* s_states, const float* s_actions,
                             const int32_t* s_count, const float* q_states, const int32_t* q_count, const float* old_loc,
                             const float* old_scale, int tasks, int batch, float inner_lr, float* kl_grad_out, void* workspace,
                             size_t workspace_bytes);
int mi_trpo_fvp_general_steps(mi_policy* p, void* stream, int steps, const float* s_states, const float* s_actions,
                              const int32_t* s_count, const float* q_states, const int32_t* q_count, const float* old_scale,
                              int tasks, int batch, float inner_lr, float damping, const float* v, float* out, void* workspace,
                              size_t workspace_bytes);

int mi_policy_adapt_lr(mi_policy* p, void* stream, const float* theta, size_t tstride, const float* states, const float* actions,
                       const float* adv, const int32_t* count, int tasks, int batch, const float* lr_vec, int head_only,
                       float* theta_out, float* loss_out, void* workspace, size_t workspace_bytes);
int mi_trpo_steps_lr_workspace_bytes(const mi_policy* p, int tasks, int batch, int steps, int lr_rows, size_t* bytes);
int mi_trpo_surrogate_steps_lr(mi_policy* p, void* stream, const float* theta, int steps, const float* s_states,
                               const float* s_actions, const float* s_adv, const int32_t* s_count, const float* q_states,
                               const float* q_actions, const float* q_adv, const int32_t* q_count, const float* old_loc,
                               const float* old_scale, int tasks, int batch, const float* lr_vec, int lr_rows,
                               const int32_t* step_lr_row, float* loss_out, float* kl_out, float* grad_out, void* workspace,
                               size_t workspace_bytes);
int mi_trpo_fvp_steps_lr(mi_policy* p, void* stream, int steps, const float* s_states, const float* s_actions, const int32_t* s_count,
                         const float* q_states, const int32_t* q_count, int tasks, int batch, const float* lr_vec, int lr_rows,
                         const int32_t* step_lr_row, float damping, const float* v, float* out, void* workspace, size_t workspace_bytes);
int mi_trpo_general_steps_lr_workspace_bytes(const mi_policy* p, int tasks, int batch, int steps, int lr_rows, size_t* bytes);
int mi_trpo_kl_prepare_steps_lr(mi_policy* p, void* stream, int steps, const float* s_states, const float* s_actions,
// ... 13 lines not shown
```

Baseline: 1921.

## Store max-pool argmax decisions in forward and reuse them in tangent BN pass

The BN+ReLU+maxpool forward kernel now optionally writes a packed byte per channel that records the winning pool position and the ReLU-off flag. The tangent forward pass reads these decisions and the stored normalized values instead of re-reading z and re-scanning each window, and the dgrad reduce epilogue also consumes the stored decisions. This lowers tangent-pass memory traffic for second-order adaptation. In exchange it adds a separately allocated decision buffer, an extra write in the primal pass and a larger graph key.

```diff
diff --git a/exploring_meta_amd/_lib.py b/exploring_meta_amd/_lib.py
--- a/exploring_meta_amd/_lib.py
+++ b/exploring_meta_amd/_lib.py
@@ -93,6 +93,7 @@
                                            C.c_void_p, C.c_void_p, C.c_void_p, C.c_size_t]),
     'mi_engine_set_fused_tail': (C.c_int, [C.c_void_p, C.c_int]),
     'mi_engine_set_fused_last_block': (C.c_int, [C.c_void_p, C.c_int]),
+    'mi_engine_set_stored_decisions': (C.c_int, [C.c_void_p, C.c_int]),
     'mi_debug_tail_stamps': (C.c_int, [C.c_void_p, C.c_void_p]),
     'mi_anil_workspace_bytes': (C.c_int, [C.c_void_p, C.c_int, C.c_int, C.c_int, C.c_int, C.POINTER(C.c_size_t)]),
     'mi_meta_batch_anil': (C.c_int, [C.c_void_p, C.c_void_p, C.c_void_p, C.c_void_p, C.c_void_p, C.c_int, C.c_int, C.c_int,
@@ -171,6 +172,11 @@
     'mi_bn_tangent_fwd': (C.c_int, [C.c_void_p, C.POINTER(MiBnTangentArgs), C.c_void_p]),
     'mi_bn_tangent_bwd': (C.c_int, [C.c_void_p, C.POINTER(MiBnTangentArgs), C.c_void_p, C.c_void_p, C.c_size_t, C.c_void_p,
                                     C.c_void_p, C.c_size_t]),
+    'mi_conv3x3_dgrad_bred': (C.c_int, [C.c_void_p] * 5 + [C.c_size_t] + [C.c_void_p] * 5 + [C.c_int] * 5 + [C.c_void_p] * 3 +
+                              [C.c_size_t, C.c_void_p, C.c_size_t]),
+    'mi_amax_cell_words': (C.c_size_t, []),
+    'mi_bn_stored_fwd': (C.c_int, [C.c_void_p, C.POINTER(MiBnTangentArgs)] + [C.c_void_p] * 4),
+    'mi_bn_stored_tangent_fwd': (C.c_int, [C.c_void_p, C.POINTER(MiBnTangentArgs)] + [C.c_void_p] * 5),
     'mi_block1_scratch_bytes': (C.c_size_t, [C.c_int] * 6),
     'mi_block1_run': (C.c_int, [C.c_void_p, C.c_int, C.POINTER(MiBlock1Args), C.c_void_p, C.c_void_p, C.c_void_p, C.c_void_p,
                                 C.c_void_p, C.c_size_t, C.c_void_p, C.c_size_t]),
diff --git a/exploring_meta_amd/csrc/bn_pool.hip b/exploring_meta_amd/csrc/bn_pool.hip
--- a/exploring_meta_amd/csrc/bn_pool.hip
+++ b/exploring_meta_amd/csrc/bn_pool.hip
@@ -37,25 +37,33 @@
   mi_finalize_last(a.fin, a.partial + (size_t)task * gridDim.x * 2 * a.c, gridDim.x, a.c, task, gridDim.x, red);
 }
 
-template <int POOL>
-__global__ __launch_bounds__(256) void bn_fwd_kernel(BnArgs a) {
+template <int POOL, bool ARG>
+__device__ __forceinline__ unsigned bn_fwd_body(const BnArgs& a) {
   BN_THREAD_SETUP(POOL)
   float* out_t = a.out + (size_t)task * p_task;
   float* zh_t = a.zh_out ? a.zh_out + (size_t)task * p_task : nullptr;
+  uint8_t* arg_t = ARG ? a.arg_out + (size_t)task * p_task : nullptr;
   unsigned am = 0u;
   Window<POOL> w;
   for (int win = blockIdx.x * wpb + wl; win < it.nwin; win += gridDim.x * wpb) {
     w.locate(a, it, win, c0);
     if (!w.pooled) continue;
     floatx4 umax, zh_at, zd_at;
-    scan_window<POOL, false>(w, z_t, nullptr, k, umax, zh_at, zd_at);
+    unsigned arg[4];
+    scan_window<POOL, false, ARG>(w, z_t, nullptr, k, umax, zh_at, zd_at, arg);
     floatx4 o;
 #pragma unroll
     for (int c = 0; c < 4; ++c) { o[c] = fmaxf(umax[c], 0.f); mi_amax_acc(am, o[c]); }
     *reinterpret_cast<floatx4*>(out_t + w.poff) = o;
     if (zh_t) *reinterpret_cast<floatx4*>(zh_t + w.poff) = zh_at;
-  }
-  if (a.amax_out) mi_amax_commit(am, a.amax_out, task);
+    if (ARG) *reinterpret_cast<unsigned*>(arg_t + w.poff) = pack_decisions(arg, umax);
+  }
+  return am;
+}
+template <int POOL, bool ARG = false>
+__global__ __launch_bounds__(256) void bn_fwd_kernel(BnArgs a) {
+  const unsigned am = bn_fwd_body<POOL, ARG>(a);
+  if (a.amax_out) mi_amax_commit(am, a.amax_out, blockIdx.y);
 }
 
 template <int POOL>
@@ -113,8 +121,8 @@
   if (a.amax_out) mi_amax_commit(am, a.amax_out, task);
 }
 
-template <int POOL>
-__global__ __launch_bounds__(256) void bn_tan_fwd_kernel(BnArgs a) {
+template <int POOL, bool STORED>
+__device__ __forceinline__ unsigned bn_tan_fwd_body(const BnArgs& a) {
   BN_THREAD_SETUP(POOL)
   const float* zd_t = a.zd + (size_t)task * z_task;
   float* out_t = a.out + (size_t)task * p_task;
@@ -129,7 +137,19 @@
     w.locate(a, it, win, c0);
     if (!w.pooled) continue;
     floatx4 umax, zh_at, zd_at;
-    scan_window<POOL, true>(w, z_t, zd_t, k, umax, zh_at, zd_at);
+    if constexpr (STORED) {
+      floatx4 zdv[Window<POOL>::NP];
+#pragma unroll
+      for (int p = 0; p < Window<POOL>::NP; ++p) zdv[p] = *reinterpret_cast<const floatx4*>(zd_t + w.off[p]);
+      zh_at = *reinterpret_cast<const floatx4*>(a.zh_in + (size_t)task * p_task + w.poff);
+      const unsigned dec = *reinterpret_cast<const unsigned*>(a.arg_in + (size_t)task * p_task + w.poff);
+      pick_by_decision<0>(dec, zdv, zd_at, umax);
+      pick_by_decision<1>(dec, zdv, zd_at, umax);
+      pick_by_decision<2>(dec, zdv, zd_at, umax);
+      pick_by_decision<3>(dec, zdv, zd_at, umax);
+    } else {
+      scan_window<POOL, true>(w, z_t, zd_t, k, umax, zh_at, zd_at);
+    }
     floatx4 o, zo;
 #pragma unroll
     for (int c = 0; c < 4; ++c) {
@@ -142,7 +162,12 @@
     *reinterpret_cast<floatx4*>(out_t + w.poff) = o;
     if (a.zh_out) *reinterpret_cast<floatx4*>(a.zh_out + (size_t)task * p_task + w.poff) = zo;
   }
-  if (a.amax_out) mi_amax_commit(am, a.amax_out, task);
+  return am;
+}
+template <int POOL, bool STORED = false>
+__global__ __launch_bounds__(256) void bn_tan_fwd_kernel(BnArgs a) {
+  const unsigned am = bn_tan_fwd_body<POOL, STORED>(a);
+  if (a.amax_out) mi_amax_commit(am, a.amax_out, blockIdx.y);
 }
 
 template <int POOL>
@@ -318,6 +343,11 @@
   else hipLaunchKernelGGL(KERNEL<0>, grid, dim3(256), 0, st, a);
 
 hipError_t launch_bn_fwd(hipStream_t st, const BnArgs& a, int tasks, int pool) {
+  if (pool && a.arg_out) {
+    const int blocks = bn_blocks_per_task(a.n, a.ho, a.wo, a.c, pool, tasks);
+    hipLaunchKernelGGL((bn_fwd_kernel<1, true>), dim3(blocks, tasks), dim3(256), 0, st, a);
+    return hipGetLastError();
+  }
   BN_LAUNCH(bn_fwd_kernel)
   return hipGetLastError();
 }
@@ -331,6 +361,12 @@
   return hipGetLastError();
 }
 hipError_t launch_bn_tan_fwd(hipStream_t st, const BnArgs& a, int tasks, int pool) {
+  if ((a.zh_in == nullptr) != (a.arg_in == nullptr)) return hipErrorInvalidValue;
+  if (pool && a.zh_in) {
+    const int blocks = bn_blocks_per_task(a.n, a.ho, a.wo, a.c, pool, tasks);
+    hipLaunchKernelGGL((bn_tan_fwd_kernel<1, true>), dim3(blocks, tasks), dim3(256), 0, st, a);
+    return hipGetLastError();
+  }
   BN_LAUNCH(bn_tan_fwd_kernel)
   return hipGetLastError();
 }
diff --git a/exploring_meta_amd/csrc/bn_window.h b/exploring_meta_amd/csrc/bn_window.h
--- a/exploring_meta_amd/csrc/bn_window.h
+++ b/exploring_meta_amd/csrc/bn_window.h
@@ -100,9 +100,9 @@
   }
 };
 
-template <int POOL, bool WITH_ZD>
+template <int POOL, bool WITH_ZD, bool WITH_ARG = false>
 __device__ __forceinline__ void scan_values(const floatx4* zv, const floatx4* zdv, const ChanConst& k, floatx4& umax, floatx4& zh_at,
-                                            floatx4& zd_at) {
+                                            floatx4& zd_at, unsigned* arg = nullptr) {
 #pragma unroll
   for (int p = 0; p < Window<POOL>::NP; ++p) {
     const floatx4 z = zv[p];
@@ -114,23 +114,38 @@
       const float u = bn_u(zh, k.g[c], k.b[c]);
       if (p == 0) {
         umax[c] = u; zh_at[c] = zh; zd_at[c] = zd[c];
+        if (WITH_ARG) arg[c] = 0u;
       } else {
         const bool gt = u > umax[c];
         umax[c] = gt ? u : umax[c];
         zh_at[c] = gt ? zh : zh_at[c];
         zd_at[c] = gt ? zd[c] : zd_at[c];
+        if (WITH_ARG) arg[c] = gt ? (unsigned)p : arg[c];
       }
     }
   }
 }
-template <int POOL, bool WITH_ZD>
+template <int POOL, bool WITH_ZD, bool WITH_ARG = false>
 __device__ __forceinline__ void scan_window(const Window<POOL>& w, const float* __restrict__ z_t, const float* __restrict__ zd_t,
-                                            const ChanConst& k, floatx4& umax, floatx4& zh_at, floatx4& zd_at) {
+                                            const ChanConst& k, floatx4& umax, floatx4& zh_at, floatx4& zd_at, unsigned* arg = nullptr) {
   floatx4 zv[Window<POOL>::NP], zdv[Window<POOL>::NP];
 #pragma unroll
   for (int p = 0; p < Window<POOL>::NP; ++p) {
     zv[p] = *reinterpret_cast<const floatx4*>(z_t + w.off[p]);
     if (WITH_ZD) zdv[p] = *reinterpret_cast<const floatx4*>(zd_t + w.off[p]);
   }
-  scan_values<POOL, WITH_ZD>(zv, zdv, k, umax, zh_at, zd_at);
+  scan_values<POOL, WITH_ZD, WITH_ARG>(zv, zdv, k, umax, zh_at, zd_at, arg);
 }
+
+__device__ __forceinline__ unsigned pack_decisions(const unsigned* arg, const floatx4& umax) {
+  unsigned w = 0u;
+#pragma unroll
+  for (int c = 0; c < 4; ++c) w |= (arg[c] | ((umax[c] > 0.f) ? 0u : 4u)) << (8 * c);
+  return w;
+}
+template <int C>
+__device__ __forceinline__ void pick_by_decision(unsigned w, const floatx4* v, floatx4& at, floatx4& on) {
+  const int b0 = lane_mask_bit<8 * C>(w), b1 = lane_mask_bit<8 * C + 1>(w), off = lane_mask_bit<8 * C + 2>(w);
+  at[C] = lane_select(b1, lane_select(b0, v[3][C], v[2][C]), lane_select(b0, v[1][C], v[0][C]));
+  on[C] = lane_select(off, 0.f, 1.f);
+}
diff --git a/exploring_meta_amd/csrc/engine.hip b/exploring_meta_amd/csrc/engine.hip
--- a/exploring_meta_amd/csrc/engine.hip
+++ b/exploring_meta_amd/csrc/engine.hip
@@ -20,7 +20,7 @@
   size_t off_gamma, off_beta, off_w, off_b;
 };
 
-typedef std::array<unsigned long long, 31> GraphKey;
+typedef std::array<unsigned long long, 33> GraphKey;
 struct mi_engine {
   mi_model_desc d;
   int device;
@@ -37,6 +37,9 @@
   bool fuse_b1red = true;
   bool fuse_tail = true;
   bool fuse_last = !(getenv("MI_FUSE_LAST") && atoi(getenv("MI_FUSE_LAST")) == 0);
+  bool stored_dec = true;
+  uint8_t* dec_buf = nullptr;
+  size_t dec_bytes = 0;
   unsigned long long* tail_stamps = nullptr;
   unsigned zoff[10] = {}, zlen[10] = {};
   int nzero = 0;
@@ -210,6 +213,7 @@
   if (!e) return;
   if (e->perm_dev) (void)hipFree(e->perm_dev);
   if (e->counters) (void)hipFree(e->counters);
+  if (e->dec_buf) (void)hipFree(e->dec_buf);
   for (auto& g : e->graphs) {
     if (g.exec) (void)hipGraphExecDestroy(g.exec);
     if (g.graph) (void)hipGraphDestroy(g.graph);
@@ -239,6 +243,12 @@
 extern "C" int mi_engine_set_fused_block1_reduce(mi_engine* e, int on) {
   if (!e) return MI_ERR_ARG;
   e->fuse_b1red = on != 0;
+  return MI_OK;
+}
+
+extern "C" int mi_engine_set_stored_decisions(mi_engine* e, int on) {
+  if (!e) return MI_ERR_ARG;
+  e->stored_dec = on != 0;
   return MI_OK;
 }
 
@@ -334,6 +344,7 @@
 struct ActSet {
   float *z[8], *p[8], *dz[8], *dp[8], *mu[8], *rstd[8];
   float* zhl[8];
+  uint8_t* argl[8];
   float* zhm;
   uint8_t* arg0;
   float *f, *df, *prob, *dl;
@@ -370,13 +381,14 @@
   bool f16 = false;
   std::vector<std::pair<const void*, unsigned*>> cellmap;
   size_t bytes;
+  size_t dec_bytes = 0;
 };
 
-static void plan_actset(const mi_engine* e, Bump& b, ActSet& A, int T, int n, bool with_bwd) {
+static void plan_actset(const mi_engine* e, Bump& b, ActSet& A, int T, int n, bool with_bwd, Bump* dec = nullptr) {
   const int nl = (int)e->L.size();
   A.zhm = nullptr;
   A.arg0 = nullptr;
-  for (int l = 0; l < 8; ++l) A.zhl[l] = nullptr;
+  for (int l = 0; l < 8; ++l) { A.zhl[l] = nullptr; A.argl[l] = nullptr; }
   for (int l = 0; l < nl; ++l) {
     const Layer& L = e->L[l];
     const size_t zs = (size_t)T * n * L.ho * L.wo * L.co, ps = (size_t)T * n * L.hp * L.wp * L.co;
@@ -386,7 +398,9 @@
     A.dz[l] = (with_bwd && !fused) ? b.take<float>(zs) : nullptr;
     A.dp[l] = with_bwd ? b.take<float>(ps) : nullptr;
     if (fused && with_bwd && e->gram1) { A.zhm = b.take<float>(ps); A.arg0 = b.take<uint8_t>(ps); }
-    A.zhl[l] = (!fused && with_bwd && l >= 1 && L.pool && dgrad_carries_reduce(e, l + 1)) ? b.take<float>(ps) : nullptr;
+    const bool keeps_zh = !fused && with_bwd && l >= 1 && L.pool && dgrad_carries_reduce(e, l + 1);
+    A.zhl[l] = keeps_zh ? b.take<float>(ps) : nullptr;
+    A.argl[l] = (keeps_zh && dec && e->stored_dec) ? dec->take<uint8_t>(ps) : nullptr;
     A.mu[l] = b.take<float>((size_t)T * L.co);
     A.rstd[l] = b.take<float>((size_t)T * L.co);
   }
@@ -487,7 +501,9 @@
   pl.tail_scr = b.take<float>(tail_scr_floats(T, nmax, e->d.ways));
   const int nsets = (second_order && K > 0) ? K : 1;
   pl.sup.resize(nsets);
-  for (int k = 0; k < nsets; ++k) plan_actset(e, b, pl.sup[k], T, ns, true);
+  Bump db{ws && e->dec_bytes ? reinterpret_cast<char*>(e->dec_buf) : nullptr, 0};
+  for (int k = 0; k < nsets; ++k) plan_actset(e, b, pl.sup[k], T, ns, true, (second_order && K > 0) ? &db : nullptr);
+  pl.dec_bytes = align_up(db.off, 256);
   plan_actset(e, b, pl.qry, T, nq, true);
   pl.cell_cap = 8 + (K + 1) * 2 * nl + K * 4 * nl + 4 * nl;
   if (s.steps) pl.cell_cap += K * 2 * nl;
@@ -534,6 +550,18 @@
 
 static int plan_in(mi_engine* e, void* workspace, size_t workspace_bytes, const PlanShape& s, Plan& pl) {
   make_plan(e, workspace, s, pl);
+  if (pl.dec_bytes > e->dec_bytes) {
+    int prev = -1;
+    (void)hipGetDevice(&prev);
+    if (prev != e->device) (void)hipSetDevice(e->device);
+    if (e->dec_buf) (void)hipFree(e->dec_buf);
+    e->dec_buf = nullptr; e->dec_bytes = 0;
+    const hipError_t me = hipMalloc(&e->dec_buf, pl.dec_bytes);
+    if (prev >= 0 && prev != e->device) (void)hipSetDevice(prev);
+    if (me != hipSuccess) { e->dec_buf = nullptr; return fail(e, MI_ERR_HIP, "allocating the decision bytes of the kept passes failed"); }
+    e->dec_bytes = pl.dec_bytes;
+  }
+  if (pl.dec_bytes) make_plan(e, workspace, s, pl);
   if (pl.bytes > workspace_bytes)
     return fail(e, MI_ERR_WORKSPACE, "workspace too small: need " + std::to_string(pl.bytes) + " bytes");
   return MI_OK;
@@ -791,6 +819,10 @@
     BnArgs ba = bn_args(e, A, tan, l, n, theta);
     ba.out = tan ? tan->X.pd[l] : A.p[l];
     ba.zh_out = tan ? (A.zhl[l] ? tan->X.zhdl[l] : nullptr) : A.zhl[l];
+    if (e->stored_dec && L.pool && A.zhl[l] && A.argl[l]) {
+      if (tan) { ba.zh_in = A.zhl[l]; ba.arg_in = A.argl[l]; }
+      else ba.arg_out = A.argl[l];
+    }
     ba.amax_out = cell_bind(e, pl, ba.out);
     LAUNCH(e, st, op_bn, l, tan ? launch_bn_tan_fwd(st, ba, T, L.pool) : launch_bn_fwd(st, ba, T, L.pool));
   }
@@ -916,7 +948,7 @@
         const Layer& L0 = e->L[l - 1];
         ca.bp = A.p[l - 1]; ca.bzh = zh_lo; ca.partial = pl.bnpart;
         if (tan) { ca.bzhd = zhd_lo; ca.bdp = A.dp[l - 1]; }
-        ca.barg = (l - 1 == 0 && e->fuse1) ? A.arg0 : nullptr;
+        ca.barg = (l - 1 == 0 && e->fuse1) ? A.arg0 : (e->stored_dec ? A.argl[l - 1] : nullptr);
         ca.fin = fin_of(e, T, 1.0, FIN_SUMS, g + L0.off_gamma, P, g + L0.off_beta, P);
         int blk0 = 0;
         LAUNCH(e, st, op_dgrad, l, launch_conv3x3(st, ca, T, nterms, EPI_BRED, 1, &blk0));
@@ -1455,7 +1487,7 @@
                   (u)c.lr_steps, (u)(uintptr_t)c.lr_grad_out, (u)(uintptr_t)c.loss_out, (u)(uintptr_t)c.acc_out,
                   (u)(uintptr_t)c.meta_grad_out, (u)(uintptr_t)c.logits_out, (u)(uintptr_t)c.workspace, (u)c.workspace_bytes,
                   (u)e->fuse1, (u)e->gram1, (u)e->gramq, (u)e->overlap, (u)e->fuse_fin, (u)e->fuse_b1red, (u)e->fuse_tail, (u)e->fuse_last,
-                  kernel_selection_key(), (u)(uintptr_t)c.step_w};
+                  kernel_selection_key(), (u)(uintptr_t)c.step_w, (u)e->stored_dec, (u)(uintptr_t)e->dec_buf};
 }
 
 static int meta_batch_entry(mi_engine* e, void* stream, const MetaCall& c) {
diff --git a/exploring_meta_amd/csrc/kernels.h b/exploring_meta_amd/csrc/kernels.h
--- a/exploring_meta_amd/csrc/kernels.h
+++ b/exploring_meta_amd/csrc/kernels.h
@@ -48,6 +48,9 @@
   float* out;
   unsigned* amax_out;
   float* zh_out;
+  uint8_t* arg_out;
+  const float* zh_in;
+  const uint8_t* arg_in;
   double* partial;
   FinArgs fin;
   int n, ho, wo, c;
diff --git a/exploring_meta_amd/engine.py b/exploring_meta_amd/engine.py
--- a/exploring_meta_amd/engine.py
+++ b/exploring_meta_amd/engine.py
@@ -126,6 +126,9 @@
 
     def set_fused_last_block(self, on):
         _lib.check(self.lib.mi_engine_set_fused_last_block(self._h, int(on)), self._h)
+
+    def set_stored_decisions(self, on):
+        _lib.check(self.lib.mi_engine_set_stored_decisions(self._h, int(on)), self._h)
 
     def set_graph(self, on):
         _lib.check(self.lib.mi_engine_set_graph(self._h, int(on)), self._h)
diff --git a/exploring_meta_amd/utils/roofline.py b/exploring_meta_amd/utils/roofline.py
--- a/exploring_meta_amd/utils/roofline.py
+++ b/exploring_meta_amd/utils/roofline.py
@@ -56,7 +56,7 @@
              'tangent_conv_fwd': (2 * f, 2 * x + 2 * z), 'tangent_dgrad': (2 * f, 2 * z + x + (3 * x + pb if rides else 0)),
              'tangent_wgrad': (2 * f, 2 * x + 2 * z),
              'bn_relu_pool_fwd': (0, z + p + (p if ridden else 0)), 'bn_bwd_reduce': (0, z + p), 'bn_bwd_apply': (0, 2 * z + p),
-             'bn_tangent_fwd': (0, 2 * z + p + (p if ridden else 0)), 'bn_tangent_bwd_reduce': (0, 2 * z + 2 * p),
+             'bn_tangent_fwd': (0, z + 3 * p + p // 4) if ridden else (0, 2 * z + p), 'bn_tangent_bwd_reduce': (0, 2 * z + 2 * p),
              'bn_tangent_bwd_apply': (0, 3 * z + 2 * p)}
         if layer == 0:
             t['tangent_conv_fwd'] = (f, x + 2 * z)
diff --git a/include/mi_maml.h b/include/mi_maml.h
--- a/include/mi_maml.h
+++ b/include/mi_maml.h
@@ -74,6 +74,8 @@
 int mi_engine_set_fused_tail(mi_engine* e, int on);
 
 int mi_engine_set_fused_last_block(mi_engine* e, int on);
+
+int mi_engine_set_stored_decisions(mi_engine* e, int on);
 int mi_debug_tail_stamps(mi_engine* e, unsigned long long* buf);
 
 int mi_anil_workspace_bytes(const mi_engine* e, int tasks, int ways, int shots, int adapt_steps, size_t* bytes);
@@ -215,6 +217,13 @@
 int mi_bn_tangent_fwd(void* stream, const mi_bn_tangent_args* a, float* pd);
 int mi_bn_tangent_bwd(void* stream, const mi_bn_tangent_args* a, float* rdgamma, float* rdbeta, size_t hstride, float* rdz,
                       void* scratch, size_t scratch_bytes);
+size_t mi_amax_cell_words(void);
+int mi_conv3x3_dgrad_bred(void* stream, const float* dz0, const float* w0, const float* dz1, const float* w1, size_t pstride, const float* p,
+                          const uint8_t* arg, const float* zh, const float* zhd, const float* dp, int tasks, int n, int h, int wd, int c, float* dx,
+                          float* sum0, float* sum1, size_t ostride, void* scratch, size_t scratch_bytes);
+int mi_bn_stored_fwd(void* stream, const mi_bn_tangent_args* a, float* p, float* zh, uint8_t* arg, unsigned* amax);
+int mi_bn_stored_tangent_fwd(void* stream, const mi_bn_tangent_args* a, const float* zh_in, const uint8_t* arg_in, float* pd, float* zhd,
+                             unsigned* amax);
 
 #define MI_B1_STATS 0
 #define MI_B1_FWD 1
```

Result: no change. 1934, median of 6 (+0.7%).
